# deryrahman/image-caption-emotion-indonesia

Measured on NVIDIA B200. Metric: decoder_train_tokens_per_sec, higher is better.
Workload: dtype bf16

## Files before the change

image-caption-emotion-indonesia_b200/_lib.py:

```python
import ctypes
import os
from ctypes import c_char_p, c_float, c_int32, c_int64, c_uint64, c_void_p

HERE = os.path.dirname(os.path.abspath(__file__))
LIB_PATH = os.path.join(HERE, "libsn100.so")

OP_NT, OP_NN, OP_TN = 0, 1, 2
CELL_FACTORED, CELL_LSTM = 0, 1

_P = c_void_p
_I32, _I64, _F = c_int32, c_int64, c_float

SIGNATURES = {
    "sn_version": (_I32, []),
    "sn_last_error": (c_char_p, []),
    "sn_device_info": (_I32, [_P, _P, _P, _P]),
    "sn_gather_pack_fwd": (_I32, [_P, _I64, _P, _I64, _P, _I64, _I32, _P, _P, _P, _I64, _P, _I64, _F, c_uint64, _P, _P, _I64, _P]),
    "sn_gather_pack_bwd": (_I32, [_P, _I64, _P, _I64, _P, _I64, _I32, _P, _P, _P, _I64, _P, _I64, _F, c_uint64, _P, _I64, _P, _P, _P]),
    "sn_gemm": (_I32, [_I32, _I64, _I64, _I64, _P, _I64, _P, _I64, _P, _I64, _P, _F, _I32, _I64, _I64, _I64, _I64, _P]),
    "sn_gemm_bf16": (_I32, [_I32, _I64, _I64, _I64, _P, _I64, _P, _I64, _P, _I64, _P, _I64, _P, _F, _I32, _I64, _I64, _I64, _I64, _I64, _P]),
    "sn_gemm_bf16_splitk": (_I32, [_I32, _I64, _I64, _I64, _P, _I64, _P, _I64, _P, _I64, _P, _I64, _P, _F, _I32, _I64, _I64, _I64, _I64, _I64, _I32, _P]),
    "sn_gemm2_ws_bytes": (_I64, [_I64, _I64, _I32, _I32]),
    "sn_gemm2_bf16": (_I32, [_I32, _I64, _I64, _I64, _P, _I64, _P, _I64, _P, _I64, _P, _I64, _P, _F, _I32, _I64, _I64, _I64, _I64, _I64, _I32, _P, _I64, _I32, _P]),
    "sn_vocab_ws_bytes": (_I64, [_I64, _I64]),
    "sn_vocab_nll_fwd": (_I32, [_I64, _I64, _I64, _P, _I64, _P, _I64, _P, _P, _P, _I64, _P, _P, _P, _P, _P, _P]),
    "sn_vocab_nll_bwd": (_I32, [_I64, _I64, _I64, _P, _I64, _P, _I64, _P, _P, _P, _P, _F, _P, _I64, _P, _P, _P]),
    "sn_cast_bf16": (_I32, [_P, _I64, _I64, _I64, _P, _I64, _I64, _P]),
    "sn_cast_bf16_ex": (_I32, [_P, _I64, _I64, _I64, _P, _I64, _I64, _I32, _P]),
    "sn_colsum": (_I32, [_P, _I64, _I64, _I64, _P, _F, _P]),
    "sn_colsum_ex": (_I32, [_P, _I64, _I64, _I64, _P, _F, _I32, _P]),
    "sn_colsum_bf16_ex": (_I32, [_P, _I64, _I64, _I64, _P, _F, _I32, _P]),
    "sn_embed_plan": (_I32, [_P, _I64, _I32, _P, _P, _P, _I64, _I64, _P, _P]),
    "sn_embed_grad": (_I32, [_P, _I64, _P, _I64, _I32, _P, _P, _P, _I64, _P, _I64, _F, c_uint64, _P, _I64, _P, _P, _I32, _P]),
    "sn_adam_clamp_dev_ex": (_I32, [_P, _P, _P, _P, _I32, _P, _P, _P, _P, _P, _F, _F, _F, _F, _I32, _P]),
    "sn_recur_ws_bytes": (_I64, [_I64, _I64]),
    "sn_recur_fwd": (_I32, [_I32, _I64, _I64, _P, _P, _I32, _I32, _P, _P, _P, _P, _P, _P, _P, _P, _P, _P, _P]),
    "sn_recur_bwd": (_I32, [_I32, _I64, _I64, _P, _P, _I32, _I32, _P, _P, _P, _P, _P, _P, _P, _P, _P, _P]),
    "sn_recur_fwd_bf16": (_I32, [_I32, _I64, _I64, _P, _P, _I32, _I32] + [_P] * 12),
    "sn_recur_bwd_bf16": (_I32, [_I32, _I64, _I64, _P, _P, _I32, _I32] + [_P] * 11),
    "sn_recur_cl_max_clusters": (_I32, [_I64]),
    "sn_recur_fwd_cl": (_I32, [_I32, _I64, _I64, _P, _P, _I32, _I32] + [_P] * 11),
    "sn_recur_bwd_cl": (_I32, [_I32, _I64, _I64, _P, _P, _I32, _I32] + [_P] * 11),
    "sn_gate_wait": (_I32, [_P, _I64, _P]),
    "sn_cast_bf16_gate_interleave": (_I32, [_P, _I64, _I64, _I64, _P, _I64, _P]),
    "sn_recur_fwd_gemm": (_I32, [_I32, _I64, _I64, _P, _P, _I32, _P, _P, _P, _P, _P, _P, _P, _P, _P]),
    "sn_recur_hprev": (_I32, [_P, _P, _P, _P, _I64, _I64, _P, _P]),
    "sn_recur_bwd_gemm": (_I32, [_I32, _I64, _I64, _P, _P, _I32, _P, _P, _P, _P, _P, _P, _P, _P, _P]),
    "sn_softmax_nll": (_I32, [_P, _I64, _I64, _I64, _P, _P, _P, _I64, _F, _P, _P, _P, _I64, _P]),
    "sn_colsum_bf16": (_I32, [_P, _I64, _I64, _I64, _P, _F, _P]),
    "sn_reduce_sum": (_I32, [_P, _I64, _F, _P, _I32, _P]),
    "sn_adam_clamp": (_I32, [_P, _P, _P, _P, _I32, _P, _P, _P, _F, _F, _F, _F, _P]),
    "sn_adam_clamp_dev": (_I32, [_P, _P, _P, _P, _I32, _P, _P, _P, _P, _P, _F, _F, _F, _F, _P]),
    "sn_enable_peer_access": (_I32, [_I32]),
    "sn_ipc_export": (_I32, [_P, _P, _P]),
    "sn_ipc_open": (_I32, [_P, _P]),
    "sn_ipc_close": (_I32, [_P]),
    "sn_dp_adam_fused": (_I32, [_I32, _I32, _P, _P, _P, _P, _P, _I32, _P, _P, _P, _P, _P, _F, _F, _F, _F, _P]),
    "sn_dp_slot_elems": (_I64, [_I64, _I32]),
    "sn_dp_push": (_I32, [_I32, _I32, _P, _P, _I64, _I32, _P, _I32, _P, _I32, _P]),
    "sn_dp_adam_recv": (_I32, [_I32, _I32, _P, _P, _P, _I64, _I32, _P, _P, _I32, _P, _P, _I32, _P, _P, _P, _P, _P, _F, _F, _F, _F, _I32, _P]),
    "sn_att_step_fwd": (_I32, [_P, _P, _P, _P, _F, _P, _I64, _I64, _I64, _I64, _P, _I64, _P, _I64, _P]),
    "sn_att_step_bwd": (_I32, [_P, _P, _P, _P, _F, _P, _P, _I64, _P, _I64, _P, _I64, _I64, _I64, _I64, _I64, _P, _P, _P, _P, _P, _P]),
    "sn_att_step_fwd_b16": (_I32, [_P, _P, _P, _P, _F, _P, _I64, _I64, _I64, _I64, _P, _I64, _P, _I64, _P]),
    "sn_att_step_bwd_b16": (_I32, [_P, _P, _P, _P, _P, _P, _I64, _P, _I64, _P, _I64, _I64, _I64, _I64, _I64, _P, _P, _P, _P, _P]),
    "sn_mean_pixels": (_I32, [_P, _I64, _I64, _I64, _P, _P]),
    "sn_beam_split_ws_floats": (_I64, [_I32, _I32, _I32]),
    "sn_beam_step_split": (_I32, [_P, _I64, _I64, _I32, _I32, _I32, _I32, _I32] + [_P] * 14 + [_I32, _P, _I32, _P]),
    "sn_split_limbs_cols": (_I32, [_P, _I64, _I64, _I64, _I64, _P, _I64, _I32, _P]),
    "sn_split_limbs_rows": (_I32, [_P, _I64, _I64, _I64, _I64, _P, _I64, _I64, _I32, _P]),
    "sn_skinny_max_rows": (_I32, []),
    "sn_skinny_linear": (_I32, [_P, _I64, _I64, _I64, _P, _I64, _I64, _I64, _I64, _P, _P, _I64, _P, _P]),
    "sn_decode_cell": (_I32, [_I32, _I64, _I64, _P, _I64, _I64, _P, _I64, _I64, _P, _P, _P, _P, _P, _P, _P, _P, _P, _P]),
    "sn_decode_cell_groups": (_I32, [_I32, _I64, _I64, _P, _I64, _P, _I64, _I64, _I64, _P, _I64, _I64, _P, _I64, _P, _P,
                                     _P, _P, _P, _P, _P, _P, _P]),
    "sn_pool_nhwc_fwd": (_I32, [_P, _I64, _I64, _I64, _I64, _I64, _P, _P, _P, _P]),
    "sn_pool_nhwc_bwd": (_I32, [_P, _I64, _I64, _I64, _I64, _I64, _P, _P]),
    "sn_bn1d_fwd": (_I32, [_P, _I64, _I64, _P, _P, _P, _P, _F, _F, _I32, _P, _P, _P, _P]),
    "sn_bn1d_bwd": (_I32, [_P, _P, _I64, _I64, _P, _P, _P, _I32, _P, _P, _P, _P]),
    "sn_beam_step": (_I32, [_P, _I64, _I64, _I32, _I32, _I32, _I32, _I32] + [_P] * 15),
    "sn_bleu_counts": (_I32, [_P, _P, _I64, _P, _P, _P, _I32, _I64, _P, _P]),
}

_lib = None


def load():
    global _lib
    if _lib is not None:
        return _lib
    if not os.path.exists(LIB_PATH):
        raise RuntimeError(
            "libsn100.so is not built (%s). Run `python -c 'import __graft_entry__ as g; g.build()'`; "
            "there is no CPU or PyTorch fallback for this path." % LIB_PATH)
    lib = ctypes.CDLL(LIB_PATH)
    for name, (res, args) in SIGNATURES.items():
        fn = getattr(lib, name)
        fn.restype = res
        fn.argtypes = args
    _lib = lib
    return lib


class SnError(RuntimeError):
    pass


def check(rc, what=""):
    if rc != 0:
        msg = load().sn_last_error()
        raise SnError("%s failed (rc=%d): %s" % (what or "libsn100 call", rc, msg.decode() if msg else "?"))


_dev_ok = {}


def require_device(device_index):
    if _dev_ok.get(device_index):
        return
    lib = load()
    sm = c_int32(); sh = c_int32(); ma = c_int32(); mi = c_int32()
    check(lib.sn_device_info(ctypes.byref(sm), ctypes.byref(sh), ctypes.byref(ma), ctypes.byref(mi)), "sn_device_info")
    _dev_ok[device_index] = (sm.value, sh.value, ma.value, mi.value)
```

image-caption-emotion-indonesia_b200/csrc/sn_elementwise.cu:

```cuda
#include <stdlib.h>
#include <string.h>
#include <cuda_bf16.h>

#include "sn_common.cuh"

namespace {

__global__ void gather_pack_fwd_kernel(const int64_t* __restrict__ captions, int64_t cap_ld,
                                       const float* __restrict__ table, int E,
                                       const float* __restrict__ features, int64_t feat_ld, int has_feat,
                                       const int32_t* __restrict__ row_b, const int32_t* __restrict__ row_t,
                                       const int32_t* __restrict__ tok_override, int64_t N,
                                       float* __restrict__ X, int64_t ldx, float p, float inv_keep,
                                       uint64_t seed, const uint64_t* __restrict__ seed_dev,
                                       __nv_bfloat16* __restrict__ Xb, int64_t ldxb, int Ep) {
  if (seed_dev) seed += *seed_dev;
  int64_t row = (int64_t)blockIdx.x * (blockDim.x >> 5) + (threadIdx.x >> 5);
  if (row >= N) return;
  int lane = threadIdx.x & 31;
  int b = row_b[row], t = row_t[row];
  int ov = tok_override ? tok_override[row] : -1;
  float* dst = X ? X + row * ldx : nullptr;
  __nv_bfloat16* dstb = Xb ? Xb + row * ldxb : nullptr;
  const float* src;
// ... 180 lines not shown
    for (int u = 0; u < EBW_BATCH; ++u) {
      const int q = q0 + u;
      x[u] = 0.f; sc[u] = 0.f;
      if (q < n) {
        const int64_t j = rows[q];
        x[u] = dX[j * ldx + c];
        sc[u] = sn::dropout_scale(seed, (uint32_t)j, (uint32_t)c, rate[q], inv_keep);
      }
    }
#pragma unroll
    for (int u = 0; u < EBW_BATCH; ++u)
      if (sc[u] != 0.f) acc = __fmaf_rn(x[u], sc[u], acc);
  }
  if (e - s <= EB_CHUNK) dtable[(int64_t)t * E + c] += acc;
  else part[(int64_t)(cstart[t] + (i - s) / EB_CHUNK) * E + c] = acc;
}

__global__ void embed_combine_kernel(const int32_t* __restrict__ cnt, const int32_t* __restrict__ cstart, int64_t V,
                                     int E, const float* __restrict__ part, float* __restrict__ dtable) {
  const int64_t t = (int64_t)blockIdx.x * (blockDim.x >> 5) + (threadIdx.x >> 5);
  if (t >= V || cnt[t] <= EB_CHUNK) return;
  const int lane = threadIdx.x & 31;
  const int32_t nq = (cnt[t] + EB_CHUNK - 1) / EB_CHUNK;
  const float* src = part + (int64_t)cstart[t] * E;
  for (int c = lane; c < E; c += 32) {
    float a = 0.f;
    for (int32_t q = 0; q < nq; ++q) a += src[(int64_t)q * E + c];
    dtable[t * E + c] += a;
  }
}

__global__ void __launch_bounds__(256) softmax_nll_kernel(const float* __restrict__ logits, int64_t V, int64_t ld,
                                                          const int64_t* __restrict__ targets,
                                                          float* __restrict__ row_loss, float* dlogits, int64_t ldd,
                                                          float grad_scale, int64_t* __restrict__ argmax,
                                                          int32_t* __restrict__ top5hit, int use_smem,
                                                          __nv_bfloat16* __restrict__ dlb, int64_t lddb) {
  extern __shared__ float srow[];
  __shared__ float red_v[8];
  __shared__ int red_i[8];
  __shared__ float bc_f[2];
  __shared__ int bc_i;
  const int64_t row = blockIdx.x;
  const float* src = logits + row * ld;
  const int tid = threadIdx.x, lane = tid & 31, warp = tid >> 5;

  float mx = -INFINITY;
  int mi = 0x7fffffff;
  for (int64_t c = tid; c < V; c += 256) {
    float v = src[c];
    if (use_smem) srow[c] = v;
    if (v > mx) { mx = v; mi = (int)c; }
  }
#pragma unroll
  for (int o = 16; o > 0; o >>= 1) {
    float ov = __shfl_xor_sync(0xffffffffu, mx, o);
    int oi = __shfl_xor_sync(0xffffffffu, mi, o);
    if (ov > mx || (ov == mx && oi < mi)) { mx = ov; mi = oi; }
  }
  if (lane == 0) { red_v[warp] = mx; red_i[warp] = mi; }
  __syncthreads();
  if (tid == 0) {
    float bm = red_v[0]; int bi = red_i[0];
    for (int w = 1; w < 8; ++w)
      if (red_v[w] > bm || (red_v[w] == bm && red_i[w] < bi)) { bm = red_v[w]; bi = red_i[w]; }
    bc_f[0] = bm; bc_i = bi;
  }
  __syncthreads();
  mx = bc_f[0];
  if (tid == 0 && argmax) argmax[row] = bc_i;
  if (!targets) return;

  const float* rd = use_smem ? srow : src;
  const int64_t tgt = targets[row];
  const float tv = rd[tgt];
  float se = 0.f;
  int above = 0;
  for (int64_t c = tid; c < V; c += 256) {
    float v = rd[c];
    se += expf(v - mx);
    above += (v > tv);
  }
  se = sn::warp_sum(se);
#pragma unroll
  for (int o = 16; o > 0; o >>= 1) above += __shfl_xor_sync(0xffffffffu, above, o);
  __syncthreads();
  if (lane == 0) { red_v[warp] = se; red_i[warp] = above; }
  __syncthreads();
  if (tid == 0) {
    float s = 0.f; int a = 0;
    for (int w = 0; w < 8; ++w) { s += red_v[w]; a += red_i[w]; }
    float lse = mx + logf(s);
    bc_f[1] = lse;
    if (row_loss) row_loss[row] = lse - tv;
    if (top5hit) top5hit[row] = a < 5 ? 1 : 0;
  }
  __syncthreads();
  if (dlogits || dlb) {
    const float lse = bc_f[1];
    float* dst = dlogits ? dlogits + row * ldd : nullptr;
    __nv_bfloat16* dstb = dlb ? dlb + row * lddb : nullptr;
    for (int64_t c = tid; c < V; c += 256) {
      float pr = expf(rd[c] - lse);
      float gr = (pr - (c == tgt ? 1.f : 0.f)) * grad_scale;
      if (dst) dst[c] = gr;
      if (dstb) dstb[c] = __float2bfloat16(gr);
    }
    if (dstb) for (int64_t c = V + tid; c < lddb; c += 256) dstb[c] = __float2bfloat16(0.f);
  }
}

__global__ void __launch_bounds__(1024) reduce_sum_kernel(const float* __restrict__ x, int64_t N, float scale,
                                                           float* out, int accumulate) {
  __shared__ double part[32];
  double s = 0.0;
  for (int64_t i = threadIdx.x; i < N; i += 1024) s += (double)x[i];
#pragma unroll
  for (int o = 16; o > 0; o >>= 1) s += __shfl_xor_sync(0xffffffffu, s, o);
  if ((threadIdx.x & 31) == 0) part[threadIdx.x >> 5] = s;
  __syncthreads();
  if (threadIdx.x == 0) {
    double t = 0.0;
    for (int w = 0; w < 32; ++w) t += part[w];
    float r = (float)(t * (double)scale);
    *out = accumulate ? *out + r : r;
  }
}

struct AdamRanges {
  static constexpr int MAX = 128;
  int64_t off[MAX];
  int32_t len[MAX];
  float step_size[MAX], bc2_sqrt[MAX];
  int step_idx[MAX];
  int32_t chunk_start[MAX + 1];
  int n;
};
static_assert(sizeof(AdamRanges) <= 3700, "AdamRanges must leave room for the other kernel parameters below 4 KB");

__global__ void adam_prepare_kernel(AdamRanges R, int32_t* __restrict__ steps, const float* __restrict__ lr,
                                    float* __restrict__ coef, float beta1, float beta2) {
  int r = threadIdx.x;
  if (r >= R.n) return;
  int st = steps[R.step_idx[r]] + 1;
  steps[R.step_idx[r]] = st;
  double bc1 = 1.0 - pow((double)beta1, (double)st);
  double bc2 = 1.0 - pow((double)beta2, (double)st);
  coef[2 * R.step_idx[r]] = (float)((double)(*lr) / bc1);
  coef[2 * R.step_idx[r] + 1] = (float)sqrt(bc2);
}
constexpr int ADAM_CHUNK = 4096;
constexpr int64_t ADAM_MAX_LEN = (1LL << 31) - 2 * ADAM_CHUNK;

__global__ void __launch_bounds__(256) adam_clamp_kernel(float* __restrict__ p, float* __restrict__ g,
                                                         float* __restrict__ m, float* __restrict__ v,
                                                         AdamRanges R, const float* __restrict__ coef, float beta1,
                                                         float beta2, float eps, float clip) {
  const int64_t total_chunks = R.chunk_start[R.n];
  for (int64_t ch = blockIdx.x; ch < total_chunks; ch += gridDim.x) {
    int r = 0;
    while (ch >= R.chunk_start[r + 1]) ++r;
    const int64_t base = R.off[r] + (ch - R.chunk_start[r]) * ADAM_CHUNK;
    const int64_t end = R.off[r] + R.len[r];
    const float ss = coef ? coef[2 * R.step_idx[r]] : R.step_size[r], bc = coef ? coef[2 * R.step_idx[r] + 1] : R.bc2_sqrt[r];
    const int64_t lim = base + ADAM_CHUNK < end ? base + ADAM_CHUNK : end;
    if ((base & 3) == 0 && lim - base == ADAM_CHUNK) {
#pragma unroll
      for (int it = 0; it < ADAM_CHUNK / (256 * 4); ++it) {
        const int64_t i = base + (int64_t)(it * 256 + threadIdx.x) * 4;
        float4 g4 = *reinterpret_cast<const float4*>(g + i);
        float4 m4 = *reinterpret_cast<const float4*>(m + i);
        float4 v4 = *reinterpret_cast<const float4*>(v + i);
        float4 p4 = *reinterpret_cast<const float4*>(p + i);
        float* gp = &g4.x; float* mp = &m4.x; float* vp = &v4.x; float* pp = &p4.x;
#pragma unroll
        for (int e = 0; e < 4; ++e) {
          float gi = gp[e];
          if (clip > 0.f) gi = fminf(fmaxf(gi, -clip), clip);
          gp[e] = gi;
          float mi = mp[e] + (1.f - beta1) * (gi - mp[e]);
          float vi = vp[e] * beta2 + (1.f - beta2) * gi * gi;
          float denom = sqrtf(vi) / bc + eps;
          pp[e] = pp[e] - ss * (mi / denom);
          mp[e] = mi; vp[e] = vi;
        }
        if (clip > 0.f) *reinterpret_cast<float4*>(g + i) = g4;
        *reinterpret_cast<float4*>(m + i) = m4;
        *reinterpret_cast<float4*>(v + i) = v4;
        *reinterpret_cast<float4*>(p + i) = p4;
      }
      continue;
    }
    for (int64_t i = base + threadIdx.x; i < lim; i += 256) {
      float gi = g[i];
      if (clip > 0.f) { gi = fminf(fmaxf(gi, -clip), clip); g[i] = gi; }
      float mi = m[i], vi = v[i];
      mi = mi + (1.f - beta1) * (gi - mi);
      vi = vi * beta2 + (1.f - beta2) * gi * gi;
      float denom = sqrtf(vi) / bc + eps;
      p[i] = p[i] - ss * (mi / denom);
      m[i] = mi; v[i] = vi;
    }
  }
}

struct DpPeers {
  float* grad[8];
  float* param[8];
  int* pad[8];
  int world, rank;
  void* recv[8];
  int64_t slot_elems;
  int* wait_pad[4];
  int n_wait;
};
constexpr int PAD_ARRIVE = 0, PAD_DONE = 8, PAD_COUNTER = 16, PAD_EPOCH = 17, PAD_DONE_COUNTER = 18;

__device__ __forceinline__ int ld_acquire_sys(const int* p) {
  int v;
  asm volatile("ld.acquire.sys.global.s32 %0, [%1];" : "=r"(v) : "l"(p) : "memory");
  return v;
}
__device__ __forceinline__ void st_release_sys(int* p, int v) {
  asm volatile("st.release.sys.global.s32 [%0], %1;" ::"l"(p), "r"(v) : "memory");
}

constexpr int DP_SUB = 4;
template <typename TT>
__global__ void __launch_bounds__(256 * DP_SUB) dp_push_kernel(DpPeers P, AdamRanges R, const float* __restrict__ g) {
  const int W = P.world;
  __shared__ int s_last;
  int* mypad = P.pad[P.rank];
  const int64_t total_chunks = R.chunk_start[R.n];
  const int sub = threadIdx.x >> 8, tid = threadIdx.x & 255;
  for (int64_t ch = (int64_t)blockIdx.x * DP_SUB + sub; ch < total_chunks; ch += (int64_t)gridDim.x * DP_SUB) {
    int r = 0;
    while (ch >= R.chunk_start[r + 1]) ++r;
    const int64_t aid = R.off[r] / ADAM_CHUNK + (ch - R.chunk_start[r]);
    const int owner = (int)(aid % W);
    if (owner == P.rank) continue;
    const int64_t end = R.off[r] + R.len[r];
    const int64_t base = aid * ADAM_CHUNK > R.off[r] ? aid * ADAM_CHUNK : R.off[r];
    const int64_t lim = (aid + 1) * ADAM_CHUNK < end ? (aid + 1) * ADAM_CHUNK : end;
    TT* dst = reinterpret_cast<TT*>(P.recv[owner]) + (int64_t)P.rank * P.slot_elems + (aid / W) * ADAM_CHUNK - aid * ADAM_CHUNK;
    if ((base & 3) == 0 && lim - base == ADAM_CHUNK) {
      float4 t[ADAM_CHUNK / 1024];
#pragma unroll
      for (int u = 0; u < ADAM_CHUNK / 1024; ++u)
        t[u] = __ldcg(reinterpret_cast<const float4*>(g + base + (int64_t)(u * 256 + tid) * 4));
#pragma unroll
      for (int u = 0; u < ADAM_CHUNK / 1024; ++u) {
        const int64_t i = base + (int64_t)(u * 256 + tid) * 4;
        if constexpr (sizeof(TT) == 4) {
          *reinterpret_cast<float4*>(dst + i) = t[u];
        } else {
          __nv_bfloat162 lo = __floats2bfloat162_rn(t[u].x, t[u].y), hi = __floats2bfloat162_rn(t[u].z, t[u].w);
          uint2 pk;
          pk.x = *reinterpret_cast<uint32_t*>(&lo); pk.y = *reinterpret_cast<uint32_t*>(&hi);
          *reinterpret_cast<uint2*>(dst + i) = pk;
        }
      }
      continue;
    }
    for (int64_t i = base + tid; i < lim; i += 256) {
      if constexpr (sizeof(TT) == 4) dst[i] = g[i]; else dst[i] = __float2bfloat16_rn(g[i]);
    }
  }
  __syncthreads();
  if (threadIdx.x == 0) {
    __threadfence_system();
    s_last = (atomicAdd(mypad + PAD_COUNTER, 1) == (int)gridDim.x - 1);
  }
  __syncthreads();
  if (s_last) {
    if (threadIdx.x == 0) {
      __threadfence_system();
      const int e = mypad[PAD_EPOCH] + 1;
      for (int q = 0; q < W; ++q) st_release_sys(P.pad[q] + PAD_ARRIVE + P.rank, e);
      mypad[PAD_COUNTER] = 0;
    }
  }
}

template <int W>
__global__ void __launch_bounds__(256) dp_adam_fused_kernel(DpPeers P, AdamRanges R, const float* __restrict__ coef,
                                                            float* __restrict__ m, float* __restrict__ v, float beta1,
                                                            float beta2, float eps, float clip, int dbg) {
  if (dbg) {
    for (int q = 0; q < P.world; ++q) {
      if (dbg & 1) P.grad[q] = P.grad[P.rank];
      if (dbg & 2) P.param[q] = P.param[P.rank];
    }
  }
  __shared__ int s_epoch, s_last;
  int* mypad = P.pad[P.rank];
  if (threadIdx.x == 0) s_epoch = mypad[PAD_EPOCH] + 1;
  __syncthreads();
  const int e = s_epoch;
  if (blockIdx.x == 0 && threadIdx.x < P.world) st_release_sys(P.pad[threadIdx.x] + PAD_ARRIVE + P.rank, e);
  if (threadIdx.x < P.world) { while (ld_acquire_sys(mypad + PAD_ARRIVE + threadIdx.x) < e) { } }
  __syncthreads();
  const int64_t total_chunks = R.chunk_start[R.n];
  const int64_t nslots = (total_chunks + W - 1) / W;
  for (int64_t slot = blockIdx.x; slot < nslots; slot += gridDim.x)
  for (int j = 0; j < W; ++j) {
    const int64_t ch = slot * W + j;
    if (ch >= total_chunks) break;
    int r = 0;
    while (ch >= R.chunk_start[r + 1]) ++r;
    const int64_t aid = R.off[r] / ADAM_CHUNK + (ch - R.chunk_start[r]);
    if ((int)(aid % W) != P.rank) continue;
    const int64_t end = R.off[r] + R.len[r];
    const int64_t base = aid * ADAM_CHUNK > R.off[r] ? aid * ADAM_CHUNK : R.off[r];
    const int64_t lim = (aid + 1) * ADAM_CHUNK < end ? (aid + 1) * ADAM_CHUNK : end;
    const float ss = coef[2 * R.step_idx[r]], bc = coef[2 * R.step_idx[r] + 1];
    if ((base & 3) == 0 && lim - base == ADAM_CHUNK) {
      constexpr int NIT = W <= 4 ? 4 : 2;
#pragma unroll
      for (int it0 = 0; it0 < ADAM_CHUNK / (256 * 4); it0 += NIT) {
        float4 t[NIT][W], m4[NIT], v4[NIT], p4[NIT];
#pragma unroll
        for (int u = 0; u < NIT; ++u) {
          const int64_t i = base + (int64_t)((it0 + u) * 256 + threadIdx.x) * 4;
#pragma unroll
          for (int q = 0; q < W; ++q) t[u][q] = __ldcg(reinterpret_cast<const float4*>(P.grad[q] + i));
        }
#pragma unroll
        for (int u = 0; u < NIT; ++u) {
          const int64_t i = base + (int64_t)((it0 + u) * 256 + threadIdx.x) * 4;
          m4[u] = *reinterpret_cast<const float4*>(m + i);
          v4[u] = *reinterpret_cast<const float4*>(v + i);
          p4[u] = *reinterpret_cast<const float4*>(P.param[P.rank] + i);
        }
#pragma unroll
        for (int u = 0; u < NIT; ++u) {
          const int64_t i = base + (int64_t)((it0 + u) * 256 + threadIdx.x) * 4;
          float4 g4 = t[u][0];
#pragma unroll
          for (int q = 1; q < W; ++q) { g4.x += t[u][q].x; g4.y += t[u][q].y; g4.z += t[u][q].z; g4.w += t[u][q].w; }
          float* gp = &g4.x; float* mp = &m4[u].x; float* vp = &v4[u].x; float* pp = &p4[u].x;
#pragma unroll
          for (int k = 0; k < 4; ++k) {
            float gi = gp[k];
            if (clip > 0.f) gi = fminf(fmaxf(gi, -clip), clip);
            const float mi = mp[k] + (1.f - beta1) * (gi - mp[k]);
            const float vi = vp[k] * beta2 + (1.f - beta2) * gi * gi;
            pp[k] = pp[k] - ss * (mi / (sqrtf(vi) / bc + eps));
            mp[k] = mi; vp[k] = vi;
          }
          *reinterpret_cast<float4*>(m + i) = m4[u];
          *reinterpret_cast<float4*>(v + i) = v4[u];
#pragma unroll
          for (int q = 0; q < W; ++q) *reinterpret_cast<float4*>(P.param[q] + i) = p4[u];
        }
      }
      continue;
// ... 37 lines not shown
                                                           const float* __restrict__ g, const TT* __restrict__ recv,
                                                           const float* p_loc, float* __restrict__ m, float* __restrict__ v, float beta1,
                                                           float beta2, float eps, float clip) {
  __shared__ int s_epoch, s_last;
  const int rank = P.rank;
  int* mypad = P.wait_pad[0];
  if (threadIdx.x == 0) s_epoch = mypad[PAD_EPOCH] + 1;
  if (threadIdx.x < W * P.n_wait) {
    const int* wp = P.wait_pad[threadIdx.x / W];
    const int q = threadIdx.x % W;
    if (q != rank) { const int we = wp[PAD_EPOCH] + 1; while (ld_acquire_sys(wp + PAD_ARRIVE + q) < we) { } }
  }
  __syncthreads();
  const int e = s_epoch;
  const int64_t total_chunks = R.chunk_start[R.n];
  const int sub = threadIdx.x >> 8, tid = threadIdx.x & 255;
  for (int64_t ch = (int64_t)blockIdx.x * DP_RSUB + sub; ch < total_chunks; ch += (int64_t)gridDim.x * DP_RSUB) {
    int r = 0;
    while (ch >= R.chunk_start[r + 1]) ++r;
    const int64_t a0 = R.off[r] / ADAM_CHUNK;
    const int64_t aid = a0 + ((rank - a0) % W + W) % W + (ch - R.chunk_start[r]) * W;
    const int64_t end = R.off[r] + R.len[r];
    const int64_t base = aid * ADAM_CHUNK > R.off[r] ? aid * ADAM_CHUNK : R.off[r];
    const int64_t lim = (aid + 1) * ADAM_CHUNK < end ? (aid + 1) * ADAM_CHUNK : end;
    const float ss = coef[2 * R.step_idx[r]], bc = coef[2 * R.step_idx[r] + 1];
    const int64_t rbase = (aid / W) * ADAM_CHUNK - aid * ADAM_CHUNK;
    if ((base & 3) == 0 && lim - base == ADAM_CHUNK) {
#pragma unroll
      for (int it = 0; it < ADAM_CHUNK / (256 * 4); ++it) {
        const int64_t i = base + (int64_t)(it * 256 + tid) * 4;
        float4 t[W];
#pragma unroll
        for (int q = 0; q < W; ++q) {
          if (q == rank) {
            t[q] = __ldcg(reinterpret_cast<const float4*>(g + i));
          } else if constexpr (sizeof(TT) == 4) {
            t[q] = __ldcg(reinterpret_cast<const float4*>(recv + q * P.slot_elems + rbase + i));
          } else {
            const uint2 pk = __ldcg(reinterpret_cast<const uint2*>(recv + q * P.slot_elems + rbase + i));
            const float2 lo = __bfloat1622float2(*reinterpret_cast<const __nv_bfloat162*>(&pk.x));
            const float2 hi = __bfloat1622float2(*reinterpret_cast<const __nv_bfloat162*>(&pk.y));
            t[q] = make_float4(lo.x, lo.y, hi.x, hi.y);
          }
        }
        float4 m4 = *reinterpret_cast<const float4*>(m + i);
        float4 v4 = *reinterpret_cast<const float4*>(v + i);
        float4 p4 = *reinterpret_cast<const float4*>(p_loc + i);
        float4 g4 = t[0];
#pragma unroll
        for (int q = 1; q < W; ++q) { g4.x += t[q].x; g4.y += t[q].y; g4.z += t[q].z; g4.w += t[q].w; }
        float* gp = &g4.x; float* mp = &m4.x; float* vp = &v4.x; float* pp = &p4.x;
#pragma unroll
        for (int k = 0; k < 4; ++k) {
          float gi = gp[k];
          if (clip > 0.f) gi = fminf(fmaxf(gi, -clip), clip);
          const float mi = mp[k] + (1.f - beta1) * (gi - mp[k]);
          const float vi = vp[k] * beta2 + (1.f - beta2) * gi * gi;
          pp[k] = pp[k] - ss * (mi / (sqrtf(vi) / bc + eps));
          mp[k] = mi; vp[k] = vi;
        }
        *reinterpret_cast<float4*>(m + i) = m4;
        *reinterpret_cast<float4*>(v + i) = v4;
#pragma unroll
        for (int q = 0; q < W; ++q) *reinterpret_cast<float4*>(P.param[q] + i) = p4;
      }
      continue;
    }
    for (int64_t i = base + tid; i < lim; i += 256) {
      float gi = 0.f;
#pragma unroll
      for (int q = 0; q < W; ++q) {
        float gq;
        if (q == rank) gq = __ldcg(g + i);
        else if constexpr (sizeof(TT) == 4) gq = __ldcg(recv + q * P.slot_elems + rbase + i);
        else gq = __bfloat162float(recv[q * P.slot_elems + rbase + i]);
        gi = q == 0 ? gq : gi + gq;
      }
      if (clip > 0.f) gi = fminf(fmaxf(gi, -clip), clip);
      const float mi = m[i] + (1.f - beta1) * (gi - m[i]);
      const float vi = v[i] * beta2 + (1.f - beta2) * gi * gi;
      const float pn = p_loc[i] - ss * (mi / (sqrtf(vi) / bc + eps));
      m[i] = mi; v[i] = vi;
#pragma unroll
      for (int q = 0; q < W; ++q) P.param[q][i] = pn;
    }
  }
  __syncthreads();
  if (threadIdx.x == 0) {
    __threadfence_system();
    s_last = (atomicAdd(mypad + PAD_DONE_COUNTER, 1) == (int)gridDim.x - 1);
  }
  __syncthreads();
  if (s_last) {
    if (threadIdx.x == 0) __threadfence_system();
    __syncthreads();
    if (threadIdx.x < W) {
      st_release_sys(P.pad[threadIdx.x] + PAD_DONE + rank, e);
      while (ld_acquire_sys(mypad + PAD_DONE + threadIdx.x) < e) { }
    }
    __syncthreads();
    if (threadIdx.x == 0) {
      mypad[PAD_DONE_COUNTER] = 0; mypad[PAD_EPOCH] = e;
      for (int k = 1; k < P.n_wait; ++k) P.wait_pad[k][PAD_EPOCH] = P.wait_pad[k][PAD_EPOCH] + 1;
    }
  }
}

__global__ void mean_pixels_kernel(const float* __restrict__ feat, int64_t P, int64_t D, float* __restrict__ out) {
  int64_t b = blockIdx.y;
  int64_t d = (int64_t)blockIdx.x * blockDim.x + threadIdx.x;
  if (d >= D) return;
  const float* src = feat + b * P * D + d;
  float s = 0.f;
  for (int64_t pz = 0; pz < P; ++pz) s += src[pz * D];
  out[b * D + d] = s / (float)P;
}

}

extern "C" {

int32_t sn_gather_pack_fwd(const int64_t* captions, int64_t cap_ld, const float* table, int64_t E,
                           const float* features, int64_t feat_ld, int32_t has_feat,
                           const int32_t* row_b, const int32_t* row_t, const int32_t* tok_override,
                           int64_t N, float* X, int64_t ldx, float p_drop, uint64_t seed, const uint64_t* seed_dev,
                           void* Xb, int64_t ldxb, void* stream) {
  SN_REQUIRE(N >= 0 && E > 0 && (X || Xb), "sn_gather_pack_fwd: bad dims N=%lld E=%lld", (long long)N, (long long)E);
  SN_REQUIRE(!X || ldx >= E, "sn_gather_pack_fwd: ldx=%lld < E", (long long)ldx);
  SN_REQUIRE(!Xb || ldxb >= E, "sn_gather_pack_fwd: ldxb=%lld < E", (long long)ldxb);
  SN_REQUIRE(p_drop >= 0.f && p_drop < 1.f, "sn_gather_pack_fwd: dropout p=%f out of [0,1)", p_drop);
  SN_REQUIRE(!has_feat || features, "sn_gather_pack_fwd: has_feat without features");
  if (N == 0) return 0;
  float inv_keep = 1.f / (1.f - p_drop);
  unsigned grid = (unsigned)((N + 7) / 8);
  gather_pack_fwd_kernel<<<grid, 256, 0, (cudaStream_t)stream>>>(captions, cap_ld, table, (int)E, features, feat_ld,
                                                                 has_feat, row_b, row_t, tok_override, N, X, ldx,
                                                                 p_drop, inv_keep, seed, seed_dev,
                                                                 (__nv_bfloat16*)Xb, ldxb, Xb ? (int)ldxb : (int)E);
  return sn::check_launch("sn_gather_pack_fwd");
}

int32_t sn_gather_pack_bwd(const int64_t* captions, int64_t cap_ld, float* dtable, int64_t E,
                           float* dfeatures, int64_t feat_ld, int32_t has_feat, const int32_t* row_b,
                           const int32_t* row_t, const int32_t* tok_override, int64_t N,
                           const float* dX, int64_t ldx, float p_drop, uint64_t seed, const uint64_t* seed_dev,
                           int64_t V, int32_t* ws_int, float* ws_part, void* stream) {
  SN_REQUIRE(N >= 0 && E > 0 && ldx >= E && V > 0, "sn_gather_pack_bwd: bad dims");
  SN_REQUIRE(p_drop >= 0.f && p_drop < 1.f, "sn_gather_pack_bwd: dropout p=%f out of [0,1)", p_drop);
  SN_REQUIRE(N < (int64_t)1 << 30, "sn_gather_pack_bwd: N=%lld rows", (long long)N);
  if (N == 0) return 0;
  SN_REQUIRE(ws_int && ws_part, "sn_gather_pack_bwd: null work space");
  if (int32_t rc = sn_embed_plan(captions, cap_ld, has_feat, row_b, row_t, tok_override, N, V, ws_int, stream)) return rc;
  return sn_embed_grad(dtable, E, dfeatures, feat_ld, has_feat, row_b, row_t, tok_override, N, dX, ldx, p_drop, seed,
                       seed_dev, V, ws_int, ws_part, 0, stream);
}

namespace {
struct EmbedWs {
  int32_t *cnt, *start, *cursor, *cstart, *tok32, *perm, *sorted;
  EmbedWs(int32_t* ws, int64_t V, int64_t N)
      : cnt(ws), start(cnt + V), cursor(start + V + 1), cstart(cursor + V), tok32(cstart + V), perm(tok32 + N),
        sorted(perm + N) {}
};
}

int32_t sn_embed_plan(const int64_t* captions, int64_t cap_ld, int32_t has_feat, const int32_t* row_b,
                      const int32_t* row_t, const int32_t* tok_override, int64_t N, int64_t V, int32_t* ws_int,
                      void* stream) {
  SN_REQUIRE(N >= 0 && N < (int64_t)1 << 30 && V > 0, "sn_embed_plan: bad dims N=%lld V=%lld", (long long)N, (long long)V);
  if (N == 0) return 0;
  SN_REQUIRE(ws_int, "sn_embed_plan: null work space");
  cudaStream_t st = (cudaStream_t)stream;
  EmbedWs w(ws_int, V, N);
  SN_CUDA(cudaMemsetAsync(w.cnt, 0, sizeof(int32_t) * (size_t)V, st));
  const unsigned g_rows = (unsigned)((N + 255) / 256);
  embed_count_kernel<<<g_rows, 256, 0, st>>>(captions, cap_ld, has_feat, row_b, row_t, tok_override, N, w.tok32, w.cnt);
  embed_scan_kernel<<<1, 1024, 0, st>>>(w.cnt, V, w.start, w.cursor, w.cstart);
  embed_place_kernel<<<g_rows, 256, 0, st>>>(w.tok32, N, w.cursor, w.perm);
  embed_order_kernel<<<g_rows, 256, 0, st>>>(w.tok32, w.start, w.perm, N, V, w.sorted);
  return sn::check_launch("sn_embed_plan");
}

int32_t sn_embed_grad(float* dtable, int64_t E, float* dfeatures, int64_t feat_ld, int32_t has_feat,
                      const int32_t* row_b, const int32_t* row_t, const int32_t* tok_override, int64_t N,
                      const float* dX, int64_t ldx, float p_drop, uint64_t seed, const uint64_t* seed_dev, int64_t V,
                      const int32_t* ws_int, float* ws_part, int32_t wide, void* stream) {
  SN_REQUIRE(N >= 0 && N < (int64_t)1 << 30 && E > 0 && ldx >= E && V > 0, "sn_embed_grad: bad dims");
  SN_REQUIRE(p_drop >= 0.f && p_drop < 1.f, "sn_embed_grad: dropout p=%f out of [0,1)", p_drop);
  if (N == 0) return 0;
  SN_REQUIRE(ws_int && ws_part, "sn_embed_grad: null work space");
  cudaStream_t st = (cudaStream_t)stream;
  float inv_keep = 1.f / (1.f - p_drop);
  if (has_feat && dfeatures)
    gather_pack_bwd_kernel<<<(unsigned)((N + 7) / 8), 256, 0, st>>>(nullptr, 0, dtable, (int)E, dfeatures,
                                                                     feat_ld, has_feat, row_b, row_t, tok_override, N,
                                                                     dX, ldx, p_drop, inv_keep, seed, seed_dev);
  EmbedWs w(const_cast<int32_t*>(ws_int), V, N);
  if (wide && E <= 512)
    embed_chunk_wide_kernel<<<(unsigned)N, (unsigned)((E + 31) / 32 * 32), 0, st>>>(
        w.tok32, w.start, w.cstart, w.sorted, V, tok_override, dX, ldx, (int)E, p_drop, inv_keep, seed, seed_dev,
        dtable, ws_part);
  else
    embed_chunk_kernel<<<(unsigned)((N + 7) / 8), 256, 0, st>>>(w.tok32, w.start, w.cstart, w.sorted, V, tok_override,
                                                                 dX, ldx, (int)E, p_drop, inv_keep, seed, seed_dev,
                                                                 dtable, ws_part);
  embed_combine_kernel<<<(unsigned)((V + 7) / 8), 256, 0, st>>>(w.cnt, w.cstart, V, (int)E, ws_part, dtable);
  return sn::check_launch("sn_embed_grad");
}

int32_t sn_softmax_nll(const float* logits, int64_t N, int64_t V, int64_t ld, const int64_t* targets,
                       float* row_loss, float* dlogits, int64_t ldd, float grad_scale, int64_t* argmax,
                       int32_t* top5hit, void* dlogits_bf16, int64_t lddb, void* stream) {
  SN_REQUIRE(N >= 0 && V > 0 && ld >= V, "sn_softmax_nll: bad dims");
  SN_REQUIRE(!dlogits_bf16 || lddb >= V, "sn_softmax_nll: lddb < V");
  if (N == 0) return 0;
  size_t smem = (size_t)V * sizeof(float);
  int use_smem = smem <= 200 * 1024;
  if (use_smem && smem > 48 * 1024) {
    static thread_local size_t configured = 0;
    if (configured < smem) {
      SN_CUDA(cudaFuncSetAttribute(softmax_nll_kernel, cudaFuncAttributeMaxDynamicSharedMemorySize, 200 * 1024));
      configured = 200 * 1024;
    }
  }
  softmax_nll_kernel<<<(unsigned)N, 256, use_smem ? smem : 0, (cudaStream_t)stream>>>(
      logits, V, ld, targets, row_loss, dlogits, ldd, grad_scale, argmax, top5hit, use_smem,
      (__nv_bfloat16*)dlogits_bf16, lddb);
  return sn::check_launch("sn_softmax_nll");
}

int32_t sn_reduce_sum(const float* x, int64_t N, float scale, float* out, int32_t accumulate, void* stream) {
  SN_REQUIRE(N >= 0 && out, "sn_reduce_sum: bad args");
  reduce_sum_kernel<<<1, 1024, 0, (cudaStream_t)stream>>>(x, N, scale, out, accumulate);
  return sn::check_launch("sn_reduce_sum");
}

int32_t sn_adam_clamp(float* p, float* g, float* m, float* v, int32_t n_ranges, const int64_t* ranges,
                      const float* step_size, const float* bc2_sqrt, float beta1, float beta2, float eps,
                      float clip, void* stream) {
  SN_REQUIRE(n_ranges >= 0, "sn_adam_clamp: n_ranges < 0");
  int done = 0;
  while (done < n_ranges) {
    AdamRanges R;
    R.n = 0;
    R.chunk_start[0] = 0;
    while (done < n_ranges && R.n < AdamRanges::MAX) {
      int64_t off = ranges[2 * done], len = ranges[2 * done + 1];
      SN_REQUIRE(off >= 0 && len >= 0 && len < ADAM_MAX_LEN, "sn_adam_clamp: bad range %d", done);
      R.off[R.n] = off; R.len[R.n] = (int32_t)len;
      R.step_size[R.n] = step_size[done]; R.bc2_sqrt[R.n] = bc2_sqrt[done];
      R.chunk_start[R.n + 1] = R.chunk_start[R.n] + (len + ADAM_CHUNK - 1) / ADAM_CHUNK;
      ++R.n; ++done;
    }
    int64_t chunks = R.chunk_start[R.n];
    if (chunks == 0) continue;
    int64_t cap = (int64_t)sn::dev_info().sm_count * 8;
    unsigned grid = (unsigned)(chunks < cap ? chunks : cap);
    adam_clamp_kernel<<<grid, 256, 0, (cudaStream_t)stream>>>(p, g, m, v, R, nullptr, beta1, beta2, eps, clip);
    int32_t rc = sn::check_launch("sn_adam_clamp");
    if (rc) return rc;
  }
  return 0;
}

int32_t sn_adam_clamp_dev(float* p, float* g, float* m, float* v, int32_t n_ranges, const int64_t* ranges,
                          const int32_t* step_idx, int32_t* steps_dev, const float* lr_dev, float* coef_ws,
                          float beta1, float beta2, float eps, float clip, void* stream) {
  return sn_adam_clamp_dev_ex(p, g, m, v, n_ranges, ranges, step_idx, steps_dev, lr_dev, coef_ws, beta1, beta2, eps,
                              clip, 0, stream);
}

int32_t sn_adam_clamp_dev_ex(float* p, float* g, float* m, float* v, int32_t n_ranges, const int64_t* ranges,
                             const int32_t* step_idx, int32_t* steps_dev, const float* lr_dev, float* coef_ws,
                             float beta1, float beta2, float eps, float clip, int32_t max_ctas, void* stream) {
  SN_REQUIRE(max_ctas >= 0, "sn_adam_clamp_dev: max_ctas < 0");
  SN_REQUIRE(n_ranges >= 0 && n_ranges <= AdamRanges::MAX, "sn_adam_clamp_dev: at most %d ranges per call", AdamRanges::MAX);
  SN_REQUIRE(steps_dev && lr_dev && coef_ws, "sn_adam_clamp_dev: null argument");
  if (n_ranges == 0) return 0;
  AdamRanges R;
  R.n = n_ranges;
  R.chunk_start[0] = 0;
  for (int i = 0; i < n_ranges; ++i) {
    SN_REQUIRE(ranges[2 * i] >= 0 && ranges[2 * i + 1] >= 0 && ranges[2 * i + 1] < ADAM_MAX_LEN, "sn_adam_clamp_dev: bad range %d", i);
    R.off[i] = ranges[2 * i]; R.len[i] = (int32_t)ranges[2 * i + 1]; R.step_idx[i] = step_idx[i];
    R.step_size[i] = 0.f; R.bc2_sqrt[i] = 1.f;
    R.chunk_start[i + 1] = R.chunk_start[i] + (R.len[i] + ADAM_CHUNK - 1) / ADAM_CHUNK;
  }
  cudaStream_t st = (cudaStream_t)stream;
  adam_prepare_kernel<<<1, AdamRanges::MAX, 0, st>>>(R, steps_dev, lr_dev, coef_ws, beta1, beta2);
  int64_t chunks = R.chunk_start[R.n];
  if (chunks == 0) return sn::check_launch("sn_adam_clamp_dev");
  int64_t cap = (int64_t)sn::dev_info().sm_count * 8;
  if (max_ctas > 0 && max_ctas < cap) cap = max_ctas;
  unsigned grid = (unsigned)(chunks < cap ? chunks : cap);
  adam_clamp_kernel<<<grid, 256, 0, st>>>(p, g, m, v, R, coef_ws, beta1, beta2, eps, clip);
  return sn::check_launch("sn_adam_clamp_dev");
}

int32_t sn_enable_peer_access(int32_t peer_device) {
  int cur = 0;
  SN_CUDA(cudaGetDevice(&cur));
  if (peer_device == cur) return 0;
  int can = 0;
  SN_CUDA(cudaDeviceCanAccessPeer(&can, cur, peer_device));
  SN_REQUIRE(can, "sn_enable_peer_access: device %d cannot access peer %d", cur, peer_device);
  cudaError_t e = cudaDeviceEnablePeerAccess(peer_device, 0);
  if (e == cudaErrorPeerAccessAlreadyEnabled) { cudaGetLastError(); return 0; }
  if (e != cudaSuccess) return sn::fail((int32_t)e, "cudaDeviceEnablePeerAccess(%d): %s", peer_device, cudaGetErrorString(e));
  return 0;
}

int32_t sn_dp_adam_fused(int32_t world, int32_t rank, void* const* grad_ptrs, void* const* param_ptrs,
                         void* const* pad_ptrs, float* m, float* v, int32_t n_ranges, const int64_t* ranges,
                         const int32_t* step_idx, int32_t* steps_dev, const float* lr_dev, float* coef_ws, float beta1,
                         float beta2, float eps, float clip, void* stream) {
  SN_REQUIRE(world >= 1 && world <= 8 && rank >= 0 && rank < world, "sn_dp_adam_fused: bad world/rank %d/%d", world, rank);
  SN_REQUIRE(n_ranges >= 0 && n_ranges <= AdamRanges::MAX, "sn_dp_adam_fused: at most %d ranges per call", AdamRanges::MAX);
  SN_REQUIRE(grad_ptrs && param_ptrs && pad_ptrs && steps_dev && lr_dev && coef_ws && m && v, "sn_dp_adam_fused: null argument");
  DpPeers P;
  memset(&P, 0, sizeof(P));
  P.world = world; P.rank = rank;
  for (int q = 0; q < 8; ++q) {
    P.grad[q] = q < world ? (float*)grad_ptrs[q] : nullptr;
    P.param[q] = q < world ? (float*)param_ptrs[q] : nullptr;
    P.pad[q] = q < world ? (int*)pad_ptrs[q] : nullptr;
    SN_REQUIRE(q >= world || (P.grad[q] && P.param[q] && P.pad[q]), "sn_dp_adam_fused: null peer pointer %d", q);
  }
  AdamRanges R;
  R.n = n_ranges;
  R.chunk_start[0] = 0;
  for (int i = 0; i < n_ranges; ++i) {
    SN_REQUIRE(ranges[2 * i] >= 0 && ranges[2 * i + 1] >= 0 && ranges[2 * i + 1] < ADAM_MAX_LEN, "sn_dp_adam_fused: bad range %d", i);
    R.off[i] = ranges[2 * i]; R.len[i] = (int32_t)ranges[2 * i + 1]; R.step_idx[i] = step_idx[i];
    R.step_size[i] = 0.f; R.bc2_sqrt[i] = 1.f;
    R.chunk_start[i + 1] = R.chunk_start[i] +
        (R.len[i] > 0 ? (R.off[i] + R.len[i] - 1) / ADAM_CHUNK - R.off[i] / ADAM_CHUNK + 1 : 0);
  }
  cudaStream_t st = (cudaStream_t)stream;
  if (n_ranges > 0) adam_prepare_kernel<<<1, AdamRanges::MAX, 0, st>>>(R, steps_dev, lr_dev, coef_ws, beta1, beta2);
  int64_t mine = (R.chunk_start[R.n] + world - 1) / world;
  int64_t cap = (int64_t)sn::dev_info().sm_count * 3;
  unsigned grid = (unsigned)(mine < 1 ? 1 : (mine < cap ? mine : cap));
  static const int dbg = [] { const char* e = getenv("SN_DP_DEBUG"); return e ? atoi(e) : 0; }();
#define SN_DP_LAUNCH(WW) dp_adam_fused_kernel<WW><<<grid, 256, 0, st>>>(P, R, coef_ws, m, v, beta1, beta2, eps, clip, dbg)
  switch (world) {
    case 1: SN_DP_LAUNCH(1); break;
    case 2: SN_DP_LAUNCH(2); break;
    case 3: SN_DP_LAUNCH(3); break;
    case 4: SN_DP_LAUNCH(4); break;
    case 5: SN_DP_LAUNCH(5); break;
    case 6: SN_DP_LAUNCH(6); break;
    case 7: SN_DP_LAUNCH(7); break;
    default: SN_DP_LAUNCH(8); break;
  }
#undef SN_DP_LAUNCH
  return sn::check_launch("sn_dp_adam_fused");
}

static int32_t dp_fill_ranges(AdamRanges& R, int32_t n_ranges, const int64_t* ranges, const int32_t* step_idx, const char* who) {
  SN_REQUIRE(n_ranges >= 0 && n_ranges <= AdamRanges::MAX, "%s: at most %d ranges per call", who, AdamRanges::MAX);
// ... 120 lines not shown
```

image-caption-emotion-indonesia_b200/decoders.py:

```python
import random
from collections import OrderedDict

import os

import torch
import torch.nn as nn

from . import ops
from .arena import ParamArena
from .packing import get_plan

GREEDY_GRAPH = [True]

GATES = ("i", "f", "o", "c")
STYLES = ("factual", "happy", "sad", "angry")


def style_attr(style, gate):
    return ("S_f" + gate) if style == "factual" else ("S_%s_%s" % (style, gate))


def _ref_init(module, emb, out):
    for p in module.parameters():
        if p.dim() >= 2:
            nn.init.xavier_uniform_(p.data)
        else:
            nn.init.zeros_(p.data)
    emb.weight.data.uniform_(-0.1, 0.1)
    out.bias.data.fill_(0)
    out.weight.data.uniform_(-0.1, 0.1)


class _Ctx:
    pass


class _HiddenFn(torch.autograd.Function):

    @staticmethod
    def forward(ctx, anchor, features, dec, plan, captions, coins, mode, save):
        c = dec._run_forward(plan, captions, features, coins, mode, save=save)
        ctx.dec, ctx.c = dec, c
        ctx.need_dfeat = features is not None and features.requires_grad
        return c.top.Hall

    @staticmethod
    def backward(ctx, dHall):
        dec, c = ctx.dec, ctx.c
        gbuf = dec._grad_target(c.grad_names)
        dfeat = dec._run_backward(c, dHall.contiguous(), gbuf, ctx.need_dfeat)
        dec._publish(c.grad_names, gbuf)
        return None, dfeat, None, None, None, None, None, None


class _LogitsFn(torch.autograd.Function):

    @staticmethod
    def forward(ctx, Hall, anchor, dec):
        ctx.dec = dec
        ctx.save_for_backward(Hall)
        return dec._vocab_logits(Hall)

    @staticmethod
    def backward(ctx, dlogits):
        dec = ctx.dec
        (Hall,) = ctx.saved_tensors
        gbuf = dec._grad_target(dec._out_names())
        dHall = dec._vocab_backward(Hall, dlogits.contiguous(), gbuf)
        dec._publish(dec._out_names(), gbuf)
        return dHall, None, None


def _pad8(n):
    return (n + 7) // 8 * 8


class _DecoderBase(nn.Module):

    cell = ops.CELL_FACTORED
    precision = "fp32"

    _TRANSIENT = ("_greedy_graphs", "_decode_sessions", "_side_streams", "_out_w16", "_out_w16_pref", "_out_w16_ev",
                  "_out_h16", "_seed_dev", "_arena", "_att_cache", "_gate_flag", "_gate_armed", "_after_recur", "_bucket_hook",
                  "_emb_early")

    def __getstate__(self):
        st = self.__dict__.copy()
        for k in self._TRANSIENT:
            st.pop(k, None)
        return st

    def set_precision(self, precision):
        if precision not in ("fp32", "bf16"):
            raise ValueError("precision must be 'fp32' or 'bf16'")
        self.precision = precision
        return self

    @property
    def bf16(self):
        return self.precision == "bf16"

    def _shadow(self, w, rows=None, cols=None):
        return ops.to_bf16_padded(w)

    def _arena_groups(self):
        raise NotImplementedError

    def arena(self):
        a = self.__dict__.get("_arena")
        if a is None:
            a = ParamArena(self, self._arena_groups())
            self.__dict__["_arena"] = a
        return a.ensure()

    def _grad_target(self, names):
        a = self.arena()
        if any(a.named[n].grad is not None for n in names):
            return torch.zeros_like(a.gflat)
        return a.gflat

    def _publish(self, names, gbuf):
        self.arena().publish_grads(names, gbuf)

    def _side(self, i=0):
        sts = self.__dict__.setdefault("_side_streams", {})
        st = sts.get(i)
        if st is None:
            st = torch.cuda.Stream()
            sts[i] = st
        return st

    def _fork(self, i=0):
        side = self._side(i)
        side.wait_stream(torch.cuda.current_stream())
        return side

    def _join(self):
        for st in self.__dict__.get("_side_streams", {}).values():
            torch.cuda.current_stream().wait_stream(st)

    def _take_out_shadow(self):
        Wb = self.__dict__.pop("_out_w16_pref", None)
        ev = self.__dict__.pop("_out_w16_ev", None)
        if Wb is not None and ev is not None:
            torch.cuda.current_stream().wait_event(ev)
        return Wb

    def _shadows_async(self, specs, max_blocks=24):
        main = torch.cuda.current_stream()
        outs = []
        for dct, key, w in specs:
            R, C = w.shape
            Cp = (C + 7) // 8 * 8
            out = torch.empty(R, Cp, dtype=torch.bfloat16, device=w.device)
            dct[key] = out
            outs.append((w, out, R, C, Cp))
        side = self._side(2)
        side.wait_stream(main)
        with torch.cuda.stream(side):
            for w, out, R, C, Cp in outs:
                ops.cast_bf16(w, R, C, w.stride(0), out, Cp, Cp, max_blocks=max_blocks)
            ev = torch.cuda.Event()
            ev.record(side)
        return ev

    def _next_seed(self, dev, p_drop):
        base = int(self.__dict__.get("_seed", 0x5EED)) * 1000003
        if p_drop <= 0.0:
            return base, None
        sd = self.__dict__.get("_seed_dev")
        if sd is None or sd.device != dev:
            sd = torch.zeros(1, dtype=torch.int64, device=dev)
            self.__dict__["_seed_dev"] = sd
        sd.add_(1)
        return base, sd

    def _check_inputs(self, captions, features):
        if not captions.is_cuda:
            raise ops._lib.SnError("decoder inputs must be CUDA tensors: this path has no CPU fallback")
        ops.lib()

    def _emb(self):
        raise NotImplementedError

    def _out(self):
        raise NotImplementedError

    def _input_projection(self, c, X, mode, r0, n):
        raise NotImplementedError

    def _input_projection_bwd(self, c, dZ, gbuf):
        raise NotImplementedError

    def _coins(self, T, teacher_forcing_ratio):
        return [random.random() < teacher_forcing_ratio for _ in range(T)]

    def _run_forward(self, plan, captions, features, coins, mode, save):
        a = self.arena()
        dev = captions.device
        d = plan.dev(dev)
        H, N, B, T = self.hidden_size, plan.N, plan.B, plan.T
        emb = self._emb()
        E = emb.weight.shape[1]
        has_feat = features is not None
        c = _Ctx()
        c.plan, c.mode, c.has_feat, c.captions = plan, mode, has_feat, captions
        c.p_drop = float(self.dropout.p) if self.training else 0.0
        c.seed, c.seed_dev = self._next_seed(dev, c.p_drop)
        feats = None
        if has_feat:
            feats = features.detach()
            if feats.dtype != torch.float32 or not feats.is_contiguous():
                feats = feats.float().contiguous()
            if feats.dim() == 3:
                feats = feats.reshape(feats.shape[0], -1)
        all_tf = all(coins)
        c.tok_override = None
        if not all_tf:
            c.tok_override = torch.full((N,), -1, dtype=torch.int32, device=dev)
        c.emb_ws = c.emb_ev = c.emb_zeroed = None
        if self.__dict__.pop("_emb_early", False) and all_tf:
            V = emb.weight.shape[0]
            c.emb_ws = ops.embed_plan_ws(V, N, dev)
            c.emb_zeroed = a.gflat
            gE = self._gview(a.gflat, [self._emb_name()], emb.weight.shape)
            side = self._side(4)
            side.wait_stream(torch.cuda.current_stream())
            with torch.cuda.stream(side):
                ops.embed_plan(captions, has_feat, d["row_b"], d["row_t"], None, N, V, c.emb_ws)
                gE.zero_()
                c.emb_ev = torch.cuda.Event()
                c.emb_ev.record(side)
        c.Ein = E
        c.w16 = {}
        c.ev_early = c.ev_late = c.ev_first = None
        if self.bf16:
            early, late = self._shadow_specs(c, mode)
            first = c.__dict__.pop("first_specs", None)
            if first:
                c.ev_first = self._shadows_async(first, max_blocks=0)
            second = c.__dict__.pop("second_specs", None)
            c.ev_second = self._shadows_async(second, max_blocks=0) if second else None
            if early:
                c.ev_early = self._shadows_async(early)
            if late:
                c.ev_late = self._shadows_async(late)
            self.__dict__["_out_w16_ev"] = self._shadows_async([(self.__dict__, "_out_w16_pref", self._out().weight)])
        if self.bf16:
            X = None
            c.Xb = torch.empty(N, _pad8(E), dtype=torch.bfloat16, device=dev)
        else:
            X = torch.empty(N, E, dtype=torch.float32, device=dev)
            c.Xb = None
        ops.gather_pack_fwd(captions, emb.weight, feats, has_feat, d["row_b"], d["row_t"], None, N, X,
                            c.p_drop, c.seed, seed_dev=c.seed_dev, Xb=c.Xb)
        c.X = X
        c.XP = torch.empty(N, 4 * H, dtype=torch.float32, device=dev)
        self._input_projection(c, X, mode, 0, N)
        c.Hall = torch.empty(N, H, dtype=torch.float32, device=dev)
        c.Call = torch.empty(N, H, dtype=torch.float32, device=dev) if save else None
        c.Hprev = torch.empty(N, H, dtype=torch.float32, device=dev) if save else None
        c.gates = torch.empty(N, 4 * H, dtype=torch.float32, device=dev) if save else None
        c_state = torch.zeros(B, H, dtype=torch.float32, device=dev)
        c.aux_argmax = None
        Whh, bhh = self._recurrent_weights()
        c.Whh, c.bhh = Whh, bhh
        use_tc = self.bf16 and H % 32 == 0
        c.Hb = c.Hpb = None
        if c.ev_late is not None:
            torch.cuda.current_stream().wait_event(c.ev_late)
        if use_tc:
            if "Whh" not in c.w16:
                c.w16["Whh"] = self._shadow(Whh)
            c.Hb = torch.empty(N, H, dtype=torch.bfloat16, device=dev)
            c.Hpb = torch.empty(N, H, dtype=torch.bfloat16, device=dev) if save else None
            c.Hprev = None
        c.upper = self._upper_layers_init(c, save)
        c.top = c.upper[-1] if c.upper else c

        c.c_state = c_state

        def run(t0, t1):
            self._recur_fwd(c, c, t0, t1)
            if c.upper:
                self._upper_layers_fwd(c, t0, t1)

        if all_tf:
            run(0, T)
        else:
            out = self._out()
            V = out.weight.shape[0]
            pred = captions[:, 0].to(torch.int32).contiguous()
            am = torch.empty(B, dtype=torch.int64, device=dev)
            t = 0
            while t < T:
                if coins[t]:
                    t1 = t
                    while t1 < T and coins[t1]:
                        t1 += 1
                    run(t, t1)
                    t = t1
                else:
                    bt, r0 = plan.bs[t], plan.off[t]
                    if t > 0:
                        bp, rp = plan.bs[t - 1], plan.off[t - 1]
                        lg = torch.empty(bp, V, dtype=torch.float32, device=dev)
                        ops.gemm(ops.OP_NT, c.top.Hall, out.weight, lg, bp, V, H, H, H, V, bias=out.bias,
                                 a_off=rp * H)
                        ops.softmax_nll(lg, bp, V, argmax=am)
                        pred = am[:bp].to(torch.int32)
                    c.tok_override[r0:r0 + bt] = pred[:bt]
                    ops.gather_pack_fwd(captions, emb.weight, feats, has_feat, d["row_b"], d["row_t"],
                                        c.tok_override, bt, X, c.p_drop, c.seed, row_off=r0, seed_dev=c.seed_dev,
                                        Xb=c.Xb)
                    self._input_projection(c, X, mode, r0, bt)
                    run(t, t + 1)
                    t += 1
        c.grad_names = self._seq_grad_names(mode)
        c.feat_shape = None if features is None else features.shape
        if not save:
            c.X = c.XP = None
        return c

    def _recur_fwd(self, c, cl, t0, t1):
        plan = c.plan
        d = plan.dev(cl.XP.device)
        H, B, T = self.hidden_size, plan.B, plan.T
        Whh, bhh = cl.Whh, cl.bhh
        if cl.Hb is not None:
            if t0 == 0 and t1 == T and B >= ops.RECUR_GEMM_MIN_BATCH[0] and H % 64 == 0:
                if "Whh_il" not in cl.w16:
                    cl.w16["Whh_il"] = ops.cast_gate_interleave(Whh)
                if cl.Call is None:
                    cl.Call = torch.empty(plan.N, H, dtype=torch.float32, device=cl.XP.device)
                ops.recur_fwd_gemm(self.cell, H, B, plan, cl.XP, cl.w16["Whh_il"], bhh, cl.Hall, cl.Hb, cl.Call, cl.gates)
                if cl.Hpb is not None:
                    ops.recur_hprev(cl.Hb, d, plan.N, H, cl.Hpb)
                cl.recur_gemm = True
                return
            h_init = cl.Hall[plan.off[t0 - 1]:] if t0 > 0 else None
            ops.recur_fwd_bf16(self.cell, H, B, d["bs"], d["off"], t0, t1, cl.XP, cl.w16["Whh"], bhh, h_init,
                               cl.Hall, cl.Hb, cl.Hpb, cl.Call, cl.gates, cl.c_state)
        else:
            h_init = cl.Hall[plan.off[t0 - 1]:] if t0 > 0 else None
            ops.recur_fwd(self.cell, H, B, d["bs"], d["off"], t0, t1, cl.XP, Whh, bhh, h_init, cl.Hall,
                          cl.Call, cl.Hprev, cl.gates, cl.c_state)

    def _shadow_specs(self, c, mode):
        H = self.hidden_size
        late = []
        if H % 32 == 0:
            late.append((c.w16, "Whh", self._recurrent_weights()[0]))
        return [], late

    def _upper_layers_init(self, c, save):
        return []

    def _upper_layers_fwd(self, c, t0, t1):
        pass

    def _layer_bwd(self, c, cl, dHall, gbuf):
        plan = c.plan
        dev = dHall.device
        d = plan.dev(dev)
        H, N, B, T = self.hidden_size, plan.N, plan.B, plan.T
        L = getattr(cl, "layer", 0)
        Whh, _ = self._recurrent_weights(L)
        dZ = torch.empty(N, 4 * H, dtype=torch.float32, device=dev)
        dhc = torch.zeros(2, B, H, dtype=torch.float32, device=dev)
        dh, dc = dhc[0], dhc[1]
        gW, gbW = self._recurrent_grads(gbuf, L)
        if cl.Hpb is not None:
            cl.dZb = torch.empty(N, 4 * H, dtype=torch.bfloat16, device=dev)
            if getattr(cl, "recur_gemm", False):
                ops.recur_bwd_gemm(self.cell, H, B, plan, cl.w16["Whh"], cl.Call, cl.gates, dHall, dZ, cl.dZb, dc)
            else:
                ops.recur_bwd_bf16(self.cell, H, B, d["bs"], d["off"], 0, T, cl.w16["Whh"], None, cl.Call, cl.gates,
                                   dHall, dZ, cl.dZb, dh, dc, start_flag=self.__dict__.pop("_gate_armed", None))
            self._run_deferred()
            with torch.cuda.stream(self._fork()):
                ops.gemm_bf16(ops.OP_TN, cl.dZb, cl.Hpb, 4 * H, H, N, 4 * H, H, C=gW, ldc=H)
                ops.colsum(dZ, N, 4 * H, 4 * H, gbW, wide=bool(ops.TAIL_SCHEDULE[0]))
            cl.colsum_dZ = gbW if ops.TAIL_SCHEDULE[0] else None
            return self._input_projection_bwd(cl, dZ, gbuf)
        ops.recur_bwd(self.cell, H, B, d["bs"], d["off"], 0, T, Whh, None, cl.Call, cl.gates, dHall, dZ, dh, dc)
        if self.bf16:
            cl.dZb = ops.to_bf16_padded(dZ)
            Hpb = ops.to_bf16_padded(cl.Hprev)
            ops.gemm_bf16(ops.OP_TN, cl.dZb, Hpb, 4 * H, H, N, 4 * H, H, C=gW, ldc=H)
        else:
            ops.gemm(ops.OP_TN, dZ, cl.Hprev, gW, 4 * H, H, N, 4 * H, H, H)
        ops.colsum(dZ, N, 4 * H, 4 * H, gbW)
        return self._input_projection_bwd(cl, dZ, gbuf)

    def _run_backward(self, c, dHall, gbuf, need_dfeat):
        for cl in reversed(c.upper):
            dHall = self._layer_bwd(c, cl, dHall, gbuf)
        dX = self._layer_bwd(c, c, dHall, gbuf)
        out = self._embedding_bwd(c, dX, gbuf, need_dfeat)
        self._join()
        return out

    def _embedding_bwd(self, c, dX, gbuf, need_dfeat):
        plan = c.plan
        dev = dX.device
        d = plan.dev(dev)
        N, B = plan.N, plan.B
        emb = self._emb()
        E = emb.weight.shape[1]
        gE = self._gview(gbuf, [self._emb_name()], emb.weight.shape)
        dfeat = torch.empty(B, E, dtype=torch.float32, device=dev) if (need_dfeat and c.has_feat) else None
        if getattr(c, "emb_ws", None) is not None:
            torch.cuda.current_stream().wait_event(c.emb_ev)
            if gbuf is not c.emb_zeroed:
                gE.zero_()
            ops.embed_grad(gE, dfeat, c.has_feat, d["row_b"], d["row_t"], c.tok_override, N, dX, c.p_drop, c.seed,
                           c.emb_ws, seed_dev=c.seed_dev, wide=True)
        else:
            gE.zero_()
            ops.gather_pack_bwd(c.captions, gE, dfeat, c.has_feat, d["row_b"], d["row_t"], c.tok_override, N, dX,
                                c.p_drop, c.seed, seed_dev=c.seed_dev)
        if dfeat is not None and c.feat_shape is not None:
            dfeat = dfeat.view(c.feat_shape)
        self._bucket_final([self._emb_name()])
        return dfeat

    def _run_deferred(self):
        todo = self.__dict__.pop("_after_recur", None)
        for fn in todo or ():
            fn()

    def _bucket_final(self, names):
        hook = self.__dict__.get("_bucket_hook")
        if hook is None:
            return
        gbuf, fn = hook
        names = [n for n in names if n in self.arena().named]
        self._publish(names, gbuf)
        fn(names)

    def _gview(self, gbuf, names, shape):
        a = self.arena()
        o, n = a._span(names)
        return gbuf[o:o + n].view(shape)

    def _vocab_logits(self, Hall, Hb=None):
        out = self._out()
        if self.bf16:
            V, H = out.weight.shape
            N = Hall.shape[0]
            if Hb is None:
                Hb = ops.to_bf16_padded(Hall.contiguous())
            Wb = self._take_out_shadow()
            if Wb is None:
                Wb = ops.to_bf16_padded(out.weight)
            self.__dict__["_out_w16"] = Wb
            logits = torch.empty(N, V, dtype=torch.float32, device=Hall.device)
            ops.gemm_bf16(ops.OP_NT, Hb, Wb, N, V, H, Hb.stride(0), Wb.stride(0), C=logits, ldc=V, bias=out.bias)
            return logits
        return ops.linear_nt(Hall.contiguous(), out.weight, out.bias)

    def _vocab_backward(self, Hall, dlogits, gbuf, Hb=None, dLb=None, defer=None, gate_B=None):
        out = self._out()
        V, H = out.weight.shape
        N = Hall.shape[0]
        wn, bn = self._out_names()
        gC = self._gview(gbuf, [wn], (V, H))
        gb = self._gview(gbuf, [bn], (V,))
        dHall = torch.empty(N, H, dtype=torch.float32, device=Hall.device)
        if self.bf16:
            have_b16 = dLb is not None
            if not have_b16:
                dLb = ops.to_bf16_padded(dlogits)
            hb_stash = self.__dict__.pop("_out_h16", None)
            if Hb is None:
                Hb = hb_stash if (have_b16 and hb_stash is not None) else ops.to_bf16_padded(Hall.contiguous())
            Wb = self.__dict__.pop("_out_w16", None) if dLb is not None and have_b16 else None
            if Wb is None:
                Wb = ops.to_bf16_padded(out.weight)
            if have_b16:
                mode_dc = ops.DC_SCHEDULE[0] if defer is not None else 0
                side = self._side(0)
                if mode_dc != 2:
                    side.wait_stream(torch.cuda.current_stream())
                ops.gemm_bf16(ops.OP_NN, dLb, Wb, N, H, V, dLb.stride(0), Wb.stride(0), C=dHall, ldc=H)
                if mode_dc == 1:
                    side.wait_stream(torch.cuda.current_stream())

                gate = None
                if mode_dc == 0 and gate_B is not None and ops.GATE_DC[0] and ops.recur_cluster_ok(H, gate_B):
                    gate = self.__dict__.get("_gate_flag")
                    if gate is None or gate.device != dHall.device:
                        gate = self.__dict__["_gate_flag"] = torch.zeros(3, dtype=torch.int32, device=dHall.device)
                    self.__dict__["_gate_armed"] = gate

                def side_work():
                    if mode_dc == 2:
                        side.wait_stream(torch.cuda.current_stream())
                    with torch.cuda.stream(side):
                        if gate is not None:
                            ops.gate_wait(gate)
                        ops.gemm_bf16(ops.OP_TN, dLb, Hb, V, H, N, dLb.stride(0), Hb.stride(0), C=gC, ldc=H,
                                      max_pairs=0 if mode_dc == 2 else ops.DC_MAX_PAIRS[0])
                        ops.colsum_bf16(dLb, N, V, dLb.stride(0), gb, wide=bool(ops.TAIL_SCHEDULE[0]))
                if mode_dc == 0:
                    side_work()
                else:
                    defer.append(side_work)
                return dHall
            ops.gemm_bf16(ops.OP_NN, dLb, Wb, N, H, V, dLb.stride(0), Wb.stride(0), C=dHall, ldc=H)
            ops.gemm_bf16(ops.OP_TN, dLb, Hb, V, H, N, dLb.stride(0), Hb.stride(0), C=gC, ldc=H)
        else:
            ops.gemm(ops.OP_NN, dlogits, out.weight, dHall, N, H, V, dlogits.stride(0), H, H)
            ops.gemm(ops.OP_TN, dlogits, Hall, gC, V, H, N, dlogits.stride(0), H, H)
        ops.colsum(dlogits, N, V, dlogits.stride(0), gb)
        return dHall

    def _vocab_nll(self, Hall, Hb, targets, denom, backward):
        out = self._out()
        V, H = out.weight.shape
        N, dev = Hall.shape[0], Hall.device
        row_loss = torch.empty(N, dtype=torch.float32, device=dev)
        argmax = torch.empty(N, dtype=torch.int64, device=dev)
        top5 = torch.empty(N, dtype=torch.int32, device=dev)
        if self.bf16:
            if Hb is None:
                Hb = ops.to_bf16_padded(Hall.contiguous())
            Wb = self._take_out_shadow()
            if Wb is None:
                Wb = ops.to_bf16_padded(out.weight)
            self.__dict__["_out_w16"] = Wb
            self.__dict__["_out_h16"] = Hb
            tl = torch.empty(N, dtype=torch.float32, device=dev)
            lse = torch.empty(N, dtype=torch.float32, device=dev)
            above = torch.empty(N, dtype=torch.int32, device=dev)
            ops.vocab_nll_fwd(Hb, Wb, out.bias, targets, N, V, H, tl, lse, row_loss=row_loss, argmax=argmax, above=above)
            dLb = torch.empty(N, _pad8(V), dtype=torch.bfloat16, device=dev) if backward else None
            ops.vocab_nll_bwd(Hb, Wb, out.bias, targets, N, V, H, tl, lse, 1.0 / denom, dLb=dLb, above=above,
                              top5hit=top5)
            return row_loss, argmax, top5, None, dLb
        logits = self._vocab_logits(Hall, Hb)
        ops.softmax_nll(logits, N, V, targets=targets, row_loss=row_loss, dlogits=logits if backward else None,
                        grad_scale=1.0 / denom, argmax=argmax, top5hit=top5)
        return row_loss, argmax, top5, logits, None

    def _forward_greedy(self, captions, lengths, features, mode):
        key = (tuple(int(l) for l in lengths), mode, tuple(captions.shape),
               None if features is None else tuple(features.shape), self.precision, self.training,
               captions.device.index, self.arena().version)
        cache = self.__dict__.setdefault("_greedy_graphs", OrderedDict())
        sess = cache.get(key)
        if sess is None:
            sess = cache[key] = _Ctx()
            sess.calls, sess.graph = 0, None
            while len(cache) > 4:
                cache.popitem(last=False)
        cache.move_to_end(key)
        sess.calls += 1
        plan = get_plan(lengths)
        coins = self._coins(plan.T, 0.0)
        if sess.graph is None and sess.calls < 2:
            c = self._run_forward(plan, captions.contiguous(), features, coins, mode, save=False)
            return self._vocab_logits(c.top.Hall, c.top.Hb)
        if sess.graph is None:
            sess.captions = captions.contiguous().clone()
            sess.features = None if features is None else features.detach().clone()
            torch.cuda.synchronize()
            g = torch.cuda.CUDAGraph()
            with ops.no_gc_during_capture(), torch.cuda.graph(g):
                c = self._run_forward(plan, sess.captions, sess.features, coins, mode, save=False)
                sess.out = self._vocab_logits(c.top.Hall, c.top.Hb)
            sess.graph = g
        sess.captions.copy_(captions, non_blocking=True)
        if features is not None:
            sess.features.copy_(features, non_blocking=True)
        sess.graph.replay()
        return sess.out.clone()

    def _greedy_eligible(self, captions, lengths, features, teacher_forcing_ratio):
        if torch.is_grad_enabled() or teacher_forcing_ratio > 0.0 or not GREEDY_GRAPH[0] or not captions.is_cuda:
            return False
        if torch.cuda.is_current_stream_capturing():
            return False
        if features is not None and features.shape[-1] != self._emb().weight.shape[1]:
            return False
        plan = get_plan(lengths)
        T_in = captions.shape[1] + (1 if features is not None else 0)
        return plan.B == captions.shape[0] and plan.T <= T_in

    def _forward_hidden(self, captions, lengths, features, teacher_forcing_ratio, mode):
        self._check_inputs(captions, features)
        if features is not None and features.shape[-1] != self._emb().weight.shape[1]:
            raise RuntimeError("features must be [B, embed_size]")
        plan = get_plan(lengths)
        if plan.B != captions.shape[0]:
            raise RuntimeError("len(lengths) != batch size")
        T_in = captions.shape[1] + (1 if features is not None else 0)
        if plan.T > T_in:
            raise RuntimeError("lengths exceed the (feature +) caption length")
        coins = self._coins(plan.T, teacher_forcing_ratio)
        captions = captions.contiguous()
        anchor = self._out().weight
        save = torch.is_grad_enabled()
        return _HiddenFn.apply(anchor, features, self, plan, captions, coins, mode, save), plan

    def forward_loss(self, captions, lengths, features=None, targets=None, teacher_forcing_ratio=1.0,
                     mode="factual", backward=True, n_global=None, grad_hook=None, early_step=None, early_embed=False):
        self._check_inputs(captions, features)
        plan = get_plan(lengths)
        coins = self._coins(plan.T, teacher_forcing_ratio)
        captions = captions.contiguous()
        dev = captions.device
        self.__dict__["_emb_early"] = bool(early_embed and backward and self.bf16 and self._emb().weight.grad is None)
        with torch.no_grad():
            c = self._run_forward(plan, captions, features, coins, mode, save=backward)
            N = plan.N
            out = self._out()
            V = out.weight.shape[0]
            if targets is None:
                if features is None:
                    raise ValueError("forward_loss: pass `targets` when features is None (language-only "
                                     "pass: inputs captions[:, :-1], targets packed captions[:, 1:])")
                if self.bf16:
                    targets = torch.empty(N, dtype=captions.dtype, device=dev)
                    side = self._side(2)
                    with torch.cuda.stream(side):
                        self._default_targets(captions, plan, True, out=targets)
                        ev = torch.cuda.Event()
                        ev.record(side)
                    torch.cuda.current_stream().wait_event(ev)
                else:
                    targets = self._default_targets(captions, plan, True)
            denom = float(n_global if n_global is not None else N)
            row_loss, argmax, top5, logits, dLb = self._vocab_nll(c.top.Hall, c.top.Hb, targets, denom, backward)
            loss = torch.empty(1, dtype=torch.float32, device=dev)
            if not (backward and dLb is not None):
                ops.reduce_sum(row_loss, N, 1.0 / denom, loss)
            if backward:
                gbuf = self._grad_target(c.grad_names + list(self._out_names()))
                deferred = []
                gate_B = plan.B if (c.top.Hpb is not None and not (plan.B >= ops.RECUR_GEMM_MIN_BATCH[0] and self.hidden_size % 64 == 0)) else None
                dHall = self._vocab_backward(c.top.Hall, logits, gbuf, c.top.Hb, dLb, defer=deferred, gate_B=gate_B)
                if dLb is not None:
                    def loss_and_bucket():
                        with torch.cuda.stream(self._side(0)):
                            ops.reduce_sum(row_loss, N, 1.0 / denom, loss)
                            if early_step is not None and gbuf is self.arena().gflat:
                                self._publish(list(self._out_names()), gbuf)
                                early_step(list(self._out_names()))
                    if deferred:
                        deferred.append(loss_and_bucket)
                    else:
                        loss_and_bucket()
                self.__dict__["_after_recur"] = deferred
                if grad_hook is not None and gbuf is self.arena().gflat:
                    self._run_deferred()
                    self._join()
                    grad_hook(list(self._out_names()))
                need_dfeat = features is not None and features.requires_grad
                self.__dict__["_bucket_hook"] = (gbuf, early_step) if (early_step is not None and gbuf is self.arena().gflat) else None
                try:
                    dfeat = self._run_backward(c, dHall, gbuf, need_dfeat)
                finally:
                    self.__dict__["_bucket_hook"] = None
                self._run_deferred()
                self._join()
                self._publish(c.grad_names + list(self._out_names()), gbuf)
                if grad_hook is not None:
                    grad_hook(c.grad_names if gbuf is self.arena().gflat else c.grad_names + list(self._out_names()))
                if dfeat is not None:
                    features.grad = dfeat if features.grad is None else features.grad + dfeat
        return loss, {"argmax": argmax, "top5hit": top5, "n_tokens": N}

    def _default_targets(self, captions, plan, has_feat, out=None):
        d = plan.dev(captions.device)
        key = "tgt_idx_%d_%d" % (captions.shape[1], 0 if has_feat else 1)
        idx = d.get(key)
        if idx is None:
            idx = (d["row_b"].long() * captions.shape[1] + d["row_t"].long() + (0 if has_feat else 1)).contiguous()
            d[key] = idx
        if out is not None:
            return torch.index_select(captions.reshape(-1), 0, idx, out=out)
        return captions.reshape(-1).index_select(0, idx)


V_CAST_SIDE = [os.environ.get("SN_V_CAST_SIDE", "1") == "1"]


class DecoderFactoredLSTM(_DecoderBase):

    cell = ops.CELL_FACTORED

    def __init__(self, embed_size, hidden_size, factored_size, vocab_size, num_layers, feature_size=2048,
                 bias=True, dropout=0.22, max_seq_length=40):
        super().__init__()
        if not bias:
            raise NotImplementedError("bias=False is not supported by the fused path")
        self.feature_size, self.hidden_size = feature_size, hidden_size
        self.factored_size, self.embed_size = factored_size, embed_size
        self.vocab_size, self.max_seq_length = vocab_size, max_seq_length
        self.num_layers = num_layers
        self.dropout = nn.Dropout(dropout)
        self.B = nn.Embedding(vocab_size, embed_size)
        for g in GATES:
            setattr(self, "U_" + g, nn.Linear(factored_size, hidden_size, bias=bias))
            setattr(self, style_attr("factual", g), nn.Linear(factored_size, factored_size, bias=bias))
            setattr(self, "V_" + g, nn.Linear(embed_size, factored_size, bias=bias))
            setattr(self, "W_" + g, nn.Linear(hidden_size, hidden_size, bias=bias))
        for s in STYLES[1:]:
            for g in GATES:
                setattr(self, style_attr(s, g), nn.Linear(factored_size, factored_size, bias=bias))
        self.C = nn.Linear(hidden_size, vocab_size, bias=bias)
        _ref_init(self, self.B, self.C)

    def _arena_groups(self):
        groups = [["B.weight"]]
        for pre in ("V_", "U_", "W_"):
            groups.append([pre + g + ".weight" for g in GATES])
            groups.append([pre + g + ".bias" for g in GATES])
        for s in STYLES:
            groups.append([style_attr(s, g) + ".weight" for g in GATES])
            groups.append([style_attr(s, g) + ".bias" for g in GATES])
        groups += [["C.weight"], ["C.bias"]]
        return groups

    def _emb(self):
        return self.B

    def _emb_name(self):
        return "B.weight"

    def _out(self):
        return self.C

    def _out_names(self):
        return ("C.weight", "C.bias")

    @staticmethod
    def _lp(layer):
        return "" if layer == 0 else "l%d_" % layer

    def _stack(self, pre, shape, grad=False, gbuf=None, bias=False, layer=0):
        names = [self._lp(layer) + pre + g + (".bias" if bias else ".weight") for g in GATES]
        if gbuf is not None:
            return self._gview(gbuf, names, shape)
        return self.arena().block(names, shape, grad=grad)

    def _style_stack(self, mode, shape, gbuf=None, bias=False, layer=0):
        names = [self._lp(layer) + style_attr(mode, g) + (".bias" if bias else ".weight") for g in GATES]
        if gbuf is not None:
            return self._gview(gbuf, names, shape)
        return self.arena().block(names, shape)

    def _shadow_specs(self, c, mode):
        H, F = self.hidden_size, self.factored_size
        early, late = super()._shadow_specs(c, mode)
        if mode in STYLES:
            if V_CAST_SIDE[0]:
                c.first_specs = [(c.w16, "V", self._stack("V_", (4 * F, c.Ein)))]
                c.second_specs = [(c.w16, "S", self._style_stack(mode, (4 * F, F)))]
                early = [(c.w16, "U", self._stack("U_", (4 * H, F)))]
            else:
                early = [(c.w16, "S", self._style_stack(mode, (4 * F, F))), (c.w16, "U", self._stack("U_", (4 * H, F)))]
        return early, late

    def _recurrent_weights(self, layer=0):
        H = self.hidden_size
        return self._stack("W_", (4 * H, H), layer=layer), self._stack("W_", (4 * H,), bias=True, layer=layer)

    def _recurrent_grads(self, gbuf, layer=0):
        H = self.hidden_size
        return (self._stack("W_", (4 * H, H), gbuf=gbuf, layer=layer),
                self._stack("W_", (4 * H,), gbuf=gbuf, bias=True, layer=layer))

    def _seq_grad_names(self, mode):
        names = ["B.weight"]
        for pre in ("V_", "U_", "W_"):
            names += [pre + g + sfx for g in GATES for sfx in (".weight", ".bias")]
        names += [style_attr(mode, g) + sfx for g in GATES for sfx in (".weight", ".bias")]
        return names

    def _input_projection(self, c, X, mode, r0, n):
        if mode not in STYLES:
            raise ValueError("mode name wrong: %r (expected one of %s)" % (mode, STYLES))
        H, F = self.hidden_size, self.factored_size
        Ein = X.shape[1] if X is not None else c.Ein
        dev = c.XP.device
        full = (r0 == 0 and n == c.XP.shape[0])
        if full and not self.bf16:
            c.A1 = torch.empty(n, 4 * F, dtype=torch.float32, device=dev)
            c.A2 = torch.empty(n, 4 * F, dtype=torch.float32, device=dev)
        A1, A2 = c.__dict__.get("A1"), c.__dict__.get("A2")
        L = getattr(c, "layer", 0)
        Vc, bV = self._stack("V_", (4 * F, Ein), layer=L), self._stack("V_", (4 * F,), bias=True, layer=L)
        Sc, bS = self._style_stack(mode, (4 * F, F), layer=L), self._style_stack(mode, (4 * F,), bias=True, layer=L)
        Uc, bU = self._stack("U_", (4 * H, F), layer=L), self._stack("U_", (4 * H,), bias=True, layer=L)
        if self.bf16:
            w16 = c.__dict__.setdefault("w16", {})
            if "V" not in w16:
                w16["V"] = self._shadow(Vc)
            if "S" not in w16:
                w16["S"], w16["U"] = self._shadow(Sc), self._shadow(Uc)
            Vb, Sb, Ub = w16["V"], w16["S"], w16["U"]
            Ep, Fp = Vb.stride(0), Sb.stride(0)
            if full:
                if X is not None:
                    c.Xb = torch.empty(n, Ep, dtype=torch.bfloat16, device=dev)
                c.A1 = torch.empty(n, 4 * F, dtype=torch.bfloat16, device=dev)
                c.A2 = torch.empty(n, 4 * F, dtype=torch.bfloat16, device=dev)
            if X is not None:
                ops.cast_bf16(X, n, Ein, Ein, c.Xb, Ep, Ep, src_off=r0 * Ein, dst_off=r0 * Ep)
            ev = c.__dict__.get("ev_first")
            if ev is not None:
                torch.cuda.current_stream().wait_event(ev)
                c.ev_first = None
            ops.gemm_bf16(ops.OP_NT, c.Xb, Vb, n, 4 * F, Ep, Ep, Ep, Cb=c.A1, ldcb=4 * F, bias=bV, a_off=r0 * Ep,
                          cb_off=r0 * 4 * F)
            ev2 = c.__dict__.get("ev_second")
            ev = c.__dict__.get("ev_early")
            if ev2 is not None:
                torch.cuda.current_stream().wait_event(ev2)
                c.ev_second = None
            elif ev is not None:
                torch.cuda.current_stream().wait_event(ev)
                c.ev_early = ev = None
            ops.gemm_bf16(ops.OP_NT, c.A1, Sb, n, F, F, 4 * F, Fp, Cb=c.A2, ldcb=4 * F, bias=bS, batch=4, sA=F,
                          sB=F * Fp, sCb=F, sBias=F, a_off=r0 * 4 * F, cb_off=r0 * 4 * F)
            if ev is not None:
                torch.cuda.current_stream().wait_event(ev)
                c.ev_early = None
            ops.gemm_bf16(ops.OP_NT, c.A2, Ub, n, H, F, 4 * F, Fp, C=c.XP, ldc=4 * H, bias=bU, batch=4, sA=F,
                          sB=H * Fp, sC=H, sBias=H, a_off=r0 * 4 * F, c_off=r0 * 4 * H)
            return
        ops.gemm(ops.OP_NT, X, Vc, A1, n, 4 * F, Ein, Ein, Ein, 4 * F, bias=bV, a_off=r0 * Ein,
                 c_off=r0 * 4 * F)
        ops.gemm(ops.OP_NT, A1, Sc, A2, n, F, F, 4 * F, F, 4 * F, bias=bS, batch=4, sA=F, sB=F * F, sC=F,
                 sBias=F, a_off=r0 * 4 * F, c_off=r0 * 4 * F)
        ops.gemm(ops.OP_NT, A2, Uc, c.XP, n, H, F, 4 * F, F, 4 * H, bias=bU, batch=4, sA=F, sB=H * F, sC=H,
                 sBias=H, a_off=r0 * 4 * F, c_off=r0 * 4 * H)

    def _input_projection_bwd(self, c, dZ, gbuf):
        H, F = self.hidden_size, self.factored_size
        N, Ein = dZ.shape[0], c.Ein
        dev = dZ.device
        mode = c.mode
        L = getattr(c, "layer", 0)
        Vc = self._stack("V_", (4 * F, Ein), layer=L)
        Sc = self._style_stack(mode, (4 * F, F), layer=L)
        Uc = self._stack("U_", (4 * H, F), layer=L)
        gV, gbV = (self._stack("V_", (4 * F, Ein), gbuf=gbuf, layer=L),
                   self._stack("V_", (4 * F,), gbuf=gbuf, bias=True, layer=L))
        gS, gbS = (self._style_stack(mode, (4 * F, F), gbuf=gbuf, layer=L),
                   self._style_stack(mode, (4 * F,), gbuf=gbuf, bias=True, layer=L))
        gU, gbU = (self._stack("U_", (4 * H, F), gbuf=gbuf, layer=L),
                   self._stack("U_", (4 * H,), gbuf=gbuf, bias=True, layer=L))
        if self.bf16:
            return self._input_projection_bwd_bf16(c, dZ, gV, gbV, gS, gbS, gU, gbU)
        ops.gemm(ops.OP_TN, dZ, c.A2, gU, H, F, N, 4 * H, 4 * F, F, batch=4, sA=H, sB=F, sC=H * F)
        ops.colsum(dZ, N, 4 * H, 4 * H, gbU)
        dA2 = torch.empty(N, 4 * F, dtype=torch.float32, device=dev)
        ops.gemm(ops.OP_NN, dZ, Uc, dA2, N, F, H, 4 * H, F, 4 * F, batch=4, sA=H, sB=H * F, sC=F)
        ops.gemm(ops.OP_TN, dA2, c.A1, gS, F, F, N, 4 * F, 4 * F, F, batch=4, sA=F, sB=F, sC=F * F)
        ops.colsum(dA2, N, 4 * F, 4 * F, gbS)
        dA1 = torch.empty(N, 4 * F, dtype=torch.float32, device=dev)
        ops.gemm(ops.OP_NN, dA2, Sc, dA1, N, F, F, 4 * F, F, 4 * F, batch=4, sA=F, sB=F * F, sC=F)
        ops.gemm(ops.OP_TN, dA1, c.X, gV, 4 * F, Ein, N, 4 * F, Ein, Ein)
        ops.colsum(dA1, N, 4 * F, 4 * F, gbV)
        dX = torch.empty(N, Ein, dtype=torch.float32, device=dev)
        ops.gemm(ops.OP_NN, dA1, Vc, dX, N, Ein, 4 * F, 4 * F, Ein, Ein)
        return dX

    def _input_projection_bwd_bf16(self, c, dZ, gV, gbV, gS, gbS, gU, gbU):
        H, F = self.hidden_size, self.factored_size
        N, Ein = dZ.shape[0], c.Ein
        dev = dZ.device
        Vb, Sb, Ub = c.w16["V"], c.w16["S"], c.w16["U"]
        Ep, Fp = Vb.stride(0), Sb.stride(0)
        dZb = c.dZb
        f32 = dict(dtype=torch.float32, device=dev)
        b16 = dict(dtype=torch.bfloat16, device=dev)
        main = torch.cuda.current_stream()
        sa, sb = self._side(0), self._side(1)
        dA2, dA2b = torch.empty(N, 4 * F, **f32), torch.empty(N, 4 * F, **b16)
        dA1, dA1b = torch.empty(N, 4 * F, **f32), torch.empty(N, 4 * F, **b16)
        dX = torch.empty(N, Ein, **f32)
        L = getattr(c, "layer", 0)
        lp = self._lp(L)
        sa.wait_stream(main)
        with torch.cuda.stream(sa):
            ops.gemm_bf16(ops.OP_TN, dZb, c.A2, H, F, N, 4 * H, 4 * F, C=gU, ldc=F, batch=4, sA=H, sB=F, sC=H * F)
            wide = bool(ops.TAIL_SCHEDULE[0])
            if getattr(c, "colsum_dZ", None) is not None:
                gbU.copy_(c.colsum_dZ)
            else:
                ops.colsum(dZ, N, 4 * H, 4 * H, gbU, wide=wide)
            self._bucket_final([lp + pre + g + sfx for pre in ("W_", "U_") for g in GATES for sfx in (".weight", ".bias")])
        ops.gemm_bf16(ops.OP_NN, dZb, Ub, N, F, H, 4 * H, Fp, C=dA2, ldc=4 * F, Cb=dA2b, ldcb=4 * F, batch=4, sA=H,
                      sB=H * Fp, sC=F, sCb=F)
        sb.wait_stream(main)
        with torch.cuda.stream(sb):
            ops.gemm_bf16(ops.OP_TN, dA2b, c.A1, F, F, N, 4 * F, 4 * F, C=gS, ldc=F, batch=4, sA=F, sB=F, sC=F * F)
            ops.colsum(dA2, N, 4 * F, 4 * F, gbS, wide=wide)
        ops.gemm_bf16(ops.OP_NN, dA2b, Sb, N, F, F, 4 * F, Fp, C=dA1, ldc=4 * F, Cb=dA1b, ldcb=4 * F, batch=4, sA=F,
                      sB=F * Fp, sC=F, sCb=F)
        sb.wait_stream(main)
        with torch.cuda.stream(sb):
            ops.gemm_bf16(ops.OP_TN, dA1b, c.Xb, 4 * F, Ein, N, 4 * F, Ep, C=gV, ldc=Ein)
            ops.colsum(dA1, N, 4 * F, 4 * F, gbV, wide=wide)
            self._bucket_final([lp + style_attr(c.mode, g) + sfx for g in GATES for sfx in (".weight", ".bias")] +
                               [lp + "V_" + g + sfx for g in GATES for sfx in (".weight", ".bias")])
        ops.gemm_bf16(ops.OP_NN, dA1b, Vb, N, Ein, 4 * F, 4 * F, Ep, C=dX, ldc=Ein)
        return dX

    def _collapse_chain(self, ctx, mode, layer=0):
        if mode not in STYLES:
            raise ValueError("mode name wrong: %r (expected one of %s)" % (mode, STYLES))
        H, F = self.hidden_size, self.factored_size
        Ein = self._chain_in(layer)
        col = ctx.__dict__.setdefault("collapsed", {})
        ent = col.get(layer)
        key = (mode, self.arena().content_key())
        if ent is not None and ent.get("key") == key:
            return ent
        if ent is None or ent["Wc"].shape != (4 * H, Ein):
            f32 = dict(dtype=torch.float32, device=self.B.weight.device)
            ent = col[layer] = {"Wc": torch.empty(4 * H, Ein, **f32), "bc": torch.empty(4 * H, **f32),
                                "SV": torch.empty(4 * F, Ein, **f32), "t": torch.empty(4 * F, **f32)}
        self._collapse_into(mode, layer, ent["Wc"], ent["bc"], ent["SV"], ent["t"])
        ent["mode"], ent["key"] = mode, key
        return ent

    def _chain_in(self, layer):
        return self.arena().named[self._lp(layer) + "V_" + GATES[0] + ".weight"].shape[1]

    def _collapse_into(self, mode, layer, Wc, bc, SV, t):
        H, F = self.hidden_size, self.factored_size
        Ein = Wc.shape[1]
        Vc, bV = self._stack("V_", (4 * F, Ein), layer=layer), self._stack("V_", (4 * F,), bias=True, layer=layer)
        Sc, bS = self._style_stack(mode, (4 * F, F), layer=layer), self._style_stack(mode, (4 * F,), bias=True, layer=layer)
        Uc, bU = self._stack("U_", (4 * H, F), layer=layer), self._stack("U_", (4 * H,), bias=True, layer=layer)
        with torch.no_grad():
            ops.gemm(ops.OP_NN, Sc, Vc, SV, F, Ein, F, F, Ein, Ein, batch=4, sA=F * F, sB=F * Ein, sC=F * Ein)
            ops.gemm(ops.OP_NN, Uc, SV, Wc, H, Ein, F, F, Ein, Ein, batch=4, sA=H * F, sB=F * Ein, sC=H * Ein)
            ops.gemm(ops.OP_NN, Sc, bV, t, F, 1, F, F, 1, 1, batch=4, sA=F * F, sB=F, sC=F)
            t.add_(bS)
            ops.gemm(ops.OP_NN, Uc, t, bc, H, 1, F, F, 1, 1, batch=4, sA=H * F, sB=F, sC=H)
            bc.add_(bU)

    def _collapse_styles(self, ctx, styles, layer=0):
        for mode in styles:
            if mode not in STYLES:
                raise ValueError("mode name wrong: %r (expected one of %s)" % (mode, STYLES))
        H, F = self.hidden_size, self.factored_size
        Ein, G = self._chain_in(layer), len(styles)
        col = ctx.__dict__.setdefault("collapsed_groups", {})
        ent = col.get(layer)
        key = (tuple(styles), self.arena().content_key())
        if ent is not None and ent.get("key") == key:
            return ent
        if ent is None or ent["Wc"].shape != (G, 4 * H, Ein):
            f32 = dict(dtype=torch.float32, device=self.B.weight.device)
            ent = col[layer] = {"Wc": torch.empty(G, 4 * H, Ein, **f32), "bc": torch.empty(G, 4 * H, **f32),
                                "SV": torch.empty(4 * F, Ein, **f32), "t": torch.empty(4 * F, **f32)}
        for g, mode in enumerate(styles):
            self._collapse_into(mode, layer, ent["Wc"][g], ent["bc"][g], ent["SV"], ent["t"])
        ent["key"] = key
        return ent

    def _small_step(self, ctx, X, mode, R, h_prev, c_prev, src_row, h_out, c_out, layer=0, x_rows=None):
        if mode not in STYLES:
            raise ValueError("mode name wrong: %r (expected one of %s)" % (mode, STYLES))
        H, F = self.hidden_size, self.factored_size
        Ein = X.shape[1]
        ent = ctx.__dict__.get("collapsed", {}).get(layer)
        if ent is not None and ent.get("mode") == mode and ent["Wc"].shape[1] == Ein:
            Whh, bhh = self._recurrent_weights(layer)
            ops.decode_cell(self.cell, H, R, ent["Wc"], Ein, X, 0, ent["bc"], Whh, bhh, h_prev, c_prev, src_row, h_out,
                            c_out, x_rows=x_rows)
            return
        a1, a2 = ctx.__dict__.get("sk_a1"), ctx.__dict__.get("sk_a2")
        if a1 is None or a1.shape[0] < R:
            a1 = ctx.sk_a1 = torch.empty(max(R, ops.SKINNY_MAX_ROWS), 4 * F, dtype=torch.float32, device=X.device)
            a2 = ctx.sk_a2 = torch.empty_like(a1)
        ops.skinny_linear(self._stack("V_", (4 * F, Ein), layer=layer), X, a1, R,
                          bias=self._stack("V_", (4 * F,), bias=True, layer=layer), x_rows=x_rows)
        Sc = self._style_stack(mode, (4 * F, F), layer=layer)
        bS = self._style_stack(mode, (4 * F,), bias=True, layer=layer)
        if F % 32 == 0:
            ops.skinny_linear(Sc, a1, a2, R, bias=bS, group_n=F, group_x=F)
        else:
            for g in range(4):
                ops.skinny_linear(Sc[g * F:(g + 1) * F], a1[:, g * F:(g + 1) * F], a2[:, g * F:(g + 1) * F], R,
                                  bias=bS[g * F:(g + 1) * F])
        Whh, bhh = self._recurrent_weights(layer)
        ops.decode_cell(self.cell, H, R, self._stack("U_", (4 * H, F), layer=layer), F, a2, F,
                        self._stack("U_", (4 * H,), bias=True, layer=layer), Whh, bhh, h_prev, c_prev, src_row, h_out, c_out)

    def forward(self, captions, lengths, features=None, teacher_forcing_ratio=0.8, mode="factual"):
        if mode not in STYLES:
            raise ValueError("mode name wrong: %r (expected one of %s)" % (mode, STYLES))
        if self._greedy_eligible(captions, lengths, features, teacher_forcing_ratio):
            return self._forward_greedy(captions, lengths, features, mode)
        hall, _ = self._forward_hidden(captions, lengths, features, teacher_forcing_ratio, mode)
        return _LogitsFn.apply(hall, self.C.weight, self)

    def forward_step(self, embedded, states, mode):
        from .decode import single_step
        return single_step(self, embedded, states, mode)

    def sample(self, features, start_token, end_token, k=5, factual_limit=-1, mode="factual",
               feed_image=False):
        from .decode import beam_sample, require_one_style
        require_one_style(mode)
        return beam_sample(self, features, start_token, end_token, k, mode, feed_image)[0]

    def sample_batch(self, features, start_token, end_token, k=5, mode="factual", feed_image=False):
        from .decode import beam_sample
        return beam_sample(self, features, start_token, end_token, k, mode, feed_image)


class DecoderRNN(_DecoderBase):

    cell = ops.CELL_LSTM

    def __init__(self, embed_size, hidden_size, vocab_size, num_layers, feature_size=2048, dropout=0.22,
                 max_seq_length=40):
        super().__init__()
        self.feature_size, self.hidden_size, self.embed_size = feature_size, hidden_size, embed_size
        self.vocab_size, self.max_seq_length = vocab_size, max_seq_length
        self.num_layers = num_layers
        self.dropout = nn.Dropout(dropout)
        self.embed = nn.Embedding(vocab_size, embed_size)
        self.lstm = nn.LSTMCell(embed_size, hidden_size, bias=True)
        self.linear = nn.Linear(hidden_size, vocab_size)
        _ref_init(self, self.embed, self.linear)

    def _arena_groups(self):
        return [["embed.weight"], ["lstm.weight_ih"], ["lstm.weight_hh"], ["lstm.bias_ih"], ["lstm.bias_hh"],
                ["linear.weight"], ["linear.bias"]]

    def _emb(self):
        return self.embed

    def _emb_name(self):
        return "embed.weight"

    def _out(self):
        return self.linear

    def _out_names(self):
        return ("linear.weight", "linear.bias")

    def _recurrent_weights(self, layer=0):
        self.arena()
        return self.lstm.weight_hh, self.lstm.bias_hh

    def _recurrent_grads(self, gbuf, layer=0):
        H = self.hidden_size
        return self._gview(gbuf, ["lstm.weight_hh"], (4 * H, H)), self._gview(gbuf, ["lstm.bias_hh"], (4 * H,))

    def _seq_grad_names(self, mode):
# ... 63 lines not shown
```

image-caption-emotion-indonesia_b200/dp.py:

```python
import os
import re

import torch
import torch.distributed as dist

from . import ops


def merged_ranges(arena, names, max_gap=64):
    spans = sorted((arena.offset[n], arena.numel[n]) for n in names)
    out = []
    for o, n in spans:
        if out and o - (out[-1][0] + out[-1][1]) < max_gap:
            out[-1] = (out[-1][0], o + n - out[-1][0])
        else:
            out.append((o, n))
    return out


class GradSync:

    def __init__(self, group=None):
        self.group = group
        self.pending = []
# ... 12 lines not shown
            w.wait()
        self.pending = []


class PeerExchange:

    _opened = {}
    N_PADS = 16

    def pads(self, bucket):
        if not 0 <= bucket < self.N_PADS:
            raise RuntimeError("too many exchange buckets in one step")
        return [p + 128 * bucket for p in self.pad_ptrs]

    def __init__(self, arena, group=None, grad_dtype=None):
        from . import ops
        self.world = dist.get_world_size(group)
        self.rank = dist.get_rank(group)
        if self.world > 8:
            raise RuntimeError("peer exchange supports one NVSwitch box (<= 8 ranks)")
        dev = arena.flat.device
        self.pad = torch.zeros(32 * self.N_PADS, dtype=torch.int32, device=dev)
        grad_dtype = grad_dtype or torch.float32
        self.elem_size = 2 if grad_dtype == torch.bfloat16 else 4
        self.slot_elems = ops.dp_slot_elems(arena.flat.numel(), self.world)
        self.recv = torch.zeros(self.world * self.slot_elems, dtype=grad_dtype, device=dev)
        torch.cuda.synchronize()
        mine = [ops.ipc_export(t) for t in (arena.flat, arena.gflat, self.pad, self.recv)]
        gathered = [None] * self.world
        dist.all_gather_object(gathered, (self.rank, dev.index, mine), group=group)
        self.param_ptrs, self.grad_ptrs, self.pad_ptrs = [0] * self.world, [0] * self.world, [0] * self.world
        self.recv_ptrs = [0] * self.world
        for r, dev_index, exports in gathered:
            if r == self.rank:
                ptrs = [t.data_ptr() for t in (arena.flat, arena.gflat, self.pad, self.recv)]
            else:
                ops.enable_peer_access(dev_index)
                ptrs = []
                for handle, offset in exports:
                    base = PeerExchange._opened.get(handle)
                    if base is None:
                        base = ops.ipc_open(handle)
                        PeerExchange._opened[handle] = base
                    ptrs.append(base + offset)
            self.param_ptrs[r], self.grad_ptrs[r], self.pad_ptrs[r], self.recv_ptrs[r] = ptrs
        self.arena_version = arena.version
        self.keep = (arena.flat, arena.gflat, self.pad, self.recv)
        torch.cuda.synchronize()
        dist.barrier(group=group)


EARLY_PEER_EXCHANGE = [True]
PEER_FORM = [os.environ.get("SN_DP_FORM", "push")]
BG_PUSH_SMS = [int(os.environ.get("SN_DP_BG_PUSH_SMS", "16"))]
BG_RECV_CTAS = [int(os.environ.get("SN_DP_BG_RECV_CTAS", "0"))]
BG_WU = [os.environ.get("SN_DP_BG_WU", "0") == "1"]
PEER_BUCKETS = [False]


def tail_schedule(world, bucketed):
    return bool(ops.TAIL_SCHEDULE[0]) and world == 1 and bool(bucketed)


class DataParallelTrainer:

    def __init__(self, decoder, optimizer, group=None, comm=None):
        self.decoder, self.optimizer = decoder, optimizer
        self.group = group
        self.world = dist.get_world_size(group) if dist.is_initialized() else 1
        self.sync = GradSync(group)
        if comm is None:
            comm = "peer" if (self.world > 1 and dist.get_backend(group) == "nccl") else "nccl"
        self.comm = comm
        self.peers = None

    def _peers(self):
        a = self.decoder.arena()
        dt = torch.bfloat16 if os.environ.get("SN_DP_GRAD_BF16") == "1" else torch.float32
        if self.peers is None or self.peers.arena_version != a.version or self.peers.recv.dtype != dt:
            self.peers = PeerExchange(a, self.group, grad_dtype=dt)
        return self.peers

    def _step_push(self, captions, lengths, features, n_global, b_global, bucketed, kw):
        peers = self._peers()
        opt = self.optimizer
        done = []
        if bucketed:
            out_names = set(self.decoder._out_names())
            calls = [0]

            def early_step(names):
                is_out = out_names.issuperset(names)
                is_wu = BG_WU[0] and bool(names) and all(re.match(r"(l\d+_)?[WU]_", n) for n in names)
                if not (is_out or is_wu) or calls[0] >= PeerExchange.N_PADS - 1:
                    return
                b = calls[0]
                bg = self.decoder._side(3)
                bg.wait_stream(torch.cuda.current_stream())
                with torch.cuda.stream(bg):
                    if opt.push_peer(peers, only=names, bucket=b, max_ctas=BG_PUSH_SMS[0]):
                        opt.step_peer_recv(peers, [b], only=names, max_ctas=BG_RECV_CTAS[0])
                        calls[0] += 1
                        done.extend(names)
            kw = dict(kw, early_step=early_step)
        loss, stats = self.forward_backward(captions, lengths, features, n_global=n_global, b_global=b_global, **kw)
        last = PeerExchange.N_PADS - 1
        if opt.push_peer(peers, skip=done or None, bucket=last):
            opt.step_peer_recv(peers, [last], skip=done or None)
        return loss, stats

    def forward_backward(self, captions, lengths, features, n_global=None, b_global=None, grad_hook=None, **kw):
        dec = self.decoder
        a = dec.arena()
        N_local = sum(int(l) for l in lengths)
        if n_global is None:
            n_global = N_local * self.world
        for p in a.named.values():
            p.grad = None
        extra = {}
        if b_global is not None or hasattr(dec, "attention"):
            extra["b_global"] = b_global if b_global is not None else len(lengths) * self.world
        return dec.forward_loss(captions, lengths, features, n_global=n_global, grad_hook=grad_hook, **extra, **kw)

    def step(self, captions, lengths, features, n_global=None, b_global=None, **kw):
        a = self.decoder.arena()
        bucketed = getattr(self.decoder, "bf16", False) and not hasattr(self.decoder, "attention") and EARLY_PEER_EXCHANGE[0]
        if self.world > 1 and self.comm == "peer" and PEER_FORM[0] == "push":
            return self._step_push(captions, lengths, features, n_global, b_global, bucketed, kw)
        if self.world > 1 and self.comm == "peer":
            peers = self._peers()
            early = []
            if bucketed:
                calls = [0]
                out_names = set(self.decoder._out_names())

                def early_step(names):
                    if not PEER_BUCKETS[0] and not out_names.issuperset(names):
                        return
                    self.optimizer.step_peer(peers, only=names, bucket=calls[0])
                    calls[0] += 1
                    early.extend(names)
                kw = dict(kw, early_step=early_step)
            loss, stats = self.forward_backward(captions, lengths, features, n_global=n_global, b_global=b_global, **kw)
            self.optimizer.step_peer(peers, skip=early or None, bucket=PeerExchange.N_PADS - 1)
            return loss, stats
        hook = None
        if self.world > 1:
            def hook(names):
                self.sync.launch(a.gflat, merged_ranges(a, names))
        early = []
        if self.world == 1 and bucketed:
            tail = tail_schedule(self.world, bucketed)
            emb = getattr(self.decoder, "_emb_name", lambda: None)()

            def early_step(names):
                cap = ops.ADAM_BG_CTAS[0] if (tail and list(names) != [emb]) else 0
                self.optimizer.step(only=names, max_ctas=cap)
                early.extend(names)
            kw = dict(kw, early_step=early_step, early_embed=tail)
        loss, stats = self.forward_backward(captions, lengths, features, n_global=n_global, b_global=b_global,
                                            grad_hook=hook, **kw)
        if self.world > 1:
            self.sync.wait()
        self.optimizer.step(skip=early or None)
        return loss, stats
```

image-caption-emotion-indonesia_b200/ops.py:

```python
import ctypes

import torch

from . import _lib
from ._lib import OP_NN, OP_NT, OP_TN, CELL_FACTORED, CELL_LSTM
from ._lib import check as _check


def check(rc, what=""):
    _check(rc, what)
    if what != "sn_device_info":
        LAUNCHES[0] += 1


LAUNCHES = [0]


class no_gc_during_capture:

    def __enter__(self):
        import gc
        gc.collect()
        self.was = gc.isenabled()
        gc.disable()
# ... 23 lines not shown
def lib():
    l = _lib.load()
    _lib.require_device(torch.cuda.current_device())
    return l


FP32_GEMM = ["split"]
SPLIT_MIN_MACS = 1 << 22
SPLIT_MAX_ACC_K = 768


def _pad8(n):
    return (n + 7) // 8 * 8


def _split_cols(X, off, rows, K, ld, batch, s, pattern):
    Kp = _pad8(K)
    if batch > 1 and s < ld:
        if s != K or ld < batch * K:
            return None
        G, R = batch, rows
    elif batch > 1:
        if s != rows * ld:
            return None
        G, R = 1, rows * batch
    else:
        G, R = 1, rows
    out = torch.empty(R, G * 6 * Kp, dtype=torch.bfloat16, device=X.device)
    check(lib().sn_split_limbs_cols(ctypes.c_void_p(X.data_ptr() + 4 * off), R, G, K, ld, _ptr(out), Kp, pattern,
                                    _stream()), "sn_split_limbs_cols")
    return out, G * 6 * Kp, (6 * Kp if G > 1 else rows * 6 * Kp)


def _split_rows(X, off, K, cols, ld, batch, s, pattern):
    Kp, ldp = _pad8(K), _pad8(ld)
    if batch > 1 and s < ld:
        if s % 8 != 0:
            return None
        G = 1
    elif batch > 1:
        if s != K * ld:
            return None
        G = batch
    else:
        G = 1
    out = torch.empty(G * 6 * Kp, ldp, dtype=torch.bfloat16, device=X.device)
    check(lib().sn_split_limbs_rows(ctypes.c_void_p(X.data_ptr() + 4 * off), G, K, ld, ld, _ptr(out), Kp, ldp, pattern,
                                    _stream()), "sn_split_limbs_rows")
    return out, ldp, (s if (batch > 1 and s < ld) else 6 * Kp * ldp)


def _gemm_split(op, A, B, C, M, N, K, lda, ldb, ldc, bias, beta, batch, sA, sB, sC, sBias, a_off, b_off, c_off,
                bias_off):
    if K > 10900:
        return False
    Kp6 = 6 * _pad8(K)
    splits = 1
    if K > SPLIT_MAX_ACC_K:
        if M < 256 or N % 4 != 0:
            return False
        splits = -(-Kp6 // SPLIT_MAX_ACC_K)
        while splits > 1 and M * N * batch * splits * 4 > (1 << 30):
            splits -= 1
    ea = _split_cols(A, a_off, M, K, lda, batch, sA, 0) if op in (OP_NT, OP_NN) else _split_rows(A, a_off, K, M, lda, batch, sA, 0)
    if ea is None:
        return False
    eb = _split_cols(B, b_off, N, K, ldb, batch, sB, 1) if op == OP_NT else _split_rows(B, b_off, K, N, ldb, batch, sB, 1)
    if eb is None:
        return False
    LAUNCHES[0] += 2
    gemm_bf16(op, ea[0], eb[0], M, N, Kp6, ea[1], eb[1], C=C, ldc=ldc, bias=bias, beta=beta, batch=batch,
              sA=ea[2] if batch > 1 else 0, sB=eb[2] if batch > 1 else 0, sC=sC, sBias=sBias, c_off=c_off,
              bias_off=bias_off, splits=splits if splits > 1 else 1, impl="pair" if splits > 1 else None)
    return True


def gemm(op, A, B, C, M, N, K, lda, ldb, ldc, bias=None, beta=0.0, batch=1, sA=0, sB=0, sC=0, sBias=0,
         a_off=0, b_off=0, c_off=0, bias_off=0):
    _req(A); _req(B); _req(C)
    if (FP32_GEMM[0] == "split" and M * N * K * batch >= SPLIT_MIN_MACS and M >= 256 and N >= 16 and K >= 16
            and batch <= 4 and ldc % 4 == 0 and c_off % 4 == 0 and (batch == 1 or sC % 4 == 0)
            and _gemm_split(op, A, B, C, M, N, K, lda, ldb, ldc, bias, beta, batch, sA, sB, sC, sBias, a_off, b_off,
                            c_off, bias_off)):
        return C
    pa = ctypes.c_void_p(A.data_ptr() + 4 * a_off)
    pb = ctypes.c_void_p(B.data_ptr() + 4 * b_off)
    pc = ctypes.c_void_p(C.data_ptr() + 4 * c_off)
    pbias = ctypes.c_void_p(bias.data_ptr() + 4 * bias_off) if bias is not None else None
    check(lib().sn_gemm(op, M, N, K, pa, lda, pb, ldb, pc, ldc, pbias, float(beta), batch, sA, sB, sC, sBias,
                        _stream()), "sn_gemm")
    return C


def linear_nt(x, w, bias=None, out=None):
    M, K = x.shape
    N = w.shape[0]
    if out is None:
        out = torch.empty(M, N, device=x.device, dtype=torch.float32)
    return gemm(OP_NT, x, w, out, M, N, K, x.stride(0), w.stride(0), out.stride(0), bias=bias)


def colsum(X, M, N, ldx, out, beta=0.0, x_off=0, out_off=0, wide=False):
    _req(X); _req(out)
    check(lib().sn_colsum_ex(ctypes.c_void_p(X.data_ptr() + 4 * x_off), M, N, ldx,
                             ctypes.c_void_p(out.data_ptr() + 4 * out_off), float(beta), 1 if wide else 0, _stream()),
          "sn_colsum")
    return out


def gather_pack_fwd(captions, table, features, has_feat, row_b, row_t, tok_override, N, X, p_drop, seed,
                    row_off=0, seed_dev=None, Xb=None):
    E = table.shape[1]
    cap = _req(captions, torch.int64)
    ro4 = 4 * row_off
    check(lib().sn_gather_pack_fwd(
        _ptr(cap), cap.stride(0), _ptr(_req(table)), E,
        _ptr(features) if features is not None else None, features.stride(0) if features is not None else 0,
        1 if has_feat else 0,
        ctypes.c_void_p(row_b.data_ptr() + ro4), ctypes.c_void_p(row_t.data_ptr() + ro4),
        ctypes.c_void_p(tok_override.data_ptr() + ro4) if tok_override is not None else None,
        N, ctypes.c_void_p(X.data_ptr() + 4 * row_off * X.stride(0)) if X is not None else None,
        X.stride(0) if X is not None else 0, float(p_drop), ctypes.c_uint64(seed), _ptr(seed_dev),
        ctypes.c_void_p(Xb.data_ptr() + 2 * row_off * Xb.stride(0)) if Xb is not None else None,
        Xb.stride(0) if Xb is not None else 0, _stream()), "sn_gather_pack_fwd")


def colsum_bf16(X, M, N, ldx, out, beta=0.0, wide=False):
    _req(X, torch.bfloat16); _req(out)
    check(lib().sn_colsum_bf16_ex(_ptr(X), M, N, ldx, _ptr(out), float(beta), 1 if wide else 0, _stream()),
          "sn_colsum_bf16")
    return out


def gather_pack_bwd(captions, dtable, dfeatures, has_feat, row_b, row_t, tok_override, N, dX, p_drop, seed,
                    seed_dev=None):
    V, E = dtable.shape
    cap = _req(captions, torch.int64)
    ws_int = torch.empty(4 * V + 1 + 3 * N, dtype=torch.int32, device=dX.device)
    ws_part = torch.empty((N // 16 + 1) * E, dtype=torch.float32, device=dX.device)
    check(lib().sn_gather_pack_bwd(
        _ptr(cap), cap.stride(0), _ptr(_req(dtable)), E,
        _ptr(dfeatures) if dfeatures is not None else None,
        dfeatures.stride(0) if dfeatures is not None else 0, 1 if has_feat else 0,
        _ptr(row_b), _ptr(row_t), _ptr(tok_override) if tok_override is not None else None,
        N, _ptr(_req(dX)), dX.stride(0), float(p_drop), ctypes.c_uint64(seed), _ptr(seed_dev),
        V, _ptr(ws_int), _ptr(ws_part), _stream()),
          "sn_gather_pack_bwd")


def embed_plan_ws(V, N, device):
    return torch.empty(4 * V + 1 + 3 * N, dtype=torch.int32, device=device)


def embed_plan(captions, has_feat, row_b, row_t, tok_override, N, V, ws_int):
    cap = _req(captions, torch.int64)
    check(lib().sn_embed_plan(_ptr(cap), cap.stride(0), 1 if has_feat else 0, _ptr(row_b), _ptr(row_t),
                              _ptr(tok_override) if tok_override is not None else None, N, V, _ptr(_req(ws_int, torch.int32)),
                              _stream()), "sn_embed_plan")


def embed_grad(dtable, dfeatures, has_feat, row_b, row_t, tok_override, N, dX, p_drop, seed, ws_int, seed_dev=None,
               wide=True):
    V, E = dtable.shape
    ws_part = torch.empty((N // 16 + 1) * E, dtype=torch.float32, device=dX.device)
    check(lib().sn_embed_grad(
        _ptr(_req(dtable)), E, _ptr(dfeatures) if dfeatures is not None else None,
        dfeatures.stride(0) if dfeatures is not None else 0, 1 if has_feat else 0, _ptr(row_b), _ptr(row_t),
        _ptr(tok_override) if tok_override is not None else None, N, _ptr(_req(dX)), dX.stride(0), float(p_drop),
        ctypes.c_uint64(seed), _ptr(seed_dev), V, _ptr(_req(ws_int, torch.int32)), _ptr(ws_part), 1 if wide else 0, _stream()),
          "sn_embed_grad")


_ws_cache = {}


def _recur_ws(device, T):
    key = (device, T)
    ws = _ws_cache.get(key)
    if ws is None:
        nbytes = lib().sn_recur_ws_bytes(1, T)
        ws = torch.empty(nbytes // 4 + 1, dtype=torch.int32, device=device)
        _ws_cache[key] = ws
    return ws


def recur_fwd(cell, H, B, bs, off, t0, t1, XP, Whh, bhh, h_init, Hall, Call, Hprev, gates, c_state):
    ws = _recur_ws(XP.device, t1 + 1)
    check(lib().sn_recur_fwd(cell, H, B, _ptr(bs), _ptr(off), t0, t1, _ptr(_req(XP)), _ptr(_req(Whh)),
                             _ptr(h_init), _ptr(bhh), _ptr(Hall), _ptr(Call), _ptr(Hprev), _ptr(gates),
                             _ptr(c_state), _ptr(ws), _stream()), "sn_recur_fwd")


def recur_bwd(cell, H, B, bs, off, t0, t1, Whh, c_init, Call, gates, dHall, dZ, dh_carry, dc_carry):
    ws = _recur_ws(dZ.device, t1 + 1)
    check(lib().sn_recur_bwd(cell, H, B, _ptr(bs), _ptr(off), t0, t1, _ptr(_req(Whh)), _ptr(c_init),
                             _ptr(Call), _ptr(gates), _ptr(_req(dHall)), _ptr(dZ), _ptr(dh_carry),
                             _ptr(dc_carry), _ptr(ws), _stream()), "sn_recur_bwd")


def softmax_nll(logits, N, V, targets=None, row_loss=None, dlogits=None, grad_scale=1.0, argmax=None,
                top5hit=None, row_off=0, dlogits_bf16=None):
    ld = logits.stride(0)
    check(lib().sn_softmax_nll(
        ctypes.c_void_p(logits.data_ptr() + 4 * row_off * ld), N, V, ld, _ptr(targets), _ptr(row_loss),
        _ptr(dlogits), dlogits.stride(0) if dlogits is not None else 0, float(grad_scale), _ptr(argmax),
        _ptr(top5hit), _ptr(dlogits_bf16), dlogits_bf16.stride(0) if dlogits_bf16 is not None else 0,
        _stream()), "sn_softmax_nll")


def reduce_sum(x, N, scale, out, accumulate=False):
    check(lib().sn_reduce_sum(_ptr(_req(x)), N, float(scale), _ptr(out), 1 if accumulate else 0, _stream()),
          "sn_reduce_sum")


def adam_clamp(p, g, m, v, ranges, step_sizes, bc2_sqrts, beta1, beta2, eps, clip):
    n = len(ranges)
    if n == 0:
        return
    R = (ctypes.c_int64 * (2 * n))()
    S = (ctypes.c_float * n)()
    C = (ctypes.c_float * n)()
    for i, (o, l) in enumerate(ranges):
        R[2 * i], R[2 * i + 1] = o, l
        S[i], C[i] = step_sizes[i], bc2_sqrts[i]
    check(lib().sn_adam_clamp(_ptr(_req(p)), _ptr(_req(g)), _ptr(_req(m)), _ptr(_req(v)), n,
                              ctypes.cast(R, ctypes.c_void_p), ctypes.cast(S, ctypes.c_void_p),
                              ctypes.cast(C, ctypes.c_void_p), beta1, beta2, eps, clip, _stream()),
          "sn_adam_clamp")


def mean_pixels(feat, B, P, D, out):
    check(lib().sn_mean_pixels(_ptr(_req(feat)), B, P, D, _ptr(out), _stream()), "sn_mean_pixels")


def _att_b16_ok(feat_b16, att1, A, D):
    return (feat_b16 is not None and D == 2048 and A % 4 == 0 and feat_b16.data_ptr() % 16 == 0
            and att1.data_ptr() % 16 == 0)


def att_step_fwd(att1, att2, feat, wfull, bfull, gate_pre, nb, P, A, D, alpha, ld_alpha, ctx, ldc, feat_b16=None):
    if _att_b16_ok(feat_b16, att1, A, D) and ldc % 2 == 0:
        check(lib().sn_att_step_fwd_b16(_ptr(_req(att1)), _ptr(_req(att2)), _ptr(_req(feat_b16, torch.bfloat16)),
                                        _ptr(_req(wfull)), float(bfull), _ptr(_req(gate_pre)), nb, P, A, D, _ptr(alpha),
                                        ld_alpha, _ptr(ctx), ldc, _stream()), "sn_att_step_fwd_b16")
        return
    check(lib().sn_att_step_fwd(_ptr(_req(att1)), _ptr(_req(att2)), _ptr(_req(feat)), _ptr(_req(wfull)),
                                float(bfull), _ptr(_req(gate_pre)), nb, P, A, D, _ptr(alpha), ld_alpha,
                                _ptr(ctx), ldc, _stream()), "sn_att_step_fwd")


def att_step_bwd(att1, att2, feat, wfull, bfull, gate_pre, alpha, ld_alpha, dctx, ldc, dalpha_extra, ld_da,
                 nb, P, A, D, datt2, dgate_pre, datt1, dwfull, dfeat, feat_b16=None):
    if dfeat is None and _att_b16_ok(feat_b16, att1, A, D) and datt1.data_ptr() % 16 == 0:
        check(lib().sn_att_step_bwd_b16(_ptr(_req(att1)), _ptr(_req(att2)), _ptr(_req(feat_b16, torch.bfloat16)),
                                        _ptr(_req(wfull)), _ptr(_req(gate_pre)), _ptr(alpha), ld_alpha, _ptr(_req(dctx)),
                                        ldc, _ptr(dalpha_extra), ld_da, nb, P, A, D, _ptr(datt2), _ptr(dgate_pre),
                                        _ptr(datt1), _ptr(dwfull), _stream()), "sn_att_step_bwd_b16")
        LAUNCHES[0] += 1
        return
    check(lib().sn_att_step_bwd(_ptr(_req(att1)), _ptr(_req(att2)), _ptr(_req(feat)), _ptr(_req(wfull)),
                                float(bfull), _ptr(_req(gate_pre)), _ptr(alpha), ld_alpha, _ptr(_req(dctx)), ldc,
                                _ptr(dalpha_extra), ld_da, nb, P, A, D, _ptr(datt2), _ptr(dgate_pre),
                                _ptr(datt1), _ptr(dwfull), _ptr(dfeat), _stream()), "sn_att_step_bwd")


def _bptr(t, off_elems, elem_size):
    return ctypes.c_void_p(t.data_ptr() + elem_size * off_elems) if t is not None else None


GEMM_IMPL = ["auto"]
_SM_PAIRS = 74


def _pick_splits(M, N, K, batch):
    tiles = ((M + 255) // 256) * ((N + 255) // 256) * batch
    kb = (K + 63) // 64
    if tiles * 2 > _SM_PAIRS or kb < 64:
        return 1
    return max(1, min(_SM_PAIRS // tiles, kb // 8, 16))


_g2_ws = {}


def _gemm2_ws(device, nbytes):
    key = (device, torch.cuda.current_stream().cuda_stream)
    ws = _g2_ws.get(key)
    if ws is None or ws.numel() * 4 < nbytes:
        ws = torch.empty(nbytes // 4 + 4, dtype=torch.float32, device=device)
        _g2_ws[key] = ws
    return ws


def gemm_bf16(op, A, B, M, N, K, lda, ldb, C=None, ldc=0, Cb=None, ldcb=0, bias=None, beta=0.0, batch=1,
              sA=0, sB=0, sC=0, sCb=0, sBias=0, a_off=0, b_off=0, c_off=0, cb_off=0, bias_off=0, splits=1,
              impl=None, max_pairs=0):
    _req(A, torch.bfloat16); _req(B, torch.bfloat16)
    impl = impl or GEMM_IMPL[0]
    if impl == "pair" or (impl == "auto" and M >= 256):
        sp = _pick_splits(M, N, K, batch) if splits in (0, 1) else splits
        if sp > 1 and N % 4 != 0:
            sp = 1
        ws, wsb = None, 0
        if sp > 1:
            wsb = lib().sn_gemm2_ws_bytes(M, N, batch, sp)
            ws = _gemm2_ws(A.device, wsb)
            LAUNCHES[0] += batch
        check(lib().sn_gemm2_bf16(op, M, N, K, _bptr(A, a_off, 2), lda, _bptr(B, b_off, 2), ldb,
                                  _bptr(C, c_off, 4), ldc, _bptr(Cb, cb_off, 2), ldcb, _bptr(bias, bias_off, 4),
                                  float(beta), batch, sA, sB, sC, sCb, sBias, sp, _ptr(ws), wsb, int(max_pairs),
                                  _stream()), "sn_gemm2_bf16")
        return
    check(lib().sn_gemm_bf16_splitk(op, M, N, K, _bptr(A, a_off, 2), lda, _bptr(B, b_off, 2), ldb,
                                    _bptr(C, c_off, 4), ldc, _bptr(Cb, cb_off, 2), ldcb, _bptr(bias, bias_off, 4),
                                    float(beta), batch, sA, sB, sC, sCb, sBias, splits, _stream()), "sn_gemm_bf16")


def vocab_nll_fwd(Hb, Wb, bias, targets, N, V, H, tlogit, lse, row_loss=None, argmax=None, above=None):
    _req(Hb, torch.bfloat16); _req(Wb, torch.bfloat16); _req(targets, torch.int64)
    nbytes = lib().sn_vocab_ws_bytes(N, V)
    ws = _gemm2_ws(Hb.device, nbytes)
    check(lib().sn_vocab_nll_fwd(N, V, H, _ptr(Hb), Hb.stride(0), _ptr(Wb), Wb.stride(0), _ptr(_req(bias)),
                                 _ptr(targets), _ptr(ws), nbytes, _ptr(tlogit), _ptr(lse), _ptr(row_loss),
                                 _ptr(argmax), _ptr(above), _stream()), "sn_vocab_nll_fwd")
    LAUNCHES[0] += 1


def vocab_nll_bwd(Hb, Wb, bias, targets, N, V, H, tlogit, lse, grad_scale, dLb=None, above=None, top5hit=None):
    _req(Hb, torch.bfloat16); _req(Wb, torch.bfloat16); _req(targets, torch.int64)
    check(lib().sn_vocab_nll_bwd(N, V, H, _ptr(Hb), Hb.stride(0), _ptr(Wb), Wb.stride(0), _ptr(_req(bias)),
                                 _ptr(targets), _ptr(tlogit), _ptr(lse), float(grad_scale), _ptr(dLb),
                                 dLb.stride(0) if dLb is not None else 0, _ptr(above), _ptr(top5hit), _stream()),
          "sn_vocab_nll_bwd")
    if top5hit is not None:
        LAUNCHES[0] += 1


def cast_bf16(src, R, C, lds, dst, Cp, ldd, src_off=0, dst_off=0, max_blocks=0):
    check(lib().sn_cast_bf16_ex(_bptr(_req(src), src_off, 4), R, C, lds, _bptr(dst, dst_off, 2), Cp, ldd, max_blocks,
                                _stream()), "sn_cast_bf16")


def to_bf16_padded(x, pad_to=8):
    R, C = x.shape
    Cp = (C + pad_to - 1) // pad_to * pad_to
    out = torch.empty(R, Cp, dtype=torch.bfloat16, device=x.device)
    cast_bf16(x, R, C, x.stride(0), out, Cp, Cp)
    return out


import os as _os
DC_SCHEDULE = [int(_os.environ.get("SN_DC_SCHEDULE", "0"))]
DC_MAX_PAIRS = [int(_os.environ.get("SN_DC_MAX_PAIRS", "37"))]

TAIL_SCHEDULE = [int(_os.environ.get("SN_TAIL_SCHEDULE", "1"))]
ADAM_BG_CTAS = [int(_os.environ.get("SN_ADAM_BG_CTAS", "0"))]

GATE_DC = [int(_os.environ.get("SN_GATE_DC", "0"))]

RECUR_IMPL = ["auto"]
_cl_max = {}


def recur_cluster_ok(H, B):
    impl = RECUR_IMPL[0]
    if impl == "flags" or H not in (128, 256, 512):
        return False
    key = (torch.cuda.current_device(), H)
    n = _cl_max.get(key)
    if n is None:
        n = _cl_max[key] = int(lib().sn_recur_cl_max_clusters(H))
    if impl == "cluster":
        if n < 1:
            raise _lib.SnError("cluster form of the recurrence is not available for H=%d on this device" % H)
        return True
    return n >= 1 and (B + 15) // 16 <= n


def recur_fwd_bf16(cell, H, B, bs, off, t0, t1, XP, Whh_b, bhh, h_init, Hall, Hb, Hprevb, Call, gates, c_state):
    if recur_cluster_ok(H, B):
        check(lib().sn_recur_fwd_cl(cell, H, B, _ptr(bs), _ptr(off), t0, t1, _ptr(_req(XP)),
                                    _ptr(_req(Whh_b, torch.bfloat16)), _ptr(bhh), _ptr(h_init), _ptr(Hall),
                                    _ptr(_req(Hb, torch.bfloat16)), _ptr(Hprevb), _ptr(Call), _ptr(gates),
                                    _ptr(c_state), _stream()), "sn_recur_fwd_cl")
        return
    ws = _recur_ws(XP.device, t1 + 1)
    check(lib().sn_recur_fwd_bf16(cell, H, B, _ptr(bs), _ptr(off), t0, t1, _ptr(_req(XP)),
                                  _ptr(_req(Whh_b, torch.bfloat16)), _ptr(bhh), _ptr(h_init), _ptr(Hall),
                                  _ptr(_req(Hb, torch.bfloat16)), _ptr(Hprevb), _ptr(Call), _ptr(gates),
                                  _ptr(c_state), _ptr(ws), _stream()), "sn_recur_fwd_bf16")


def recur_bwd_bf16(cell, H, B, bs, off, t0, t1, Whh_b, c_init, Call, gates, dHall, dZ, dZb, dh_carry, dc_carry,
                   start_flag=None):
    if recur_cluster_ok(H, B):
        check(lib().sn_recur_bwd_cl(cell, H, B, _ptr(bs), _ptr(off), t0, t1, _ptr(_req(Whh_b, torch.bfloat16)),
                                    _ptr(c_init), _ptr(Call), _ptr(gates), _ptr(_req(dHall)), _ptr(dZ),
                                    _ptr(_req(dZb, torch.bfloat16)), _ptr(dh_carry), _ptr(dc_carry), _ptr(start_flag),
                                    _stream()), "sn_recur_bwd_cl")
        return
    ws = _recur_ws(dZb.device, t1 + 1)
    check(lib().sn_recur_bwd_bf16(cell, H, B, _ptr(bs), _ptr(off), t0, t1, _ptr(_req(Whh_b, torch.bfloat16)),
                                  _ptr(c_init), _ptr(Call), _ptr(gates), _ptr(_req(dHall)), _ptr(dZ),
                                  _ptr(_req(dZb, torch.bfloat16)), _ptr(dh_carry), _ptr(dc_carry), _ptr(ws),
                                  _stream()), "sn_recur_bwd_bf16")


RECUR_GEMM_MIN_BATCH = [1024]


def _host_steps(plan):
    hs = plan.__dict__.get("_host_steps")
    if hs is None:
        T = plan.T
        hs = ((ctypes.c_int32 * T)(*[int(x) for x in plan.bs]), (ctypes.c_int32 * T)(*[int(x) for x in plan.off[:T]]))
        plan.__dict__["_host_steps"] = hs
    return hs


_zeros_b16 = {}


def _zeros_bf16(device, n):
    z = _zeros_b16.get(device)
    if z is None or z.numel() < n:
        z = torch.zeros(n, dtype=torch.bfloat16, device=device)
        _zeros_b16[device] = z
    return z


def cast_gate_interleave(W):
    H4, K = W.shape
    H = H4 // 4
    Kp = (K + 7) // 8 * 8
    out = torch.empty(H4, Kp, dtype=torch.bfloat16, device=W.device)
    check(lib().sn_cast_bf16_gate_interleave(_ptr(_req(W)), H, K, W.stride(0), _ptr(out), Kp, _stream()),
          "sn_cast_bf16_gate_interleave")
    return out


def recur_fwd_gemm(cell, H, B, plan, XP, Wp, bhh, Hall, Hb, Call, gates):
    bs_h, off_h = _host_steps(plan)
    z = _zeros_bf16(XP.device, max(B * H, 4 * H))
    check(lib().sn_recur_fwd_gemm(cell, H, B, ctypes.cast(bs_h, ctypes.c_void_p), ctypes.cast(off_h, ctypes.c_void_p),
                                  plan.T, _ptr(_req(XP)), _ptr(_req(Wp, torch.bfloat16)), _ptr(bhh), _ptr(Hall),
                                  _ptr(_req(Hb, torch.bfloat16)), _ptr(_req(Call)), _ptr(gates), _ptr(z), _stream()),
          "sn_recur_fwd_gemm")
    LAUNCHES[0] += plan.T - 1


def recur_hprev(Hb, d, N, H, Hprevb):
    check(lib().sn_recur_hprev(_ptr(_req(Hb, torch.bfloat16)), _ptr(d["row_b"]), _ptr(d["row_t"]), _ptr(d["off"]), N, H,
                               _ptr(_req(Hprevb, torch.bfloat16)), _stream()), "sn_recur_hprev")


def recur_bwd_gemm(cell, H, B, plan, Whh_b, Call, gates, dHall, dZ, dZb, dc_carry):
    bs_h, off_h = _host_steps(plan)
    z = _zeros_bf16(dZb.device, max(B * H, 4 * H))
    check(lib().sn_recur_bwd_gemm(cell, H, B, ctypes.cast(bs_h, ctypes.c_void_p), ctypes.cast(off_h, ctypes.c_void_p),
                                  plan.T, _ptr(_req(Whh_b, torch.bfloat16)), _ptr(_req(Call)), _ptr(_req(gates)),
                                  _ptr(_req(dHall)), _ptr(dZ), _ptr(_req(dZb, torch.bfloat16)), _ptr(_req(dc_carry)),
                                  _ptr(z), _stream()), "sn_recur_bwd_gemm")
    LAUNCHES[0] += plan.T


def adam_clamp_dev(p, g, m, v, ranges, step_idx, steps_dev, lr_dev, coef_ws, beta1, beta2, eps, clip, max_ctas=0):
    n = len(ranges)
    for i0 in range(0, n, 48):
        k = min(48, n - i0)
        R = (ctypes.c_int64 * (2 * k))()
        S = (ctypes.c_int32 * k)()
        for i in range(k):
            R[2 * i], R[2 * i + 1] = ranges[i0 + i]
            S[i] = step_idx[i0 + i]
        check(lib().sn_adam_clamp_dev_ex(_ptr(_req(p)), _ptr(_req(g)), _ptr(_req(m)), _ptr(_req(v)), k,
                                         ctypes.cast(R, ctypes.c_void_p), ctypes.cast(S, ctypes.c_void_p),
                                         _ptr(steps_dev), _ptr(lr_dev), _ptr(coef_ws), beta1, beta2, eps, clip,
                                         int(max_ctas), _stream()), "sn_adam_clamp_dev")


def enable_peer_access(peer_device):
    _check(lib().sn_enable_peer_access(int(peer_device)), "sn_enable_peer_access")


def dp_adam_fused(world, rank, grad_ptrs, param_ptrs, pad_ptrs, m, v, ranges, step_idx, steps_dev, lr_dev, coef_ws,
                  beta1, beta2, eps, clip):
    if len(ranges) > 48:
        for i0 in range(0, len(ranges), 48):
            dp_adam_fused(world, rank, grad_ptrs, param_ptrs, pad_ptrs, m, v, ranges[i0:i0 + 48],
                          step_idx[i0:i0 + 48], steps_dev, lr_dev, coef_ws, beta1, beta2, eps, clip)
        return
    n = len(ranges)
    G = (ctypes.c_void_p * world)(*grad_ptrs)
    Pp = (ctypes.c_void_p * world)(*param_ptrs)
    D = (ctypes.c_void_p * world)(*pad_ptrs)
    R = (ctypes.c_int64 * (2 * max(n, 1)))()
    S = (ctypes.c_int32 * max(n, 1))()
    for i in range(n):
        R[2 * i], R[2 * i + 1] = ranges[i]
        S[i] = step_idx[i]
    check(lib().sn_dp_adam_fused(world, rank, ctypes.cast(G, ctypes.c_void_p), ctypes.cast(Pp, ctypes.c_void_p),
                                 ctypes.cast(D, ctypes.c_void_p), _ptr(_req(m)), _ptr(_req(v)), n,
                                 ctypes.cast(R, ctypes.c_void_p), ctypes.cast(S, ctypes.c_void_p), _ptr(steps_dev),
                                 _ptr(lr_dev), _ptr(coef_ws), beta1, beta2, eps, clip, _stream()), "sn_dp_adam_fused")


DP_MAX_RANGES = 128

# ... 141 lines not shown
```

image-caption-emotion-indonesia_b200/optim.py:

```python
import torch

from . import ops


class FusedClampAdam:
    def __init__(self, decoder, lr=2e-4, betas=(0.9, 0.999), eps=1e-8, grad_clip=0.5, extra_params=()):
        self.decoder = decoder
        self.betas, self.eps, self.grad_clip = betas, float(eps), float(grad_clip)
        self.param_groups = [{"lr": float(lr), "params": list(decoder.parameters()) + list(extra_params)}]
        self._arena_version = -1
        self.m = self.v = None
        self.extra = list(extra_params)
        self.extra_state = {}
        self._lr_on_device = None

    def _state(self):
        a = self.decoder.arena()
        if self._arena_version != a.version or self.m is None:
            dev = a.flat.device
            names = list(a.named)
            if self.m is not None and self.m.numel() == a.total and getattr(self, "names", None) == names:
                self.m, self.v = self.m.to(dev), self.v.to(dev)
                self.steps_dev = self.steps_dev.to(dev)
            else:
                self.m = torch.zeros_like(a.flat)
                self.v = torch.zeros_like(a.flat)
                self.steps_dev = torch.zeros(len(names), dtype=torch.int32, device=dev)
            self.names = names
            self.index = {n: i for i, n in enumerate(self.names)}
            self.lr_dev = torch.zeros(1, dtype=torch.float32, device=dev)
            self.coef_ws = torch.zeros(2 * len(self.names) + 2, dtype=torch.float32, device=dev)
            self._lr_on_device = None
            self._arena_version = a.version
        return a

    def _sync_lr(self):
        lr = float(self.param_groups[0]["lr"])
        if self._lr_on_device != lr:
            self.lr_dev.fill_(lr)
            self._lr_on_device = lr

    def step_counts(self):
        self._state()
        return dict(zip(self.names, self.steps_dev.tolist()))

    def zero_grad(self):
        for p in self.param_groups[0]["params"]:
            p.grad = None

    def __getstate__(self):
        st = self.__dict__.copy()
        st["_lr_on_device"] = None
        return st

    def state_dict(self):
        a = self._state()
        params = self.param_groups[0]["params"]
        by_id = {id(p): n for n, p in a.named.items()}
        steps = self.steps_dev.tolist()
        state = {}
        for i, p in enumerate(params):
            n = by_id.get(id(p))
            if n is not None:
                st = self.extra_state.get(("arena", n))
                if st is not None and int(st["step"].item()) > 0:
                    state[i] = {"step": st["step"].float().reshape(()).clone(), "exp_avg": st["m"].clone(),
                                "exp_avg_sq": st["v"].clone()}
                elif steps[self.index[n]] > 0:
                    o, k = a.offset[n], a.numel[n]
                    state[i] = {"step": torch.tensor(float(steps[self.index[n]])),
                                "exp_avg": self.m[o:o + k].view(p.shape).clone(),
                                "exp_avg_sq": self.v[o:o + k].view(p.shape).clone()}
        for j, p in enumerate(self.extra):
            st = self.extra_state.get(("extra", j))
            if st is not None and int(st["step"].item()) > 0:
                state[len(params) - len(self.extra) + j] = {
                    "step": st["step"].float().reshape(()).clone(), "exp_avg": st["m"].clone(), "exp_avg_sq": st["v"].clone()}
        group = {"lr": self.param_groups[0]["lr"], "betas": tuple(self.betas), "eps": self.eps, "weight_decay": 0,
                 "amsgrad": False, "grad_clip": self.grad_clip, "params": list(range(len(params)))}
        return {"state": state, "param_groups": [group]}

    def load_state_dict(self, sd):
        a = self._state()
        params = self.param_groups[0]["params"]
        group = sd["param_groups"][0]
        if len(group["params"]) != len(params):
            raise ValueError("loaded state dict has a different number of parameters")
        self.param_groups[0]["lr"] = float(group["lr"])
        self.betas, self.eps = tuple(group.get("betas", self.betas)), float(group.get("eps", self.eps))
        by_id = {id(p): n for n, p in a.named.items()}
        self.m.zero_(); self.v.zero_(); self.steps_dev.zero_()
        self.extra_state = {}
        steps = [0] * len(self.names)
        for i, st in sd["state"].items():
            p = params[int(i)]
            n = by_id.get(id(p))
            if n is not None:
                o, k = a.offset[n], a.numel[n]
                self.m[o:o + k].copy_(st["exp_avg"].reshape(-1))
                self.v[o:o + k].copy_(st["exp_avg_sq"].reshape(-1))
                steps[self.index[n]] = int(float(st["step"]))
            else:
                j = int(i) - (len(params) - len(self.extra))
                self.extra_state[("extra", j)] = {
                    "m": st["exp_avg"].to(p.device).clone(), "v": st["exp_avg_sq"].to(p.device).clone(),
                    "step": torch.full((1,), int(float(st["step"])), dtype=torch.int32, device=p.device),
                    "coef": torch.zeros(2, dtype=torch.float32, device=p.device)}
        self.steps_dev.copy_(torch.tensor(steps, dtype=torch.int32))
        self._lr_on_device = None

    @torch.no_grad()
    def step(self, only=None, skip=None, max_ctas=0):
        a = self._state()
        self._sync_lr()
        items, foreign = a.grad_ranges()
        if only is not None:
            keep = set(only)
            items = [it for it in items if it[2] in keep]
            foreign = [n for n in foreign if n in keep]
        if skip is not None:
            drop = set(skip)
            items = [it for it in items if it[2] not in drop]
            foreign = [n for n in foreign if n not in drop]
        b1, b2 = self.betas
        ranges = [(off, n) for off, n, _ in items]
        idx = [self.index[name] for _, _, name in items]
        a.kernel_epoch += 1
        ops.adam_clamp_dev(a.flat, a.gflat, self.m, self.v, ranges, idx, self.steps_dev, self.lr_dev, self.coef_ws,
                           b1, b2, self.eps, self.grad_clip, max_ctas=max_ctas)
        for name in foreign:
            self._step_tensor(a.named[name], ("arena", name))
        if only is None:
            for i, p in enumerate(self.extra):
                if p.grad is not None:
                    self._step_tensor(p, ("extra", i))

    @torch.no_grad()
    def step_peer(self, peers, only=None, skip=None, bucket=0):
        a = self._state()
        self._sync_lr()
        items, foreign = a.grad_ranges()
        if only is not None:
            keep = set(only)
            items = [it for it in items if it[2] in keep]
        if skip is not None:
            drop = set(skip)
            items = [it for it in items if it[2] not in drop]
        if foreign or any(p.grad is not None for p in self.extra):
            raise RuntimeError("peer-fused step needs every gradient in the arena")
        ranges = [(off, n) for off, n, _ in items]
        idx = [self.index[name] for _, _, name in items]
        if not ranges:
            return
        a.kernel_epoch += 1
        ops.dp_adam_fused(peers.world, peers.rank, peers.grad_ptrs, peers.param_ptrs, peers.pads(bucket), self.m, self.v,
                          ranges, idx, self.steps_dev, self.lr_dev, self.coef_ws, self.betas[0], self.betas[1],
                          self.eps, self.grad_clip)

    def _peer_items(self, only, skip):
        a = self._state()
        items, foreign = a.grad_ranges()
        if only is not None:
            keep = set(only)
            items = [it for it in items if it[2] in keep]
        if skip is not None:
            drop = set(skip)
            items = [it for it in items if it[2] not in drop]
        if foreign or any(p.grad is not None for p in self.extra):
            raise RuntimeError("peer-fused step needs every gradient in the arena")
        return a, items

    @torch.no_grad()
    def push_peer(self, peers, only=None, skip=None, bucket=0, max_ctas=0):
        a, items = self._peer_items(only, skip)
        if not items:
            return False
        ops.dp_push(peers.world, peers.rank, a.gflat, peers.recv_ptrs, peers.slot_elems, peers.elem_size,
                    peers.pads(bucket), [(off, n) for off, n, _ in items], max_ctas=max_ctas)
        return True

    @torch.no_grad()
    def step_peer_recv(self, peers, buckets, only=None, skip=None, max_ctas=0):
        a, items = self._peer_items(only, skip)
        self._sync_lr()
        if not items:
            if buckets:
                raise RuntimeError("step_peer_recv: pushed buckets without gradients")
            return
        ranges = [(off, n) for off, n, _ in items]
        idx = [self.index[name] for _, _, name in items]
        mine = [peers.pads(b)[peers.rank] for b in buckets]
        a.kernel_epoch += 1
        ops.dp_adam_recv(peers.world, peers.rank, a.gflat, peers.param_ptrs, peers.recv, peers.slot_elems,
                         peers.elem_size, peers.pads(buckets[0]), mine, self.m, self.v, ranges, idx, self.steps_dev,
                         self.lr_dev, self.coef_ws, self.betas[0], self.betas[1], self.eps, self.grad_clip,
                         max_ctas=max_ctas)

    def _step_tensor(self, p, key):
        st = self.extra_state.get(key)
        if st is None:
            st = {"m": torch.zeros_like(p.data), "v": torch.zeros_like(p.data),
                  "step": torch.zeros(1, dtype=torch.int32, device=p.device),
                  "coef": torch.zeros(2, dtype=torch.float32, device=p.device)}
            self.extra_state[key] = st
        if not p.data.is_contiguous():
            raise RuntimeError("non-contiguous parameter")
        g = p.grad.contiguous()
        ops.adam_clamp_dev(p.data.view(-1), g.view(-1), st["m"].view(-1), st["v"].view(-1), [(0, p.numel())], [0],
                           st["step"], self.lr_dev, st["coef"], self.betas[0], self.betas[1], self.eps,
                           self.grad_clip)
        if g.data_ptr() != p.grad.data_ptr():
            p.grad.copy_(g.view_as(p.grad))
```

include/sn100.h:

```cpp
#ifndef SN100_H_
#define SN100_H_

#include <stdint.h>

#ifdef __cplusplus
extern "C" {
#endif

#define SN_VERSION 100

#define SN_OP_NT 0
#define SN_OP_NN 1
#define SN_OP_TN 2

#define SN_PREC_F32 0
#define SN_PREC_BF16X6 1
#define SN_PREC_BF16 2

#define SN_CELL_FACTORED 0
#define SN_CELL_LSTM 1

int32_t sn_version(void);
const char* sn_last_error(void);
int32_t sn_device_info(int32_t* sm_count, int32_t* smem_optin, int32_t* cc_major, int32_t* cc_minor);

int32_t sn_gather_pack_fwd(const int64_t* captions, int64_t cap_ld, const float* table, int64_t E,
                           const float* features, int64_t feat_ld, int32_t has_feat,
                           const int32_t* row_b, const int32_t* row_t, const int32_t* tok_override,
                           int64_t N, float* X, int64_t ldx, float p_drop, uint64_t seed,
                           const uint64_t* seed_dev, void* Xb, int64_t ldxb, void* stream);
int32_t sn_gather_pack_bwd(const int64_t* captions, int64_t cap_ld, float* dtable, int64_t E,
                           float* dfeatures, int64_t feat_ld, int32_t has_feat,
                           const int32_t* row_b, const int32_t* row_t, const int32_t* tok_override,
                           int64_t N, const float* dX, int64_t ldx, float p_drop, uint64_t seed,
                           const uint64_t* seed_dev, int64_t V, int32_t* ws_int, float* ws_part, void* stream);
int32_t sn_embed_plan(const int64_t* captions, int64_t cap_ld, int32_t has_feat, const int32_t* row_b,
                      const int32_t* row_t, const int32_t* tok_override, int64_t N, int64_t V, int32_t* ws_int,
                      void* stream);
int32_t sn_embed_grad(float* dtable, int64_t E, float* dfeatures, int64_t feat_ld, int32_t has_feat,
                      const int32_t* row_b, const int32_t* row_t, const int32_t* tok_override, int64_t N,
                      const float* dX, int64_t ldx, float p_drop, uint64_t seed, const uint64_t* seed_dev, int64_t V,
                      const int32_t* ws_int, float* ws_part, int32_t wide, void* stream);

int32_t sn_gemm(int32_t op, int64_t M, int64_t N, int64_t K, const float* A, int64_t lda,
                const float* B, int64_t ldb, float* C, int64_t ldc, const float* bias, float beta,
                int32_t batch, int64_t strideA, int64_t strideB, int64_t strideC, int64_t strideBias,
                void* stream);
int32_t sn_gemm_bf16(int32_t op, int64_t M, int64_t N, int64_t K, const void* A, int64_t lda,
                     const void* B, int64_t ldb, float* C, int64_t ldc, void* Cb, int64_t ldcb,
                     const float* bias, float beta, int32_t batch, int64_t strideA, int64_t strideB,
                     int64_t strideC, int64_t strideCb, int64_t strideBias, void* stream);
int32_t sn_gemm_bf16_splitk(int32_t op, int64_t M, int64_t N, int64_t K, const void* A, int64_t lda,
                            const void* B, int64_t ldb, float* C, int64_t ldc, void* Cb, int64_t ldcb,
                            const float* bias, float beta, int32_t batch, int64_t strideA,
                            int64_t strideB, int64_t strideC, int64_t strideCb, int64_t strideBias,
                            int32_t splits, void* stream);
int64_t sn_gemm2_ws_bytes(int64_t M, int64_t N, int32_t batch, int32_t splits);
int32_t sn_gemm2_bf16(int32_t op, int64_t M, int64_t N, int64_t K, const void* A, int64_t lda,
                      const void* B, int64_t ldb, float* C, int64_t ldc, void* Cb, int64_t ldcb,
                      const float* bias, float beta, int32_t batch, int64_t strideA, int64_t strideB,
                      int64_t strideC, int64_t strideCb, int64_t strideBias, int32_t splits, void* ws,
                      int64_t ws_bytes, int32_t max_pairs, void* stream);
int32_t sn_cast_bf16(const float* src, int64_t R, int64_t C, int64_t lds, void* dst, int64_t Cp,
                     int64_t ldd, void* stream);
int32_t sn_cast_bf16_ex(const float* src, int64_t R, int64_t C, int64_t lds, void* dst, int64_t Cp,
                        int64_t ldd, int32_t max_blocks, void* stream);
int32_t sn_colsum(const float* X, int64_t M, int64_t N, int64_t ldx, float* out, float beta,
                  void* stream);
int32_t sn_colsum_bf16(const void* X, int64_t M, int64_t N, int64_t ldx, float* out, float beta,
                       void* stream);
int32_t sn_colsum_ex(const float* X, int64_t M, int64_t N, int64_t ldx, float* out, float beta, int32_t wide,
                     void* stream);
int32_t sn_colsum_bf16_ex(const void* X, int64_t M, int64_t N, int64_t ldx, float* out, float beta, int32_t wide,
                          void* stream);

int64_t sn_recur_ws_bytes(int64_t B, int64_t T);
int32_t sn_recur_fwd(int32_t cell, int64_t H, int64_t B, const int32_t* batch_sizes,
                     const int32_t* offsets, int32_t t0, int32_t t1, const float* XP,
                     const float* Whh, const float* h_init, const float* bhh, float* Hall,
                     float* Call, float* Hprev, float* gates, float* c_state, void* ws,
                     void* stream);
int32_t sn_recur_bwd(int32_t cell, int64_t H, int64_t B, const int32_t* batch_sizes,
                     const int32_t* offsets, int32_t t0, int32_t t1, const float* Whh,
                     const float* c_init, const float* Call, const float* gates, const float* dHall,
                     float* dZ, float* dh_carry, float* dc_carry, void* ws, void* stream);

int32_t sn_recur_fwd_bf16(int32_t cell, int64_t H, int64_t B, const int32_t* batch_sizes,
                          const int32_t* offsets, int32_t t0, int32_t t1, const float* XP,
                          const void* Whh_bf16, const float* bhh, const float* h_init, float* Hall,
                          void* Hb, void* Hprevb, float* Call, float* gates, float* c_state, void* ws,
                          void* stream);
int32_t sn_recur_bwd_bf16(int32_t cell, int64_t H, int64_t B, const int32_t* batch_sizes,
                          const int32_t* offsets, int32_t t0, int32_t t1, const void* Whh_bf16,
                          const float* c_init, const float* Call, const float* gates,
                          const float* dHall, float* dZ, void* dZb, float* dh_carry, float* dc_carry,
                          void* ws, void* stream);

int32_t sn_recur_cl_max_clusters(int64_t H);
int32_t sn_recur_fwd_cl(int32_t cell, int64_t H, int64_t B, const int32_t* batch_sizes,
                        const int32_t* offsets, int32_t t0, int32_t t1, const float* XP,
                        const void* Whh_bf16, const float* bhh, const float* h_init, float* Hall,
                        void* Hb, void* Hprevb, float* Call, float* gates, float* c_state,
                        void* stream);
int32_t sn_recur_bwd_cl(int32_t cell, int64_t H, int64_t B, const int32_t* batch_sizes,
                        const int32_t* offsets, int32_t t0, int32_t t1, const void* Whh_bf16,
                        const float* c_init, const float* Call, const float* gates,
                        const float* dHall, float* dZ, void* dZb, float* dh_carry, float* dc_carry,
                        int32_t* start_flag, void* stream);
int32_t sn_gate_wait(int32_t* flag3, int64_t timeout_us, void* stream);

int32_t sn_cast_bf16_gate_interleave(const float* W, int64_t H, int64_t K, int64_t ldw, void* Wp,
                                     int64_t ldp, void* stream);
int32_t sn_recur_fwd_gemm(int32_t cell, int64_t H, int64_t B, const int32_t* bs_host,
                          const int32_t* off_host, int32_t T, const float* XP, const void* Wp_bf16,
                          const float* bhh, float* Hall, void* Hb, float* Call, float* gates,
                          const void* zeros_bf16, void* stream);
int32_t sn_recur_hprev(const void* Hb, const int32_t* row_b, const int32_t* row_t,
                       const int32_t* offsets, int64_t N, int64_t H, void* Hprevb, void* stream);
int32_t sn_recur_bwd_gemm(int32_t cell, int64_t H, int64_t B, const int32_t* bs_host,
                          const int32_t* off_host, int32_t T, const void* Whh_bf16, const float* Call,
                          const float* gates, const float* dHall, float* dZ, void* dZb, float* dc_carry,
                          const void* zeros_bf16, void* stream);

int32_t sn_softmax_nll(const float* logits, int64_t N, int64_t V, int64_t ld, const int64_t* targets,
                       float* row_loss, float* dlogits, int64_t ldd, float grad_scale,
                       int64_t* argmax, int32_t* top5hit, void* dlogits_bf16, int64_t lddb, void* stream);
int64_t sn_vocab_ws_bytes(int64_t N, int64_t V);
int32_t sn_vocab_nll_fwd(int64_t N, int64_t V, int64_t H, const void* Hb, int64_t ldh, const void* Wb,
                         int64_t ldw, const float* bias, const int64_t* targets, void* ws, int64_t ws_bytes,
                         float* tlogit, float* lse, float* row_loss, int64_t* argmax, int32_t* above,
                         void* stream);
int32_t sn_vocab_nll_bwd(int64_t N, int64_t V, int64_t H, const void* Hb, int64_t ldh, const void* Wb,
                         int64_t ldw, const float* bias, const int64_t* targets, const float* tlogit,
                         const float* lse, float grad_scale, void* dL, int64_t lddl, int32_t* above,
                         int32_t* top5hit, void* stream);
int32_t sn_reduce_sum(const float* x, int64_t N, float scale, float* out, int32_t accumulate,
                      void* stream);

int32_t sn_adam_clamp(float* p, float* g, float* m, float* v, int32_t n_ranges,
                      const int64_t* ranges, const float* step_size, const float* bc2_sqrt,
                      float beta1, float beta2, float eps, float clip, void* stream);

int32_t sn_adam_clamp_dev(float* p, float* g, float* m, float* v, int32_t n_ranges,
                          const int64_t* ranges, const int32_t* step_idx, int32_t* steps_dev,
                          const float* lr_dev, float* coef_ws, float beta1, float beta2, float eps,
                          float clip, void* stream);
int32_t sn_adam_clamp_dev_ex(float* p, float* g, float* m, float* v, int32_t n_ranges,
                             const int64_t* ranges, const int32_t* step_idx, int32_t* steps_dev,
                             const float* lr_dev, float* coef_ws, float beta1, float beta2, float eps,
                             float clip, int32_t max_ctas, void* stream);

int32_t sn_enable_peer_access(int32_t peer_device);
int32_t sn_ipc_export(const void* ptr, uint8_t* handle64, int64_t* offset);
int32_t sn_ipc_open(const uint8_t* handle64, void** base_out);
int32_t sn_ipc_close(void* base);
int32_t sn_dp_adam_fused(int32_t world, int32_t rank, void* const* grad_ptrs, void* const* param_ptrs,
                         void* const* pad_ptrs, float* m, float* v, int32_t n_ranges,
                         const int64_t* ranges, const int32_t* step_idx, int32_t* steps_dev,
                         const float* lr_dev, float* coef_ws, float beta1, float beta2, float eps,
                         float clip, void* stream);
int64_t sn_dp_slot_elems(int64_t arena_elems, int32_t world);
int32_t sn_dp_push(int32_t world, int32_t rank, const float* grad, void* const* recv_ptrs, int64_t slot_elems,
                   int32_t elem_size, void* const* pad_ptrs, int32_t n_ranges, const int64_t* ranges,
                   int32_t max_ctas, void* stream);
int32_t sn_dp_adam_recv(int32_t world, int32_t rank, float* grad, void* const* param_ptrs, void* recv,
                        int64_t slot_elems, int32_t elem_size, void* const* pad_ptrs, void* const* wait_pads,
                        int32_t n_wait, float* m, float* v, int32_t n_ranges, const int64_t* ranges,
                        const int32_t* step_idx, int32_t* steps_dev, const float* lr_dev, float* coef_ws,
                        float beta1, float beta2, float eps, float clip, int32_t max_ctas, void* stream);

int32_t sn_att_step_fwd(const float* att1, const float* att2, const float* feat, const float* wfull,
                        float bfull, const float* gate_pre, int64_t nb, int64_t P, int64_t A,
                        int64_t D, float* alpha, int64_t ld_alpha, float* ctx, int64_t ldc,
                        void* stream);
int32_t sn_att_step_bwd(const float* att1, const float* att2, const float* feat, const float* wfull,
                        float bfull, const float* gate_pre, const float* alpha, int64_t ld_alpha,
                        const float* dctx, int64_t ldc, const float* dalpha_extra, int64_t ld_da,
                        int64_t nb, int64_t P, int64_t A, int64_t D, float* datt2, float* dgate_pre,
                        float* datt1, float* dwfull, float* dfeat, void* stream);
int32_t sn_mean_pixels(const float* feat, int64_t B, int64_t P, int64_t D, float* out, void* stream);

int32_t sn_beam_step(const float* logits, int64_t ld, int64_t V, int32_t n_img, int32_t kmax,
                     int32_t step, int32_t max_len, int32_t end_token, int32_t* k_live,
                     float* run_score, int32_t* prev_word, int32_t* src_row, int32_t* cur_buf,
                     int32_t* seqs, int32_t* done_seq, int32_t* done_len, float* done_score,
                     int32_t* n_done, int32_t* out_seq, int32_t* out_len, int32_t* n_unfinished,
                     const int32_t* step_dev, void* stream);

int32_t sn_att_step_fwd_b16(const float* att1, const float* att2, const void* feat_bf16, const float* wfull,
                            float bfull, const float* gate_pre, int64_t nb, int64_t P, int64_t A, int64_t D,
                            float* alpha, int64_t ld_alpha, float* ctx, int64_t ldc, void* stream);
int32_t sn_att_step_bwd_b16(const float* att1, const float* att2, const void* feat_bf16, const float* wfull,
                            const float* gate_pre, const float* alpha, int64_t ld_alpha, const float* dctx,
                            int64_t ldc, const float* dalpha_extra, int64_t ld_da, int64_t nb, int64_t P,
                            int64_t A, int64_t D, float* datt2, float* dgate_pre, float* datt1,
// ... 51 lines not shown
```

profiles/tail_ab.py:

```python
import json, os, statistics, subprocess, sys, tempfile
import numpy as np

out = sys.argv[1]
runs = int(sys.argv[2]) if len(sys.argv) > 2 else 5
arms = {"tail0": {"SN_TAIL_SCHEDULE": "0"}, "tail1": {"SN_TAIL_SCHEDULE": "1"}}
for spec in (sys.argv[3].split(",") if len(sys.argv) > 3 and sys.argv[3] else []):
    name, kv = spec.split(":", 1)
    arms[name] = dict(SN_TAIL_SCHEDULE="1", **dict(x.split("=", 1) for x in kv.split(";")))
os.makedirs(out, exist_ok=True)
gpu = subprocess.run(["nvidia-smi", "--query-gpu=name,power.limit,clocks.max.sm", "--format=csv,noheader"],
                     capture_output=True, text=True).stdout.strip()
res = {a: [] for a in arms}
with open(os.path.join(out, "tail_ab_runs.jsonl"), "w") as f:
    for i in range(runs):
        for a, env in arms.items():
            p = subprocess.run([sys.executable, "bench.py", "--no-extras", "--no-cpu-baseline"], capture_output=True,
                               text=True, env=dict(os.environ, **env))
            line = [l for l in p.stdout.splitlines() if l.startswith("{")][-1]
            d = json.loads(line)
            res[a].append(d["ms_per_step"])
            f.write(json.dumps({"arm": a, "env": env, "run": i, "ms_per_step": d["ms_per_step"],
                                "clocks": d.get("clocks"), "gpu": gpu}) + "\n")
            f.flush()
summary = {"gpu": gpu, "runs_per_arm": runs}
for a, v in res.items():
    summary[a] = {"median": statistics.median(v), "min": min(v), "max": max(v), "all": v}
dumps = {}
with tempfile.TemporaryDirectory() as td:
    for a in ("tail0", "tail1"):
        d = os.path.join(td, a)
        subprocess.run([sys.executable, "bench.py", "--no-extras", "--no-cpu-baseline", "--steps", "5",
                        "--dump-outputs", d], capture_output=True, text=True, check=True,
                       env=dict(os.environ, **arms[a]))
        dumps[a] = {n: np.load(os.path.join(d, n)) for n in sorted(os.listdir(d)) if n.endswith(".npy")}
    same = sorted(dumps["tail0"]) == sorted(dumps["tail1"]) and all(
        np.array_equal(dumps["tail0"][n], dumps["tail1"][n]) for n in dumps["tail0"])
summary["dump_outputs_identical"] = bool(same)
summary["dump_outputs_files"] = len(dumps["tail0"])
print(json.dumps(summary))
with open(os.path.join(out, "tail_ab_summary.json"), "w") as f:
    json.dump(summary, f, indent=1)
```

Before: 4.543 million.

## Split embedding Adam into untouched-row and touched-row steps overlapped with backward

```diff
diff --git a/image-caption-emotion-indonesia_b200/_lib.py b/image-caption-emotion-indonesia_b200/_lib.py
--- a/image-caption-emotion-indonesia_b200/_lib.py
+++ b/image-caption-emotion-indonesia_b200/_lib.py
@@ -31,7 +31,10 @@
     "sn_colsum_ex": (_I32, [_P, _I64, _I64, _I64, _P, _F, _I32, _P]),
     "sn_colsum_bf16_ex": (_I32, [_P, _I64, _I64, _I64, _P, _F, _I32, _P]),
     "sn_embed_plan": (_I32, [_P, _I64, _I32, _P, _P, _P, _I64, _I64, _P, _P]),
-    "sn_embed_grad": (_I32, [_P, _I64, _P, _I64, _I32, _P, _P, _P, _I64, _P, _I64, _F, c_uint64, _P, _I64, _P, _P, _I32, _P]),
+    "sn_embed_grad": (_I32, [_P, _I64, _P, _I64, _I32, _P, _P, _P, _I64, _P, _I64, _F, c_uint64, _P, _I64, _P, _P, _I32, _I32, _P]),
+    "sn_embed_touched": (_I32, [_P, _I64, _P, _P]),
+    "sn_embed_adam_untouched": (_I32, [_P, _P, _P, _P, _I64, _I64, _I64, _P, _I32, _P, _P, _P, _F, _F, _F, _F, _I32, _P]),
+    "sn_embed_adam_touched": (_I32, [_P, _P, _P, _P, _I64, _I64, _I64, _P, _P, _P, _I32, _P, _F, _F, _F, _F, _P]),
     "sn_adam_clamp_dev_ex": (_I32, [_P, _P, _P, _P, _I32, _P, _P, _P, _P, _P, _F, _F, _F, _F, _I32, _P]),
     "sn_recur_ws_bytes": (_I64, [_I64, _I64]),
     "sn_recur_fwd": (_I32, [_I32, _I64, _I64, _P, _P, _I32, _I32, _P, _P, _P, _P, _P, _P, _P, _P, _P, _P, _P]),
diff --git a/image-caption-emotion-indonesia_b200/csrc/sn_elementwise.cu b/image-caption-emotion-indonesia_b200/csrc/sn_elementwise.cu
--- a/image-caption-emotion-indonesia_b200/csrc/sn_elementwise.cu
+++ b/image-caption-emotion-indonesia_b200/csrc/sn_elementwise.cu
@@ -356,6 +356,16 @@
 constexpr int ADAM_CHUNK = 4096;
 constexpr int64_t ADAM_MAX_LEN = (1LL << 31) - 2 * ADAM_CHUNK;
 
+__device__ __forceinline__ void adam_elem(float& p, float gi, float& m, float& v, float ss, float bc, float beta1,
+                                          float beta2, float eps, bool vec) {
+  const float mi = __fmaf_rn(1.f - beta1, __fsub_rn(gi, m), m);
+  const float t = __fmul_rn(1.f - beta2, gi);
+  const float vi = vec ? __fmaf_rn(v, beta2, __fmul_rn(gi, t)) : __fmaf_rn(gi, t, __fmul_rn(v, beta2));
+  const float denom = sqrtf(vi) / bc + eps;
+  p = __fmaf_rn(-ss, mi / denom, p);
+  m = mi; v = vi;
+}
+
 __global__ void __launch_bounds__(256) adam_clamp_kernel(float* __restrict__ p, float* __restrict__ g,
                                                          float* __restrict__ m, float* __restrict__ v,
                                                          AdamRanges R, const float* __restrict__ coef, float beta1,
@@ -382,11 +392,7 @@
           float gi = gp[e];
           if (clip > 0.f) gi = fminf(fmaxf(gi, -clip), clip);
           gp[e] = gi;
-          float mi = mp[e] + (1.f - beta1) * (gi - mp[e]);
-          float vi = vp[e] * beta2 + (1.f - beta2) * gi * gi;
-          float denom = sqrtf(vi) / bc + eps;
-          pp[e] = pp[e] - ss * (mi / denom);
-          mp[e] = mi; vp[e] = vi;
+          adam_elem(pp[e], gi, mp[e], vp[e], ss, bc, beta1, beta2, eps, true);
         }
         if (clip > 0.f) *reinterpret_cast<float4*>(g + i) = g4;
         *reinterpret_cast<float4*>(m + i) = m4;
@@ -398,14 +404,91 @@
     for (int64_t i = base + threadIdx.x; i < lim; i += 256) {
       float gi = g[i];
       if (clip > 0.f) { gi = fminf(fmaxf(gi, -clip), clip); g[i] = gi; }
-      float mi = m[i], vi = v[i];
-      mi = mi + (1.f - beta1) * (gi - mi);
-      vi = vi * beta2 + (1.f - beta2) * gi * gi;
-      float denom = sqrtf(vi) / bc + eps;
-      p[i] = p[i] - ss * (mi / denom);
-      m[i] = mi; v[i] = vi;
-    }
-  }
+      float pi = p[i], mi = m[i], vi = v[i];
+      adam_elem(pi, gi, mi, vi, ss, bc, beta1, beta2, eps, false);
+      p[i] = pi; m[i] = mi; v[i] = vi;
+    }
+  }
+}
+
+__device__ __forceinline__ bool adam_vec_path(int64_t off, int64_t j, int64_t n) {
+  return (off & 3) == 0 && j < n / ADAM_CHUNK * ADAM_CHUNK;
+}
+
+__global__ void __launch_bounds__(256) embed_adam_untouched_kernel(float* __restrict__ p, const float* __restrict__ g,
+                                                                   float* __restrict__ m, float* __restrict__ v,
+                                                                   const int32_t* __restrict__ cnt, int64_t V, int E,
+                                                                   int64_t off, const float* __restrict__ coef,
+                                                                   int step_idx, float beta1, float beta2, float eps,
+                                                                   float clip) {
+  const float ss = coef[2 * step_idx], bc = coef[2 * step_idx + 1];
+  const int64_t n = V * E, stride = (int64_t)gridDim.x * blockDim.x;
+  if ((E & 3) == 0 && (((uintptr_t)p | (uintptr_t)g | (uintptr_t)m | (uintptr_t)v) & 15) == 0) {
+    for (int64_t i = ((int64_t)blockIdx.x * blockDim.x + threadIdx.x) * 4; i < n; i += stride * 4) {
+      if (cnt[i / E]) continue;
+      const bool vec = adam_vec_path(off, i, n);
+      float4 g4 = *reinterpret_cast<const float4*>(g + i);
+      float4 m4 = *reinterpret_cast<const float4*>(m + i);
+      float4 v4 = *reinterpret_cast<const float4*>(v + i);
+      float4 p4 = *reinterpret_cast<const float4*>(p + i);
+      float* gp = &g4.x; float* mp = &m4.x; float* vp = &v4.x; float* pp = &p4.x;
+#pragma unroll
+      for (int e = 0; e < 4; ++e) {
+        float gi = gp[e];
+        if (clip > 0.f) gi = fminf(fmaxf(gi, -clip), clip);
+        adam_elem(pp[e], gi, mp[e], vp[e], ss, bc, beta1, beta2, eps, vec);
+      }
+      *reinterpret_cast<float4*>(m + i) = m4;
+      *reinterpret_cast<float4*>(v + i) = v4;
+      *reinterpret_cast<float4*>(p + i) = p4;
+    }
+    return;
+  }
+  for (int64_t i = (int64_t)blockIdx.x * blockDim.x + threadIdx.x; i < n; i += stride) {
+    if (cnt[i / E]) continue;
+    float gi = g[i];
+    if (clip > 0.f) gi = fminf(fmaxf(gi, -clip), clip);
+    float pi = p[i], mi = m[i], vi = v[i];
+    adam_elem(pi, gi, mi, vi, ss, bc, beta1, beta2, eps, adam_vec_path(off, i, n));
+    p[i] = pi; m[i] = mi; v[i] = vi;
+  }
+}
+
+__global__ void __launch_bounds__(512) embed_adam_touched_kernel(float* __restrict__ p, float* __restrict__ g,
+                                                                 float* __restrict__ m, float* __restrict__ v,
+                                                                 const int32_t* __restrict__ cnt,
+                                                                 const int32_t* __restrict__ cstart,
+                                                                 const float* __restrict__ part,
+                                                                 const int32_t* __restrict__ touched, int64_t V, int E,
+                                                                 int64_t off, const float* __restrict__ coef,
+                                                                 int step_idx, float beta1, float beta2, float eps,
+                                                                 float clip) {
+  const float ss = coef[2 * step_idx], bc = coef[2 * step_idx + 1];
+  const int32_t n = touched[0];
+  for (int32_t k = blockIdx.x; k < n; k += gridDim.x) {
+    const int64_t t = touched[1 + k];
+    const int32_t nq = cnt[t] > EB_CHUNK ? (cnt[t] + EB_CHUNK - 1) / EB_CHUNK : 0;
+    const float* src = part + (int64_t)cstart[t] * E;
+    for (int c = threadIdx.x; c < E; c += blockDim.x) {
+      const int64_t i = t * E + c;
+      float gi = g[i];
+      if (nq) {
+        float a = 0.f;
+        for (int32_t q = 0; q < nq; ++q) a += src[(int64_t)q * E + c];
+        gi += a;
+      }
+      if (clip > 0.f) gi = fminf(fmaxf(gi, -clip), clip);
+      if (nq || clip > 0.f) g[i] = gi;
+      float pi = p[i], mi = m[i], vi = v[i];
+      adam_elem(pi, gi, mi, vi, ss, bc, beta1, beta2, eps, adam_vec_path(off, i, V * E));
+      p[i] = pi; m[i] = mi; v[i] = vi;
+    }
+  }
+}
+
+__global__ void embed_touched_kernel(const int32_t* __restrict__ cnt, int64_t V, int32_t* __restrict__ touched) {
+  const int64_t t = (int64_t)blockIdx.x * blockDim.x + threadIdx.x;
+  if (t < V && cnt[t] > 0) touched[1 + atomicAdd(touched, 1)] = (int32_t)t;
 }
 
 struct DpPeers {
@@ -749,7 +832,7 @@
   SN_REQUIRE(ws_int && ws_part, "sn_gather_pack_bwd: null work space");
   if (int32_t rc = sn_embed_plan(captions, cap_ld, has_feat, row_b, row_t, tok_override, N, V, ws_int, stream)) return rc;
   return sn_embed_grad(dtable, E, dfeatures, feat_ld, has_feat, row_b, row_t, tok_override, N, dX, ldx, p_drop, seed,
-                       seed_dev, V, ws_int, ws_part, 0, stream);
+                       seed_dev, V, ws_int, ws_part, 0, 1, stream);
 }
 
 namespace {
@@ -781,7 +864,7 @@
 int32_t sn_embed_grad(float* dtable, int64_t E, float* dfeatures, int64_t feat_ld, int32_t has_feat,
                       const int32_t* row_b, const int32_t* row_t, const int32_t* tok_override, int64_t N,
                       const float* dX, int64_t ldx, float p_drop, uint64_t seed, const uint64_t* seed_dev, int64_t V,
-                      const int32_t* ws_int, float* ws_part, int32_t wide, void* stream) {
+                      const int32_t* ws_int, float* ws_part, int32_t wide, int32_t combine, void* stream) {
   SN_REQUIRE(N >= 0 && N < (int64_t)1 << 30 && E > 0 && ldx >= E && V > 0, "sn_embed_grad: bad dims");
   SN_REQUIRE(p_drop >= 0.f && p_drop < 1.f, "sn_embed_grad: dropout p=%f out of [0,1)", p_drop);
   if (N == 0) return 0;
@@ -801,8 +884,51 @@
     embed_chunk_kernel<<<(unsigned)((N + 7) / 8), 256, 0, st>>>(w.tok32, w.start, w.cstart, w.sorted, V, tok_override,
                                                                  dX, ldx, (int)E, p_drop, inv_keep, seed, seed_dev,
                                                                  dtable, ws_part);
-  embed_combine_kernel<<<(unsigned)((V + 7) / 8), 256, 0, st>>>(w.cnt, w.cstart, V, (int)E, ws_part, dtable);
+  if (combine) embed_combine_kernel<<<(unsigned)((V + 7) / 8), 256, 0, st>>>(w.cnt, w.cstart, V, (int)E, ws_part, dtable);
   return sn::check_launch("sn_embed_grad");
+}
+
+int32_t sn_embed_touched(const int32_t* ws_int, int64_t V, int32_t* touched, void* stream) {
+  SN_REQUIRE(ws_int && touched && V > 0 && V < (int64_t)1 << 30, "sn_embed_touched: bad arguments");
+  cudaStream_t st = (cudaStream_t)stream;
+  SN_CUDA(cudaMemsetAsync(touched, 0, sizeof(int32_t), st));
+  embed_touched_kernel<<<(unsigned)((V + 255) / 256), 256, 0, st>>>(ws_int, V, touched);
+  return sn::check_launch("sn_embed_touched");
+}
+
+int32_t sn_embed_adam_untouched(float* p, const float* g, float* m, float* v, int64_t off, int64_t V, int64_t E,
+                                const int32_t* ws_int, int32_t step_idx, int32_t* steps_dev, const float* lr_dev,
+                                float* coef_ws, float beta1, float beta2, float eps, float clip, int32_t max_ctas,
+                                void* stream) {
+  SN_REQUIRE(p && g && m && v && ws_int && steps_dev && lr_dev && coef_ws, "sn_embed_adam_untouched: null argument");
+  SN_REQUIRE(off >= 0 && V > 0 && E > 0 && V * E < ADAM_MAX_LEN && step_idx >= 0 && max_ctas >= 0,
+             "sn_embed_adam_untouched: bad dims V=%lld E=%lld", (long long)V, (long long)E);
+  cudaStream_t st = (cudaStream_t)stream;
+  AdamRanges R;
+  R.n = 1;
+  R.step_idx[0] = step_idx;
+  adam_prepare_kernel<<<1, AdamRanges::MAX, 0, st>>>(R, steps_dev, lr_dev, coef_ws, beta1, beta2);
+  int64_t cap = (int64_t)sn::dev_info().sm_count * 8;
+  if (max_ctas > 0 && max_ctas < cap) cap = max_ctas;
+  const int64_t blocks = (V * E / 4 + 255) / 256;
+  embed_adam_untouched_kernel<<<(unsigned)(blocks < cap ? blocks : cap), 256, 0, st>>>(
+      p, g, m, v, EmbedWs(const_cast<int32_t*>(ws_int), V, 0).cnt, V, (int)E, off, coef_ws, step_idx, beta1, beta2, eps,
+      clip);
+  return sn::check_launch("sn_embed_adam_untouched");
+}
+
+int32_t sn_embed_adam_touched(float* p, float* g, float* m, float* v, int64_t off, int64_t V, int64_t E,
+                              const int32_t* ws_int,
+                              const float* ws_part, const int32_t* touched, int32_t step_idx, const float* coef_ws,
+                              float beta1, float beta2, float eps, float clip, void* stream) {
+  SN_REQUIRE(p && g && m && v && ws_int && ws_part && touched && coef_ws, "sn_embed_adam_touched: null argument");
+  SN_REQUIRE(off >= 0 && V > 0 && E > 0 && V * E < ADAM_MAX_LEN && step_idx >= 0, "sn_embed_adam_touched: bad dims");
+  EmbedWs w(const_cast<int32_t*>(ws_int), V, 0);
+  const int64_t cap = (int64_t)sn::dev_info().sm_count * 6;
+  const unsigned threads = (unsigned)(E < 512 ? (E + 31) / 32 * 32 : 512);
+  embed_adam_touched_kernel<<<(unsigned)(V < cap ? V : cap), threads, 0, (cudaStream_t)stream>>>(
+      p, g, m, v, w.cnt, w.cstart, ws_part, touched, V, (int)E, off, coef_ws, step_idx, beta1, beta2, eps, clip);
+  return sn::check_launch("sn_embed_adam_touched");
 }
 
 int32_t sn_softmax_nll(const float* logits, int64_t N, int64_t V, int64_t ld, const int64_t* targets,
diff --git a/image-caption-emotion-indonesia_b200/decoders.py b/image-caption-emotion-indonesia_b200/decoders.py
--- a/image-caption-emotion-indonesia_b200/decoders.py
+++ b/image-caption-emotion-indonesia_b200/decoders.py
@@ -82,7 +82,7 @@
 
     _TRANSIENT = ("_greedy_graphs", "_decode_sessions", "_side_streams", "_out_w16", "_out_w16_pref", "_out_w16_ev",
                   "_out_h16", "_seed_dev", "_arena", "_att_cache", "_gate_flag", "_gate_armed", "_after_recur", "_bucket_hook",
-                  "_emb_early")
+                  "_emb_early", "_emb_adam")
 
     def __getstate__(self):
         st = self.__dict__.copy()
@@ -218,19 +218,26 @@
         c.tok_override = None
         if not all_tf:
             c.tok_override = torch.full((N,), -1, dtype=torch.int32, device=dev)
-        c.emb_ws = c.emb_ev = c.emb_zeroed = None
+        c.emb_ws = c.emb_ev = c.emb_zeroed = c.emb_adam = None
+        emb_adam = self.__dict__.pop("_emb_adam", None)
         if self.__dict__.pop("_emb_early", False) and all_tf:
             V = emb.weight.shape[0]
+            c.emb_adam = emb_adam
             c.emb_ws = ops.embed_plan_ws(V, N, dev)
+            c.emb_touched = torch.empty(V + 1, dtype=torch.int32, device=dev) if c.emb_adam is not None else None
             c.emb_zeroed = a.gflat
             gE = self._gview(a.gflat, [self._emb_name()], emb.weight.shape)
             side = self._side(4)
             side.wait_stream(torch.cuda.current_stream())
             with torch.cuda.stream(side):
-                ops.embed_plan(captions, has_feat, d["row_b"], d["row_t"], None, N, V, c.emb_ws)
+                ops.embed_plan(captions, has_feat, d["row_b"], d["row_t"], None, N, V, c.emb_ws, touched=c.emb_touched)
                 gE.zero_()
                 c.emb_ev = torch.cuda.Event()
                 c.emb_ev.record(side)
+                if c.emb_adam is not None:
+                    c.emb_adam.step_untouched_rows(self._emb_name(), c.emb_ws, max_ctas=_UNTOUCHED_CTAS)
+                    c.emb_adam_ev = torch.cuda.Event()
+                    c.emb_adam_ev.record(side)
         c.Ein = E
         c.w16 = {}
         c.ev_early = c.ev_late = c.ev_first = None
@@ -414,15 +421,18 @@
             torch.cuda.current_stream().wait_event(c.emb_ev)
             if gbuf is not c.emb_zeroed:
                 gE.zero_()
-            ops.embed_grad(gE, dfeat, c.has_feat, d["row_b"], d["row_t"], c.tok_override, N, dX, c.p_drop, c.seed,
-                           c.emb_ws, seed_dev=c.seed_dev, wide=True)
+            part = ops.embed_grad(gE, dfeat, c.has_feat, d["row_b"], d["row_t"], c.tok_override, N, dX, c.p_drop,
+                                  c.seed, c.emb_ws, seed_dev=c.seed_dev, wide=True, combine=c.emb_adam is None)
+            if c.emb_adam is not None:
+                torch.cuda.current_stream().wait_event(c.emb_adam_ev)
+                c.emb_adam.step_touched_rows(self._emb_name(), c.emb_ws, part, c.emb_touched)
         else:
             gE.zero_()
             ops.gather_pack_bwd(c.captions, gE, dfeat, c.has_feat, d["row_b"], d["row_t"], c.tok_override, N, dX,
                                 c.p_drop, c.seed, seed_dev=c.seed_dev)
         if dfeat is not None and c.feat_shape is not None:
             dfeat = dfeat.view(c.feat_shape)
-        self._bucket_final([self._emb_name()])
+        self._bucket_final([self._emb_name()], stepped=c.emb_adam is not None)
         return dfeat
 
     def _run_deferred(self):
@@ -430,14 +440,17 @@
         for fn in todo or ():
             fn()
 
-    def _bucket_final(self, names):
+    def _bucket_final(self, names, stepped=False):
         hook = self.__dict__.get("_bucket_hook")
         if hook is None:
             return
         gbuf, fn = hook
         names = [n for n in names if n in self.arena().named]
         self._publish(names, gbuf)
-        fn(names)
+        if stepped:
+            fn(names, stepped=True)
+        else:
+            fn(names)
 
     def _gview(self, gbuf, names, shape):
         a = self.arena()
@@ -460,7 +473,7 @@
             return logits
         return ops.linear_nt(Hall.contiguous(), out.weight, out.bias)
 
-    def _vocab_backward(self, Hall, dlogits, gbuf, Hb=None, dLb=None, defer=None, gate_B=None):
+    def _vocab_backward(self, Hall, dlogits, gbuf, Hb=None, dLb=None, defer=None, gate_B=None, split=False):
         out = self._out()
         V, H = out.weight.shape
         N = Hall.shape[0]
@@ -480,10 +493,20 @@
                 Wb = ops.to_bf16_padded(out.weight)
             if have_b16:
                 mode_dc = ops.DC_SCHEDULE[0] if defer is not None else 0
-                side = self._side(0)
+                side = self._side(5 if split else 0)
                 if mode_dc != 2:
                     side.wait_stream(torch.cuda.current_stream())
                 ops.gemm_bf16(ops.OP_NN, dLb, Wb, N, H, V, dLb.stride(0), Wb.stride(0), C=dHall, ldc=H)
+                if split:
+                    self._side(6).wait_stream(torch.cuda.current_stream())
+
+                    def bias_sum():
+                        with torch.cuda.stream(self._side(6)):
+                            ops.colsum_bf16(dLb, N, V, dLb.stride(0), gb, wide=True)
+                    if _BIAS_AT == "dh":
+                        bias_sum()
+                    elif _BIAS_AT == "recur":
+                        defer.append(bias_sum)
                 if mode_dc == 1:
                     side.wait_stream(torch.cuda.current_stream())
 
@@ -502,7 +525,8 @@
                             ops.gate_wait(gate)
                         ops.gemm_bf16(ops.OP_TN, dLb, Hb, V, H, N, dLb.stride(0), Hb.stride(0), C=gC, ldc=H,
                                       max_pairs=0 if mode_dc == 2 else ops.DC_MAX_PAIRS[0])
-                        ops.colsum_bf16(dLb, N, V, dLb.stride(0), gb, wide=bool(ops.TAIL_SCHEDULE[0]))
+                        if not split or _BIAS_AT == "dc":
+                            ops.colsum_bf16(dLb, N, V, dLb.stride(0), gb, wide=bool(ops.TAIL_SCHEDULE[0]))
                 if mode_dc == 0:
                     side_work()
                 else:
@@ -605,13 +629,18 @@
         return _HiddenFn.apply(anchor, features, self, plan, captions, coins, mode, save), plan
 
     def forward_loss(self, captions, lengths, features=None, targets=None, teacher_forcing_ratio=1.0,
-                     mode="factual", backward=True, n_global=None, grad_hook=None, early_step=None, early_embed=False):
+                     mode="factual", backward=True, n_global=None, grad_hook=None, early_step=None, early_embed=False,
+                     embed_adam=None):
         self._check_inputs(captions, features)
         plan = get_plan(lengths)
         coins = self._coins(plan.T, teacher_forcing_ratio)
         captions = captions.contiguous()
         dev = captions.device
         self.__dict__["_emb_early"] = bool(early_embed and backward and self.bf16 and self._emb().weight.grad is None)
+        split = bool(self.__dict__["_emb_early"] and embed_adam is not None and early_step is not None and all(coins)
+                     and plan.N > 0
+                     and all(p.grad is None for p in self.arena().named.values()))
+        self.__dict__["_emb_adam"] = embed_adam if split else None
         with torch.no_grad():
             c = self._run_forward(plan, captions, features, coins, mode, save=backward)
             N = plan.N
@@ -640,11 +669,18 @@
                 gbuf = self._grad_target(c.grad_names + list(self._out_names()))
                 deferred = []
                 gate_B = plan.B if (c.top.Hpb is not None and not (plan.B >= ops.RECUR_GEMM_MIN_BATCH[0] and self.hidden_size % 64 == 0)) else None
-                dHall = self._vocab_backward(c.top.Hall, logits, gbuf, c.top.Hb, dLb, defer=deferred, gate_B=gate_B)
+                dHall = self._vocab_backward(c.top.Hall, logits, gbuf, c.top.Hb, dLb, defer=deferred, gate_B=gate_B,
+                                             split=split)
                 if dLb is not None:
                     def loss_and_bucket():
-                        with torch.cuda.stream(self._side(0)):
-                            ops.reduce_sum(row_loss, N, 1.0 / denom, loss)
+                        vs = self._side(5 if split else 0)
+                        if split:
+                            with torch.cuda.stream(self._side(6)):
+                                ops.reduce_sum(row_loss, N, 1.0 / denom, loss)
+                            vs.wait_stream(self._side(6))
+                        with torch.cuda.stream(vs):
+                            if not split:
+                                ops.reduce_sum(row_loss, N, 1.0 / denom, loss)
                             if early_step is not None and gbuf is self.arena().gflat:
                                 self._publish(list(self._out_names()), gbuf)
                                 early_step(list(self._out_names()))
@@ -685,6 +721,8 @@
 
 
 V_CAST_SIDE = [os.environ.get("SN_V_CAST_SIDE", "1") == "1"]
+_BIAS_AT = os.environ.get("SN_VOCAB_BIAS_AT", "dh")
+_UNTOUCHED_CTAS = int(os.environ.get("SN_EMB_UNTOUCHED_CTAS", "0"))
 
 
 class DecoderFactoredLSTM(_DecoderBase):
@@ -897,16 +935,29 @@
             self._bucket_final([lp + pre + g + sfx for pre in ("W_", "U_") for g in GATES for sfx in (".weight", ".bias")])
         ops.gemm_bf16(ops.OP_NN, dZb, Ub, N, F, H, 4 * H, Fp, C=dA2, ldc=4 * F, Cb=dA2b, ldcb=4 * F, batch=4, sA=H,
                       sB=H * Fp, sC=F, sCb=F)
+        sc = self._side(6) if getattr(c, "emb_adam", None) is not None else None
         sb.wait_stream(main)
+        if sc is not None:
+            sc.wait_stream(main)
+            with torch.cuda.stream(sc):
+                ops.colsum(dA2, N, 4 * F, 4 * F, gbS, wide=wide)
         with torch.cuda.stream(sb):
             ops.gemm_bf16(ops.OP_TN, dA2b, c.A1, F, F, N, 4 * F, 4 * F, C=gS, ldc=F, batch=4, sA=F, sB=F, sC=F * F)
-            ops.colsum(dA2, N, 4 * F, 4 * F, gbS, wide=wide)
+            if sc is None:
+                ops.colsum(dA2, N, 4 * F, 4 * F, gbS, wide=wide)
         ops.gemm_bf16(ops.OP_NN, dA2b, Sb, N, F, F, 4 * F, Fp, C=dA1, ldc=4 * F, Cb=dA1b, ldcb=4 * F, batch=4, sA=F,
                       sB=F * Fp, sC=F, sCb=F)
         sb.wait_stream(main)
+        if sc is not None:
+            sc.wait_stream(main)
+            with torch.cuda.stream(sc):
+                ops.colsum(dA1, N, 4 * F, 4 * F, gbV, wide=wide)
         with torch.cuda.stream(sb):
             ops.gemm_bf16(ops.OP_TN, dA1b, c.Xb, 4 * F, Ein, N, 4 * F, Ep, C=gV, ldc=Ein)
-            ops.colsum(dA1, N, 4 * F, 4 * F, gbV, wide=wide)
+            if sc is None:
+                ops.colsum(dA1, N, 4 * F, 4 * F, gbV, wide=wide)
+            else:
+                sb.wait_stream(sc)
             self._bucket_final([lp + style_attr(c.mode, g) + sfx for g in GATES for sfx in (".weight", ".bias")] +
                                [lp + "V_" + g + sfx for g in GATES for sfx in (".weight", ".bias")])
         ops.gemm_bf16(ops.OP_NN, dA1b, Vb, N, Ein, 4 * F, 4 * F, Ep, C=dX, ldc=Ein)
diff --git a/image-caption-emotion-indonesia_b200/dp.py b/image-caption-emotion-indonesia_b200/dp.py
--- a/image-caption-emotion-indonesia_b200/dp.py
+++ b/image-caption-emotion-indonesia_b200/dp.py
@@ -188,12 +188,17 @@
         if self.world == 1 and bucketed:
             tail = tail_schedule(self.world, bucketed)
             emb = getattr(self.decoder, "_emb_name", lambda: None)()
-
-            def early_step(names):
-                cap = ops.ADAM_BG_CTAS[0] if (tail and list(names) != [emb]) else 0
-                self.optimizer.step(only=names, max_ctas=cap)
+            embed_adam = None
+            if tail and ops.TAIL_SCHEDULE[0] >= 2 and not getattr(self.decoder, "_layered", False):
+                embed_adam = self.optimizer
+                embed_adam.sync_lr()
+
+            def early_step(names, stepped=False):
+                if not stepped:
+                    cap = ops.ADAM_BG_CTAS[0] if (tail and list(names) != [emb]) else 0
+                    self.optimizer.step(only=names, max_ctas=cap)
                 early.extend(names)
-            kw = dict(kw, early_step=early_step, early_embed=tail)
+            kw = dict(kw, early_step=early_step, early_embed=tail, embed_adam=embed_adam)
         loss, stats = self.forward_backward(captions, lengths, features, n_global=n_global, b_global=b_global,
                                             grad_hook=hook, **kw)
         if self.world > 1:
diff --git a/image-caption-emotion-indonesia_b200/ops.py b/image-caption-emotion-indonesia_b200/ops.py
--- a/image-caption-emotion-indonesia_b200/ops.py
+++ b/image-caption-emotion-indonesia_b200/ops.py
@@ -199,23 +199,44 @@
     return torch.empty(4 * V + 1 + 3 * N, dtype=torch.int32, device=device)
 
 
-def embed_plan(captions, has_feat, row_b, row_t, tok_override, N, V, ws_int):
+def embed_plan(captions, has_feat, row_b, row_t, tok_override, N, V, ws_int, touched=None):
     cap = _req(captions, torch.int64)
     check(lib().sn_embed_plan(_ptr(cap), cap.stride(0), 1 if has_feat else 0, _ptr(row_b), _ptr(row_t),
                               _ptr(tok_override) if tok_override is not None else None, N, V, _ptr(_req(ws_int, torch.int32)),
                               _stream()), "sn_embed_plan")
+    if touched is not None and N > 0:
+        check(lib().sn_embed_touched(_ptr(ws_int), V, _ptr(_req(touched, torch.int32)), _stream()), "sn_embed_touched")
+    elif touched is not None:
+        ws_int[:V].zero_()
+        touched[:1].zero_()
 
 
 def embed_grad(dtable, dfeatures, has_feat, row_b, row_t, tok_override, N, dX, p_drop, seed, ws_int, seed_dev=None,
-               wide=True):
+               wide=True, combine=True):
     V, E = dtable.shape
     ws_part = torch.empty((N // 16 + 1) * E, dtype=torch.float32, device=dX.device)
     check(lib().sn_embed_grad(
         _ptr(_req(dtable)), E, _ptr(dfeatures) if dfeatures is not None else None,
         dfeatures.stride(0) if dfeatures is not None else 0, 1 if has_feat else 0, _ptr(row_b), _ptr(row_t),
         _ptr(tok_override) if tok_override is not None else None, N, _ptr(_req(dX)), dX.stride(0), float(p_drop),
-        ctypes.c_uint64(seed), _ptr(seed_dev), V, _ptr(_req(ws_int, torch.int32)), _ptr(ws_part), 1 if wide else 0, _stream()),
-          "sn_embed_grad")
+        ctypes.c_uint64(seed), _ptr(seed_dev), V, _ptr(_req(ws_int, torch.int32)), _ptr(ws_part), 1 if wide else 0,
+        1 if combine else 0, _stream()), "sn_embed_grad")
+    return ws_part
+
+
+def embed_adam_untouched(p, g, m, v, off, V, E, ws_int, step_idx, steps_dev, lr_dev, coef_ws, beta1, beta2, eps, clip,
+                         max_ctas=0):
+    check(lib().sn_embed_adam_untouched(_bptr(_req(p), off, 4), _bptr(_req(g), off, 4), _bptr(_req(m), off, 4),
+                                        _bptr(_req(v), off, 4), off, V, E, _ptr(_req(ws_int, torch.int32)), int(step_idx),
+                                        _ptr(_req(steps_dev, torch.int32)), _ptr(_req(lr_dev)), _ptr(_req(coef_ws)),
+                                        beta1, beta2, eps, clip, int(max_ctas), _stream()), "sn_embed_adam_untouched")
+
+
+def embed_adam_touched(p, g, m, v, off, V, E, ws_int, ws_part, touched, step_idx, coef_ws, beta1, beta2, eps, clip):
+    check(lib().sn_embed_adam_touched(_bptr(_req(p), off, 4), _bptr(_req(g), off, 4), _bptr(_req(m), off, 4),
+                                      _bptr(_req(v), off, 4), off, V, E, _ptr(_req(ws_int, torch.int32)), _ptr(_req(ws_part)),
+                                      _ptr(_req(touched, torch.int32)), int(step_idx), _ptr(_req(coef_ws)), beta1, beta2,
+                                      eps, clip, _stream()), "sn_embed_adam_touched")
 
 
 _ws_cache = {}
@@ -400,7 +421,7 @@
 DC_SCHEDULE = [int(_os.environ.get("SN_DC_SCHEDULE", "0"))]
 DC_MAX_PAIRS = [int(_os.environ.get("SN_DC_MAX_PAIRS", "37"))]
 
-TAIL_SCHEDULE = [int(_os.environ.get("SN_TAIL_SCHEDULE", "1"))]
+TAIL_SCHEDULE = [int(_os.environ.get("SN_TAIL_SCHEDULE", "2"))]
 ADAM_BG_CTAS = [int(_os.environ.get("SN_ADAM_BG_CTAS", "0"))]
 
 GATE_DC = [int(_os.environ.get("SN_GATE_DC", "0"))]
diff --git a/image-caption-emotion-indonesia_b200/optim.py b/image-caption-emotion-indonesia_b200/optim.py
--- a/image-caption-emotion-indonesia_b200/optim.py
+++ b/image-caption-emotion-indonesia_b200/optim.py
@@ -136,6 +136,27 @@
                     self._step_tensor(p, ("extra", i))
 
     @torch.no_grad()
+    def step_untouched_rows(self, name, plan_ws, max_ctas=0):
+        a = self._state()
+        V, E = a.named[name].shape
+        a.kernel_epoch += 1
+        ops.embed_adam_untouched(a.flat, a.gflat, self.m, self.v, a.offset[name], V, E, plan_ws, self.index[name],
+                                 self.steps_dev, self.lr_dev, self.coef_ws, self.betas[0], self.betas[1], self.eps,
+                                 self.grad_clip, max_ctas=max_ctas)
+
+    @torch.no_grad()
+    def step_touched_rows(self, name, plan_ws, part, touched):
+        a = self._state()
+        V, E = a.named[name].shape
+        a.kernel_epoch += 1
+        ops.embed_adam_touched(a.flat, a.gflat, self.m, self.v, a.offset[name], V, E, plan_ws, part, touched,
+                               self.index[name], self.coef_ws, self.betas[0], self.betas[1], self.eps, self.grad_clip)
+
+    def sync_lr(self):
+        self._state()
+        self._sync_lr()
+
+    @torch.no_grad()
     def step_peer(self, peers, only=None, skip=None, bucket=0):
         a = self._state()
         self._sync_lr()
diff --git a/include/sn100.h b/include/sn100.h
--- a/include/sn100.h
+++ b/include/sn100.h
@@ -40,7 +40,15 @@
 int32_t sn_embed_grad(float* dtable, int64_t E, float* dfeatures, int64_t feat_ld, int32_t has_feat,
                       const int32_t* row_b, const int32_t* row_t, const int32_t* tok_override, int64_t N,
                       const float* dX, int64_t ldx, float p_drop, uint64_t seed, const uint64_t* seed_dev, int64_t V,
-                      const int32_t* ws_int, float* ws_part, int32_t wide, void* stream);
+                      const int32_t* ws_int, float* ws_part, int32_t wide, int32_t combine, void* stream);
+int32_t sn_embed_touched(const int32_t* ws_int, int64_t V, int32_t* touched, void* stream);
+int32_t sn_embed_adam_untouched(float* p, const float* g, float* m, float* v, int64_t off, int64_t V, int64_t E,
+                                const int32_t* ws_int, int32_t step_idx, int32_t* steps_dev, const float* lr_dev,
+                                float* coef_ws, float beta1, float beta2, float eps, float clip, int32_t max_ctas,
+                                void* stream);
+int32_t sn_embed_adam_touched(float* p, float* g, float* m, float* v, int64_t off, int64_t V, int64_t E,
+                              const int32_t* ws_int, const float* ws_part, const int32_t* touched, int32_t step_idx, const float* coef_ws,
+                              float beta1, float beta2, float eps, float clip, void* stream);
 
 int32_t sn_gemm(int32_t op, int64_t M, int64_t N, int64_t K, const float* A, int64_t lda,
                 const float* B, int64_t ldb, float* C, int64_t ldc, const float* bias, float beta,
diff --git a/profiles/tail_ab.py b/profiles/tail_ab.py
--- a/profiles/tail_ab.py
+++ b/profiles/tail_ab.py
@@ -3,10 +3,10 @@
 
 out = sys.argv[1]
 runs = int(sys.argv[2]) if len(sys.argv) > 2 else 5
-arms = {"tail0": {"SN_TAIL_SCHEDULE": "0"}, "tail1": {"SN_TAIL_SCHEDULE": "1"}}
+arms = {"tail1": {"SN_TAIL_SCHEDULE": "1"}, "tail2": {"SN_TAIL_SCHEDULE": "2"}}
 for spec in (sys.argv[3].split(",") if len(sys.argv) > 3 and sys.argv[3] else []):
     name, kv = spec.split(":", 1)
-    arms[name] = dict(SN_TAIL_SCHEDULE="1", **dict(x.split("=", 1) for x in kv.split(";")))
+    arms[name] = dict({"SN_TAIL_SCHEDULE": "2"}, **dict(x.split("=", 1) for x in kv.split(";")))
 os.makedirs(out, exist_ok=True)
 gpu = subprocess.run(["nvidia-smi", "--query-gpu=name,power.limit,clocks.max.sm", "--format=csv,noheader"],
                      capture_output=True, text=True).stdout.strip()
@@ -24,19 +24,20 @@
             f.flush()
 summary = {"gpu": gpu, "runs_per_arm": runs}
 for a, v in res.items():
-    summary[a] = {"median": statistics.median(v), "min": min(v), "max": max(v), "all": v}
+    summary[a] = {"env": arms[a], "median": statistics.median(v), "min": min(v), "max": max(v), "all": v}
 dumps = {}
 with tempfile.TemporaryDirectory() as td:
-    for a in ("tail0", "tail1"):
+    for a in arms:
         d = os.path.join(td, a)
         subprocess.run([sys.executable, "bench.py", "--no-extras", "--no-cpu-baseline", "--steps", "5",
                         "--dump-outputs", d], capture_output=True, text=True, check=True,
                        env=dict(os.environ, **arms[a]))
         dumps[a] = {n: np.load(os.path.join(d, n)) for n in sorted(os.listdir(d)) if n.endswith(".npy")}
-    same = sorted(dumps["tail0"]) == sorted(dumps["tail1"]) and all(
-        np.array_equal(dumps["tail0"][n], dumps["tail1"][n]) for n in dumps["tail0"])
-summary["dump_outputs_identical"] = bool(same)
-summary["dump_outputs_files"] = len(dumps["tail0"])
+first = next(iter(arms))
+summary["dump_outputs_files"] = len(dumps[first])
+summary["dump_outputs_identical_to_" + first] = {
+    a: sorted(dumps[a]) == sorted(dumps[first]) and all(np.array_equal(dumps[a][n], dumps[first][n]) for n in dumps[first])
+    for a in arms if a != first}
 print(json.dumps(summary))
 with open(os.path.join(out, "tail_ab_summary.json"), "w") as f:
     json.dump(summary, f, indent=1)
```

New measurement: 4.876 million (median of 6 runs). 1.07x the previous value.
